# AIM-SE/AC-TSR

Hardware: NVIDIA B200
Metric: AC-SASRec train seq/s (higher is better)
Workload: dtype f32

## Files before the change

### ac-tsr_b200/csrc/attn_bwd.cu

```cuda
#include "attn_bwd_rows.cuh"

namespace acsr {

template <int DH, int G, int MAXNJ, int NS>
__device__ __forceinline__ void bwd_body(const AttnParams& p, const AttnSmem& sm, const BwdSmem<NS>& bs, const RowConst& kc,
                                         const BwdFlags& f, const float* dpen, int b, int h, int nkey, int rstride, BwdAcc& acc) {
  constexpr int dhp = DH + 4;
  constexpr int RPW = 32 / G;
  using CM = CMap<DH, G>;
  const int L = p.L, LP = (L + 3) & ~3;
  const int lane = threadIdx.x & 31, warp = threadIdx.x >> 5;
  const int grp = lane / G, sub = lane % G;
  const int c0 = CM::c0(sub);
  float* wbuf = bs.rowbuf + warp * rowbuf_floats_per_warp(LP, 2 * NS);
  const int rt = p.ctx_rows ? (int)p.ctx_rows[b] - 1 : -1;
  float accOq[CM::CPL], accDq[CM::CPL];
#pragma unroll
  for (int k = 0; k < CM::CPL; ++k) accOq[k] = accDq[k] = 0.f;
  for (int t0 = next_task(sm.misc + 2, RPW); t0 < L; t0 = next_task(sm.misc + 2, RPW)) {
    const int iw = L - 1 - t0;
    const int iraw = iw - grp;
    const bool rowok = iraw >= 0;
    const int i = rowok ? iraw : 0;
    const int bound = p.full ? nkey : min(i + 1, nkey);
    const int nj = ((p.full ? nkey : min(iw + 1, nkey)) + G - 1) / G;
    if (rt >= 0 && (rt > iw || rt <= iw - RPW)) {
#define ACSR_BWD_ROW_M(NJV) bwd_row_iter_m<DH, G, NJV, NS>(p, sm, bs, kc, dpen, b, h, i, rowok, bound, grp, sub, rstride, wbuf)
      if (MAXNJ == 1 || nj == 1) ACSR_BWD_ROW_M(1);
      else if (nj == 2) ACSR_BWD_ROW_M((MAXNJ >= 2 ? 2 : 1));
      else ACSR_BWD_ROW_M((MAXNJ >= 4 ? 4 : 1));
#undef ACSR_BWD_ROW_M
      continue;
    }
#define ACSR_BWD_ROW(NJV) \
  bwd_row_iter<DH, G, NJV, NS>(p, sm, bs, kc, f, dpen, b, h, i, rowok, bound, grp, sub, rstride, wbuf, acc, accOq, accDq)
    if (MAXNJ == 1 || nj == 1) ACSR_BWD_ROW(1);
    else if (nj == 2) ACSR_BWD_ROW((MAXNJ >= 2 ? 2 : 1));
    else ACSR_BWD_ROW((MAXNJ >= 4 ? 4 : 1));
#undef ACSR_BWD_ROW
  }
  if ((p.d_ow || p.d_dw) && CM::split(sub) == 0) {
#pragma unroll
    for (int k = 0; k < CM::CPL; ++k) {
      const int c = c0 + k;
      if (accOq[k] != 0.f) atomicAdd(bs.pacc + c, accOq[k]);
      if (accDq[k] != 0.f) atomicAdd(bs.pacc + 2 * DH + c, accDq[k]);
    }
  }
}

template <int DH, int CG, int NS>
__device__ __forceinline__ void bwd_cols(const AttnParams& p, const AttnSmem& sm, const BwdSmem<NS>& bs, const BwdFlags& f, int b, int h,
                                         int nkey) {
  constexpr int dhp = DH + 4;
  constexpr int RPW = 32 / CG;
  using CM = CMap<DH, CG>;
  const int L = p.L, LP = (L + 3) & ~3;
  const int lane = threadIdx.x & 31;
  const int grp = lane / CG, sub = lane % CG;
  const int c0 = CM::c0(sub);
  float accOk[CM::CPL], accDk[CM::CPL];
#pragma unroll
  for (int k = 0; k < CM::CPL; ++k) accOk[k] = accDk[k] = 0.f;
  for (int t0 = next_task(sm.misc + 3, RPW); t0 < nkey; t0 = next_task(sm.misc + 3, RPW)) {
    const int jraw = t0 + grp;
    const bool colok = jraw < nkey;
    const int j = colok ? jraw : 0;
    float ak_[NS][CM::CPL], ak2_[NS][CM::CPL], av_[NS][CM::CPL];
#pragma unroll
    for (int s = 0; s < NS; ++s)
#pragma unroll
      for (int k = 0; k < CM::CPL; ++k) ak_[s][k] = ak2_[s][k] = av_[s][k] = 0.f;
    int lo, hi;
    CM::slice(sub, p.full ? 0 : (j & ~3), LP, lo, hi);
    const int off = mat_row(p, j, LP);
    for (int i = lo; i < hi; i += 4) {
      float s1v[NS][4], s2v[NS][4];
#pragma unroll
      for (int s = 0; s < NS; ++s) {
        const float4 s1 = *reinterpret_cast<const float4*>(bs.matST[s] + off + i);
        const float4 s2 = *reinterpret_cast<const float4*>(bs.matS2T[s] + off + i);
        s1v[s][0] = s1.x; s1v[s][1] = s1.y; s1v[s][2] = s1.z; s1v[s][3] = s1.w;
        s2v[s][0] = s2.x; s2v[s][1] = s2.y; s2v[s][2] = s2.z; s2v[s][3] = s2.w;
      }
      const float4 pr = *reinterpret_cast<const float4*>(bs.matRT + off + i);
      const float4 pa = *reinterpret_cast<const float4*>(bs.matAT + off + i);
      const float prv[4] = {pr.x, pr.y, pr.z, pr.w}, pav[4] = {pa.x, pa.y, pa.z, pa.w};
#pragma unroll
      for (int u = 0; u < 4; ++u) {
        float qv[CM::CPL], q2v[CM::CPL], t0v[CM::CPL], t1v[CM::CPL];
        VecLd<CM::CPL>::ld(sm.Q + (i + u) * dhp + c0, qv);
        VecLd<CM::CPL>::ld(sm.Q2 + (i + u) * dhp + c0, q2v);
        VecLd<CM::CPL>::ld(bs.sT0 + (i + u) * dhp + c0, t0v);
        VecLd<CM::CPL>::ld(bs.sT1 + (i + u) * dhp + c0, t1v);
#pragma unroll
        for (int k = 0; k < CM::CPL; ++k) {
#pragma unroll
          for (int s = 0; s < NS; ++s) {
            ak_[s][k] = fmaf(s1v[s][u], qv[k], ak_[s][k]);
            ak2_[s][k] = fmaf(s2v[s][u], q2v[k], ak2_[s][k]);
          }
          av_[0][k] = fmaf(prv[u], t0v[k], av_[0][k]);
          av_[NS - 1][k] = fmaf(f.t1_att ? pav[u] : prv[u], t1v[k], av_[NS - 1][k]);
        }
      }
    }
    float kv[CM::CPL];
    VecLd<CM::CPL>::ld(sm.K + j * dhp + c0, kv);
#pragma unroll
    for (int s = 0; s < NS; ++s) {
      const float cdu = bs.colDU[s * LP + j], cdt = bs.colDT[s * LP + j];
      float o1[CM::CPL], o2[CM::CPL], o3[CM::CPL];
#pragma unroll
      for (int k = 0; k < CM::CPL; ++k) {
        o1[k] = CM::reduce(ak_[s][k]) + cdu * sm.wo[DH + c0 + k] + cdt * sm.wd[DH + c0 + k];
        o2[k] = CM::reduce(ak2_[s][k]);
        o3[k] = CM::reduce(av_[s][k]);
      }
      if (CM::split(sub) == 0 && colok) {
        const long long o = s * p.s1_td + ((long long)b * L + j) * p.d + h * DH + c0;
        VecLd<CM::CPL>::st(p.d_mk + o, o1);
        VecLd<CM::CPL>::st(p.d_ak + o, o2);
        VecLd<CM::CPL>::st(p.d_mv + o, o3);
        if (s == 0) {
#pragma unroll
          for (int k = 0; k < CM::CPL; ++k) { accOk[k] = fmaf(cdu, kv[k], accOk[k]); accDk[k] = fmaf(cdt, kv[k], accDk[k]); }
        }
      }
    }
  }
  if ((p.d_ow || p.d_dw) && CM::split(sub) == 0) {
#pragma unroll
    for (int k = 0; k < CM::CPL; ++k) {
      const int c = c0 + k;
      if (accOk[k] != 0.f) atomicAdd(bs.pacc + DH + c, accOk[k]);
      if (accDk[k] != 0.f) atomicAdd(bs.pacc + 3 * DH + c, accDk[k]);
    }
  }
}

template <int DH, int NS>
__global__ void __launch_bounds__(kAttnThreads, 2) attn_bwd_kernel(const AttnParams p) {
  pdl_launch_dependents();
  pdl_wait();
  extern __shared__ __align__(16) float smem_f[];
  constexpr int dhp = DH + 4;
  const int L = p.L, LP = (L + 3) & ~3;
  const int TRI = mat_floats(p.full, L, LP);
  const int b = p.order ? p.order[blockIdx.x / p.H] : (int)(blockIdx.x / p.H), h = blockIdx.x % p.H;
  const int lane = threadIdx.x & 31, warp = threadIdx.x >> 5;
  float* ptr = smem_f;
  AttnSmem sm = carve_common(ptr, LP, DH);
  BwdSmem<NS> bs;
  bs.sT0 = ptr; ptr += LP * dhp;
  bs.sT1 = ptr; ptr += LP * dhp;
#pragma unroll
  for (int s = 0; s < NS; ++s) { bs.matST[s] = ptr; ptr += TRI; bs.matS2T[s] = ptr; ptr += TRI; }
  bs.matRT = ptr; ptr += TRI;
  bs.matAT = ptr; ptr += TRI;
  bs.rowbuf = ptr; ptr += kAttnWarps * rowbuf_floats_per_warp(LP, 2 * NS);
  bs.colDU = ptr; ptr += NS * LP;
  bs.colDT = ptr; ptr += NS * LP;
  bs.pacc = ptr; ptr += 4 * DH;
  bs.red = ptr; ptr += kAttnWarps * 4;
  BwdFlags f;
  f.has_t0 = p.t0 != nullptr || p.dprob_cal != nullptr; f.has_t1 = p.t1 != nullptr || p.dprob_att != nullptr;
  f.t1_att = NS == 1 ? true : (p.t1_is_att != 0);
  f.has_att = f.has_t1 && f.t1_att;
  f.gate = p.combine == ACSR_ATTN_COMBINE_GATE;

  stage_tile<DH>(bs.sT0, p.t0, b, h, L, p.d, L, LP);
  stage_tile<DH>(bs.sT1, p.t1, b, h, L, p.d, L, LP);
  {
    const int ntri = (2 * NS + 2) * TRI;
    float4* z4 = reinterpret_cast<float4*>(bs.matST[0]);
    for (int e = threadIdx.x; e < ntri / 4; e += blockDim.x) z4[e] = make_float4(0.f, 0.f, 0.f, 0.f);
  }
  for (int j = threadIdx.x; j < NS * LP; j += blockDim.x) { bs.colDU[j] = 0.f; bs.colDT[j] = 0.f; }
  for (int j = threadIdx.x; j < 4 * DH; j += blockDim.x) bs.pacc[j] = 0.f;
  const int nkey = stage_common<DH>(p, sm, b, h, LP);

  const RowConst kc = make_consts<DH>(p, f.has_att);
  f.sc2 = kc.sc * kc.sc;
  float dpen[NS];
  dpen[0] = p.d_pen0 ? p.d_pen0[0] : 0.f;
  if (NS == 2) dpen[NS - 1] = p.d_pen1 ? p.d_pen1[0] : 0.f;
  BwdAcc acc;
  acc.s_ob = acc.s_db = acc.s_scalar = acc.s_ratio = 0.f;

  if (nkey <= 8) bwd_body<DH, 8, 1, NS>(p, sm, bs, kc, f, dpen, b, h, nkey, 8, acc);
  else bwd_body<DH, 16, 4, NS>(p, sm, bs, kc, f, dpen, b, h, nkey, LP, acc);
  __syncthreads();
  if (nkey <= 8) bwd_cols<DH, 32, NS>(p, sm, bs, f, b, h, nkey);
  else bwd_cols<DH, 16, NS>(p, sm, bs, f, b, h, nkey);

  for (int e = threadIdx.x; e < (L - nkey) * (DH / 4); e += blockDim.x) {
    const int j = nkey + e / (DH / 4), c4 = e % (DH / 4);
    const float4 z = make_float4(0.f, 0.f, 0.f, 0.f);
#pragma unroll
    for (int s = 0; s < NS; ++s) {
      const long long o = s * p.s1_td + ((long long)b * L + j) * p.d + h * DH + c4 * 4;
      *reinterpret_cast<float4*>(p.d_mk + o) = z;
      *reinterpret_cast<float4*>(p.d_ak + o) = z;
      *reinterpret_cast<float4*>(p.d_mv + o) = z;
    }
  }
  const float s_ob = warp_sum(acc.s_ob), s_db = warp_sum(acc.s_db);
  const float s_scalar = warp_sum(acc.s_scalar), s_ratio = warp_sum(acc.s_ratio);
  if (lane == 0) {
    bs.red[warp * 4 + 0] = s_ob; bs.red[warp * 4 + 1] = s_db; bs.red[warp * 4 + 2] = s_scalar; bs.red[warp * 4 + 3] = s_ratio;
  }
  __syncthreads();
  if (threadIdx.x < 4) {
    float s = 0.f;
    for (int w = 0; w < kAttnWarps; ++w) s += bs.red[w * 4 + threadIdx.x];
    float* dst = threadIdx.x == 0 ? p.d_ob : threadIdx.x == 1 ? p.d_db : threadIdx.x == 2 ? p.d_scalar : p.d_ratio;
    if (dst != nullptr && s != 0.f) atomicAdd(dst, s);
  }
  for (int c = threadIdx.x; c < 4 * DH; c += blockDim.x) {
    const float v = bs.pacc[c];
    float* dst = c < 2 * DH ? p.d_ow : p.d_dw;
    if (dst != nullptr && v != 0.f) atomicAdd(dst + (c < 2 * DH ? c : c - 2 * DH), v);
  }
}

static size_t bwd_smem_bytes(int L, int dh, int ns, int bidir) {
  const int LP = (L + 3) & ~3;
  size_t f = common_floats(LP, dh) + (size_t)2 * LP * (dh + 4) + (size_t)(2 * ns + 2) * mat_floats(bidir, L, LP) +
             (size_t)kAttnWarps * rowbuf_floats_per_warp(LP, 2 * ns) + 2 * ns * LP + 4 * dh + kAttnWarps * 4;
  return f * sizeof(float);
}

template <int DH, int NS>
static int launch_bwd(const AttnParams& p, cudaStream_t st) {
  size_t smem = bwd_smem_bytes(p.L, DH, NS, p.full);
  int rc = prep_kernel(attn_bwd_kernel<DH, NS>, smem, "attn_calib_bwd");
  if (rc) return rc;
  launch_pdl(attn_bwd_kernel<DH, NS>, dim3(p.B * p.H), dim3(kAttnThreads), smem, st, p);
  return check_launch("attn_calib_bwd");
}

template <int NS>
static int dispatch_bwd(const AttnParams& p, cudaStream_t st) {
  switch (p.dh) {
    case 8: return launch_bwd<8, NS>(p, st);
    case 16: return launch_bwd<16, NS>(p, st);
    case 32: return launch_bwd<32, NS>(p, st);
    case 64: return launch_bwd<64, NS>(p, st);
  }
  return ACSR_ERR_UNSUPPORTED;
}

}

using namespace acsr;

extern "C" {

int acsr_attn_calib_bwd(const float* d_ctx_att, const float* d_ctx_cal, const float* d_pen_sq, const float* mq, const float* mk,
                        const float* mv, const float* aq, const float* ak, const float* gate_logit, const int64_t* item_seq,
                        const float* order_w, const float* order_b, const float* dist_w, const float* dist_b, const float* scalar,
                        int B, int L, int H, int dh, int two_level, int combine_option, float comb_scalar, int rich_mode,
                        const float* rich_ratio, float p_attn, const float* D1, const float* D2, const float* D3,
                        const float* noise, const void* rng, uint32_t rng_stream, float* d_mq, float* d_mk, float* d_mv,
                        float* d_aq, float* d_ak, float* d_gate_logit, float* d_order_w, float* d_order_b, float* d_dist_w,
                        float* d_dist_b, float* d_scalar, float* d_rich_ratio, const int32_t* order, const int64_t* ctx_rows,
                        void* stream) {
  AttnParams p = {};
  attn_fill_common(p, mq, mk, mv, aq, ak, gate_logit, item_seq, order_w, order_b, dist_w, dist_b, scalar, B, L, H, dh, two_level,
                   combine_option, comb_scalar, rich_mode, rich_ratio, p_attn, D1, D2, D3, noise, rng, rng_stream, order, ctx_rows);
  p.t0 = d_ctx_cal; p.t1 = d_ctx_att; p.t1_is_att = 1; p.d_pen0 = d_pen_sq;
  p.d_mq = d_mq; p.d_mk = d_mk; p.d_mv = d_mv; p.d_aq = d_aq; p.d_ak = d_ak; p.d_gate = d_gate_logit;
  p.d_ow = d_order_w; p.d_ob = d_order_b; p.d_dw = d_dist_w; p.d_db = d_dist_b; p.d_scalar = d_scalar; p.d_ratio = d_rich_ratio;
  plain_range(p, d_ctx_att != nullptr);
  int rc = attn_validate(p, "attn_calib_bwd");
  if (rc) return rc;
  ACSR_REQUIRE(d_mq && d_mk && d_mv && d_aq && d_ak, "attn_calib_bwd: NULL output");
  ACSR_REQUIRE(combine_option != ACSR_ATTN_COMBINE_GATE || d_gate_logit != nullptr, "attn_calib_bwd: d_gate_logit is NULL");
  if (L > 64) return attn_long_bwd(p, 1, (cudaStream_t)stream);
  return dispatch_bwd<1>(p, (cudaStream_t)stream);
}

int acsr_attn_calib_ti_bwd(const float* d_ctx_att, const float* d_ctx_cal, const float* d_pen_sq, const float* d_prob_att,
                           const float* d_prob_cal, const float* s_bias, const float* mq, const float* mk,
                           const float* mv, const float* aq, const float* ak, const float* gate_logit, const int64_t* item_seq,
                           const float* order_w, const float* order_b, const float* dist_w, const float* dist_b, const float* scalar,
                           int B, int L, int H, int dh, int two_level, int combine_option, float comb_scalar, int rich_mode,
                           const float* rich_ratio, float p_attn, const float* D1, const float* D2, const float* D3,
                           const float* noise, const void* rng, uint32_t rng_stream, float* d_mq, float* d_mk, float* d_mv,
                           float* d_aq, float* d_ak, float* d_gate_logit, float* d_order_w, float* d_order_b, float* d_dist_w,
                           float* d_dist_b, float* d_scalar, float* d_rich_ratio, float* d_s_bias, void* stream) {
  AttnParams p = {};
  attn_fill_common(p, mq, mk, mv, aq, ak, gate_logit, item_seq, order_w, order_b, dist_w, dist_b, scalar, B, L, H, dh, two_level,
                   combine_option, comb_scalar, rich_mode, rich_ratio, p_attn, D1, D2, D3, noise, rng, rng_stream, nullptr, nullptr);
  p.t0 = d_ctx_cal; p.t1 = d_ctx_att; p.t1_is_att = 1; p.d_pen0 = d_pen_sq;
  p.s_bias = s_bias; p.dprob_att = d_prob_att; p.dprob_cal = d_prob_cal; p.d_s_bias = d_s_bias;
  p.d_mq = d_mq; p.d_mk = d_mk; p.d_mv = d_mv; p.d_aq = d_aq; p.d_ak = d_ak; p.d_gate = d_gate_logit;
  p.d_ow = d_order_w; p.d_ob = d_order_b; p.d_dw = d_dist_w; p.d_db = d_dist_b; p.d_scalar = d_scalar; p.d_ratio = d_rich_ratio;
  plain_range(p, d_ctx_att != nullptr || d_prob_att != nullptr);
  int rc = attn_validate(p, "attn_calib_ti_bwd");
  if (rc) return rc;
  ACSR_REQUIRE(d_mq && d_mk && d_mv && d_aq && d_ak, "attn_calib_ti_bwd: NULL output");
  ACSR_REQUIRE(combine_option != ACSR_ATTN_COMBINE_GATE || d_gate_logit != nullptr, "attn_calib_ti_bwd: d_gate_logit is NULL");
  ACSR_REQUIRE(p.plain && L <= 64, "attn_calib_ti_bwd: the time-aware terms need ACSR_ATTN_PLAIN and L <= 64");
  return dispatch_bwd<1>(p, (cudaStream_t)stream);
}

int acsr_attn_calib_bwd2(const float* d_ctx_cal0, const float* d_pen_sq0, const float* d_ctx_att1, const float* d_ctx_cal1,
                         const float* d_pen_sq1, const float* mq, const float* mk, const float* mv, const float* aq,
                         const float* ak, const float* gate_logit, const int64_t* item_seq, const float* order_w,
                         const float* order_b, const float* dist_w, const float* dist_b, const float* scalar, int B, int L, int H,
                         int dh, int two_level, int combine_option, float comb_scalar, int rich_mode, const float* rich_ratio,
                         float p_attn, const float* D1, const float* D2, const float* D3, const float* noise, const void* rng,
                         uint32_t rng_stream, float* d_mq, float* d_mk, float* d_mv, float* d_aq, float* d_ak,
                         float* d_gate_logit, float* d_order_w, float* d_order_b, float* d_dist_w, float* d_dist_b,
                         float* d_scalar, float* d_rich_ratio, const int32_t* order, const int64_t* ctx_rows, void* stream) {
  AttnParams p = {};
  attn_fill_common(p, mq, mk, mv, aq, ak, gate_logit, item_seq, order_w, order_b, dist_w, dist_b, scalar, B, L, H, dh, two_level,
                   combine_option, comb_scalar, rich_mode, rich_ratio, p_attn, D1, D2, D3, noise, rng, rng_stream, order, ctx_rows);
  ACSR_REQUIRE(!(d_ctx_att1 && d_ctx_cal1), "attn_calib_bwd2: stream 1 takes d_ctx_att or d_ctx_cal, not both");
  p.t0 = d_ctx_cal0; p.t1 = d_ctx_att1 ? d_ctx_att1 : d_ctx_cal1; p.t1_is_att = d_ctx_att1 != nullptr;
  p.d_pen0 = d_pen_sq0; p.d_pen1 = d_pen_sq1;
  p.s1_td = (long long)B * L * H * dh; p.s1_ll = (long long)B * L * L;
  p.d_mq = d_mq; p.d_mk = d_mk; p.d_mv = d_mv; p.d_aq = d_aq; p.d_ak = d_ak; p.d_gate = d_gate_logit;
  p.d_ow = d_order_w; p.d_ob = d_order_b; p.d_dw = d_dist_w; p.d_db = d_dist_b; p.d_scalar = d_scalar; p.d_ratio = d_rich_ratio;
  plain_range(p, d_ctx_att1 != nullptr);
  int rc = attn_validate(p, "attn_calib_bwd2");
  if (rc) return rc;
  ACSR_REQUIRE(d_mq && d_mk && d_mv && d_aq && d_ak, "attn_calib_bwd2: NULL output");
  ACSR_REQUIRE(combine_option != ACSR_ATTN_COMBINE_GATE || d_gate_logit != nullptr, "attn_calib_bwd2: d_gate_logit is NULL");
  if (L > 64) return attn_long_bwd(p, 2, (cudaStream_t)stream);
  return dispatch_bwd<2>(p, (cudaStream_t)stream);
}

}
```

### ac-tsr_b200/csrc/attn_bwd_rows.cuh

```cuda
#pragma once
#include "attn_common.cuh"

namespace acsr {

template <int NS>
struct BwdSmem {
  float *sT0, *sT1;
  float *matST[NS], *matS2T[NS];
  float *matRT, *matAT;
  float *rowbuf;
  float *colDU, *colDT;
  float *pacc;
  float *red;
  float *gS[NS], *gS2[NS], *gR, *gA;
};

struct BwdAcc {
  float s_ob, s_db, s_scalar, s_ratio;
};

struct BwdFlags {
  bool has_t0, has_t1, t1_att, has_att, gate;
  float sc2;
};

template <int DH, int G, int NJ, int NS, bool LONG = false>
__device__ __forceinline__ void bwd_row_iter(const AttnParams& p, const AttnSmem& sm, const BwdSmem<NS>& bs, const RowConst& kc,
                                             const BwdFlags& f, const float* dpen, int b, int h, int i, bool rowok, int bound,
                                             int grp, int sub, int rstride, float* wbuf, BwdAcc& acc, float* accOq,
                                             float* accDq) {
  constexpr int dhp = DH + 4;
  using CM = CMap<DH, G>;
  const int L = p.L, LP = (L + 3) & ~3;
  RowF<NJ> r;
  row_forward<DH, G, NJ>(p, sm, kc, b, h, i, bound, sub, f.has_att, r);
  const unsigned act = r.act;
  float d0[NJ], d1[NJ];
#pragma unroll
  for (int jj = 0; jj < NJ; ++jj) d0[jj] = d1[jj] = 0.f;
  if (f.has_t0 || f.has_t1) {
    const float4* a0 = reinterpret_cast<const float4*>(bs.sT0 + i * dhp);
    const float4* a1 = reinterpret_cast<const float4*>(bs.sT1 + i * dhp);
#pragma unroll
    for (int jj = 0; jj < NJ; ++jj) {
      const int jcl = ((act >> jj) & 1u) ? sub + G * jj : 0;
      const float4* vj = reinterpret_cast<const float4*>(sm.V + jcl * dhp);
      float x0 = 0.f, x1 = 0.f;
#pragma unroll
      for (int c4 = 0; c4 < DH / 4; ++c4) {
        const float4 v = vj[c4];
        if (f.has_t0) x0 = dot4(a0[c4], v, x0);
        if (f.has_t1) x1 = dot4(a1[c4], v, x1);
      }
      if ((act >> jj) & 1u) { d0[jj] = x0; d1[jj] = x1; }
    }
  }
  if (p.dprob_cal != nullptr || p.dprob_att != nullptr) {
    const long long ebase = (((long long)b * p.H + h) * L + i) * L;
#pragma unroll
    for (int jj = 0; jj < NJ; ++jj)
      if ((act >> jj) & 1u) {
        const int j = sub + G * jj;
        if (p.dprob_cal != nullptr) d0[jj] += __ldg(p.dprob_cal + ebase + j);
        if (p.dprob_att != nullptr) d1[jj] += __ldg(p.dprob_att + ebase + j);
      }
  }
  float Pj[NJ], Mj[NJ], Oj[NJ], expm[NJ];
#pragma unroll
  for (int jj = 0; jj < NJ; ++jj) {
    const bool a = (act >> jj) & 1u;
    Pj[jj] = r.Psoft[jj] * r.D1[jj];
    Mj[jj] = r.Msoft[jj] * r.D3[jj];
    Oj[jj] = p.two_level ? Pj[jj] : r.P0soft[jj] * r.D2[jj];
    expm[jj] = a ? fexp(1.0f - Mj[jj]) : 0.f;
    if (a && rowok) {
      const int j = sub + G * jj;
      const float rfin = p.two_level ? r.R[jj] : (kc.rr * r.R[jj] + (1.0f - kc.rr) * Pj[jj]);
      if (LONG) {
        bs.gR[(long long)i * L + j] = rfin;
        bs.gA[(long long)i * L + j] = r.A[jj];
      } else {
        const int t = mat_row(p, j, LP) + i;
        bs.matRT[t] = rfin;
        bs.matAT[t] = r.A[jj];
      }
    }
  }
  float* gbuf = wbuf + grp * 2 * NS * rstride;
  bool live[NS];
  float row_du[NS], row_dt[NS];
#pragma unroll
  for (int s = 0; s < NS; ++s) {
    float* bufS = gbuf + (2 * s + 0) * rstride;
    float* bufS2 = gbuf + (2 * s + 1) * rstride;
    row_du[s] = row_dt[s] = 0.f;
    const float* dRf = (NS == 1 || s == 0) ? d0 : d1;
    const float* dA = d1;
    bool useR = (NS == 1 || s == 0) ? f.has_t0 : (f.has_t1 && !f.t1_att);
    bool useA = (NS == 1) ? f.has_t1 : (s == 1 && f.has_t1 && f.t1_att);
    bool nzR = false, nzA = false;
#pragma unroll
    for (int jj = 0; jj < NJ; ++jj) { nzR |= dRf[jj] != 0.f; nzA |= dA[jj] != 0.f; }
    useR = useR && __any_sync(kFull, nzR && rowok);
    useA = useA && __any_sync(kFull, nzA && rowok);
    const float dp = dpen[s];
    live[s] = useR || useA || dp != 0.f;
    if (!live[s]) {
      if (LONG && rowok) {
#pragma unroll
        for (int jj = 0; jj < NJ; ++jj)
          if ((act >> jj) & 1u) {
            const long long e = (long long)i * L + sub + G * jj;
            bs.gS[s][e] = 0.f;
            bs.gS2[s][e] = 0.f;
          }
      }
      continue;
    }
    const bool owner = s == 0;
    float dO[NJ], dP[NJ], dM[NJ], tmp[NJ];
#pragma unroll
    for (int jj = 0; jj < NJ; ++jj) { dO[jj] = 0.f; dP[jj] = 0.f; dM[jj] = 0.f; }
    if (useR) {
      float dR[NJ], dcm[NJ], dC[NJ];
#pragma unroll
      for (int jj = 0; jj < NJ; ++jj) {
        if (p.two_level) dR[jj] = dRf[jj];
        else {
          dR[jj] = dRf[jj] * kc.rr;
          dP[jj] = dRf[jj] * (1.0f - kc.rr);
          if (owner && rowok) acc.s_ratio += dRf[jj] * (r.R[jj] - Pj[jj]);
        }
      }
      if (p.plain) {
#pragma unroll
        for (int jj = 0; jj < NJ; ++jj) dcm[jj] = dR[jj];
      } else softmax_bwd_row<G, NJ>(r.R, dR, dcm);
      if (p.combine == ACSR_ATTN_COMBINE_FIXED) {
        softmax_bwd_row<G, NJ>(r.F, dcm, tmp);
#pragma unroll
        for (int jj = 0; jj < NJ; ++jj) { dO[jj] += tmp[jj]; dC[jj] = 0.5f * tmp[jj]; }
      } else {
#pragma unroll
        for (int jj = 0; jj < NJ; ++jj) {
          const float g = r.g[jj];
          dO[jj] += dcm[jj] * g;
          dC[jj] = dcm[jj] * (1.0f - g);
          if (f.gate && ((act >> jj) & 1u) && rowok) {
            const float dgl = dcm[jj] * (Oj[jj] - r.C[jj]) * g * (1.0f - g);
            if (dgl != 0.f) atomicAdd(p.d_gate + s * p.s1_ll + ((long long)b * L + i) * L + sub + G * jj, dgl);
          }
        }
      }
      if (p.plain) {
#pragma unroll
        for (int jj = 0; jj < NJ; ++jj) tmp[jj] = dC[jj];
      } else softmax_bwd_row<G, NJ>(r.C, dC, tmp);
#pragma unroll
      for (int jj = 0; jj < NJ; ++jj) {
        dO[jj] += tmp[jj] * expm[jj];
        dM[jj] -= tmp[jj] * Oj[jj] * expm[jj];
      }
    }
    if (useA) {
      if (p.plain) {
#pragma unroll
        for (int jj = 0; jj < NJ; ++jj) tmp[jj] = dA[jj];
      } else softmax_bwd_row<G, NJ>(r.A, dA, tmp);
#pragma unroll
      for (int jj = 0; jj < NJ; ++jj) {
        dO[jj] += tmp[jj] * Mj[jj];
        dM[jj] += tmp[jj] * (Oj[jj] - r.nz[jj]);
      }
    }
    float dS2[NJ], dS[NJ], dz[NJ];
#pragma unroll
    for (int jj = 0; jj < NJ; ++jj) {
      if ((act >> jj) & 1u) dM[jj] += dp * (-2.0f) * (1.0f - Mj[jj]);
      dM[jj] *= r.D3[jj];
    }
    softmax_bwd_row<G, NJ>(r.Msoft, dM, dS2);
#pragma unroll
    for (int jj = 0; jj < NJ; ++jj) { dS2[jj] *= kc.inv_sq; dz[jj] = 0.f; dS[jj] = 0.f; }
    if (useR || useA) {
      float dP0[NJ];
#pragma unroll
      for (int jj = 0; jj < NJ; ++jj) {
        if (p.two_level) { dP[jj] += dO[jj]; dP0[jj] = 0.f; }
        else dP0[jj] = dO[jj] * r.D2[jj];
        dP[jj] *= r.D1[jj];
      }
      softmax_bwd_row<G, NJ>(r.Psoft, dP, dz);
#pragma unroll
      for (int jj = 0; jj < NJ; ++jj) { dz[jj] *= kc.inv_sq; dS[jj] = dz[jj]; }
      if (!p.two_level) {
        softmax_bwd_row<G, NJ>(r.P0soft, dP0, tmp);
#pragma unroll
        for (int jj = 0; jj < NJ; ++jj) dS[jj] += tmp[jj] * kc.inv_sq;
      }
    }
    float rdu = 0.f, rdt = 0.f;
#pragma unroll
    for (int jj = 0; jj < NJ; ++jj) {
      const int j = sub + G * jj;
      const bool a = ((act >> jj) & 1u) && rowok;
      if (j < rstride) { bufS[j] = a ? dS[jj] : 0.f; bufS2[j] = a ? dS2[jj] : 0.f; }
      if (!a) continue;
      if (p.ow) {
        const float sg = r.sig[jj];
        const float de = (j > i) ? sg * (1.0f - sg) * frcp(sg + kOrderEps) : -sg * (1.0f - sg) * frcp((1.0f - sg) + kOrderEps);
        const float du = dz[jj] * de;
        rdu += du;
        if (du != 0.f) atomicAdd(bs.colDU + s * LP + j, du);
      }
      if (p.dw) {
        const float dl = r.delta[jj];
        const float dt = dz[jj] * dl * f.sc2;
        rdt += dt;
        if (dt != 0.f) atomicAdd(bs.colDT + s * LP + j, dt);
        if (owner) acc.s_scalar += dz[jj] * (-(dl * dl) * kc.sc);
      }
      if (LONG) {
        bs.gS[s][(long long)i * L + j] = dS[jj];
        bs.gS2[s][(long long)i * L + j] = dS2[jj];
      } else {
        const int t = mat_row(p, j, LP) + i;
        bs.matST[s][t] = dS[jj];
        bs.matS2T[s][t] = dS2[jj];
        if (NS == 1 && p.d_s_bias != nullptr) p.d_s_bias[(((long long)b * p.H + h) * L + i) * L + j] = dS[jj];
      }
    }
    row_du[s] = grp_sum<G>(rdu);
    row_dt[s] = grp_sum<G>(rdt);
  }
  if (sub == 0) { acc.s_ob += row_du[0]; acc.s_db += row_dt[0]; }
  __syncwarp();
  float aq_[NS][CM::CPL], aq2_[NS][CM::CPL];
#pragma unroll
  for (int s = 0; s < NS; ++s)
#pragma unroll
    for (int k = 0; k < CM::CPL; ++k) aq_[s][k] = aq2_[s][k] = 0.f;
  int lo, hi;
  CM::slice(sub, 0, (bound + 3) & ~3, lo, hi);
  const int c0 = CM::c0(sub);
  bool any_live = false;
#pragma unroll
  for (int s = 0; s < NS; ++s) any_live |= live[s];
  if (any_live) {
    for (int j = lo; j < hi; j += 4) {
      float s1v[NS][4], s2v[NS][4];
#pragma unroll
      for (int s = 0; s < NS; ++s) {
        const float4 s1 = *reinterpret_cast<const float4*>(gbuf + (2 * s + 0) * rstride + j);
        const float4 s2 = *reinterpret_cast<const float4*>(gbuf + (2 * s + 1) * rstride + j);
        s1v[s][0] = s1.x; s1v[s][1] = s1.y; s1v[s][2] = s1.z; s1v[s][3] = s1.w;
        s2v[s][0] = s2.x; s2v[s][1] = s2.y; s2v[s][2] = s2.z; s2v[s][3] = s2.w;
      }
#pragma unroll
      for (int u = 0; u < 4; ++u) {
        float kv[CM::CPL], k2v[CM::CPL];
        VecLd<CM::CPL>::ld(sm.K + (j + u) * dhp + c0, kv);
        VecLd<CM::CPL>::ld(sm.K2 + (j + u) * dhp + c0, k2v);
#pragma unroll
        for (int s = 0; s < NS; ++s) {
          if (!live[s]) continue;
#pragma unroll
          for (int k = 0; k < CM::CPL; ++k) {
            aq_[s][k] = fmaf(s1v[s][u], kv[k], aq_[s][k]);
            aq2_[s][k] = fmaf(s2v[s][u], k2v[k], aq2_[s][k]);
          }
        }
      }
    }
  }
  {
    float qv[CM::CPL];
    VecLd<CM::CPL>::ld(sm.Q + i * dhp + c0, qv);
#pragma unroll
    for (int s = 0; s < NS; ++s) {
      float o1[CM::CPL], o2[CM::CPL];
#pragma unroll
      for (int k = 0; k < CM::CPL; ++k) {
        o1[k] = CM::reduce(aq_[s][k]) + row_du[s] * sm.wo[c0 + k] + row_dt[s] * sm.wd[c0 + k];
        o2[k] = CM::reduce(aq2_[s][k]);
      }
      if (CM::split(sub) == 0 && rowok) {
        const long long o = s * p.s1_td + ((long long)b * L + i) * p.d + h * DH + c0;
        VecLd<CM::CPL>::st(p.d_mq + o, o1);
        VecLd<CM::CPL>::st(p.d_aq + o, o2);
      }
    }
    if (CM::split(sub) == 0 && rowok) {
#pragma unroll
      for (int k = 0; k < CM::CPL; ++k) { accOq[k] = fmaf(row_du[0], qv[k], accOq[k]); accDq[k] = fmaf(row_dt[0], qv[k], accDq[k]); }
    }
  }
  __syncwarp();
}

template <int DH, int G, int NJ, int NS, bool LONG = false>
__device__ __forceinline__ void bwd_row_iter_m(const AttnParams& p, const AttnSmem& sm, const BwdSmem<NS>& bs, const RowConst& kc,
                                               const float* dpen, int b, int h, int i, bool rowok, int bound, int grp, int sub,
                                               int rstride, float* wbuf) {
  constexpr int dhp = DH + 4;
  using CM = CMap<DH, G>;
  const int L = p.L, LP = (L + 3) & ~3;
  float Msoft[NJ], D3[NJ];
  unsigned act;
  row_forward_m<DH, G, NJ>(p, sm, kc, b, h, i, bound, sub, Msoft, D3, act);
  float* gbuf = wbuf + grp * 2 * NS * rstride;
  const int c0 = CM::c0(sub);
  if (LONG && rowok) {
#pragma unroll
    for (int jj = 0; jj < NJ; ++jj)
      if ((act >> jj) & 1u) {
        const long long e = (long long)i * L + sub + G * jj;
        bs.gR[e] = 0.f;
        bs.gA[e] = 0.f;
#pragma unroll
        for (int s = 0; s < NS; ++s) {
          bs.gS[s][e] = 0.f;
          if (dpen[s] == 0.f) bs.gS2[s][e] = 0.f;
        }
      }
  }
#pragma unroll
  for (int s = 0; s < NS; ++s) {
    const float dp = dpen[s];
    float o2[CM::CPL];
#pragma unroll
    for (int k = 0; k < CM::CPL; ++k) o2[k] = 0.f;
    if (dp != 0.f) {
      float dM[NJ], dS2[NJ];
#pragma unroll
      for (int jj = 0; jj < NJ; ++jj) dM[jj] = ((act >> jj) & 1u) ? dp * (-2.0f) * (1.0f - Msoft[jj] * D3[jj]) * D3[jj] : 0.f;
      softmax_bwd_row<G, NJ>(Msoft, dM, dS2);
      float* bufS2 = gbuf + (2 * s + 1) * rstride;
#pragma unroll
// ... 39 lines not shown
```

### ac-tsr_b200/csrc/attn_common.cuh

```cuda
#pragma once
#include "acsr_common.cuh"
#include "../../include/acsr.h"

namespace acsr {

constexpr int kAttnWarps = 8;
constexpr int kAttnThreads = kAttnWarps * 32;
constexpr unsigned kFull = 0xffffffffu;

struct AttnParams {
  const float *mq, *mk, *mv, *aq, *ak, *gate;
  const int64_t* item_seq;
  const int32_t* order;
  const int64_t* ctx_rows;
  const float *ow, *ob, *dw, *db, *scalar;
  int B, L, H, dh, d;
  int two_level, combine, rich;
  int bidir;
  int plain;
  int full;
  float comb_scalar;
  const float* rich_ratio;
  float p;
  const float *D1, *D2, *D3, *noise;
  const RngState* rng;
  uint32_t stream;
  float *ctx_att, *ctx_cal;
  double* pen_sq;
  float* probs;
  const float* s_bias;
  float *prob_att_out, *prob_cal_out;
  const float *dprob_att, *dprob_cal;
  float* d_s_bias;
  const float *t0, *t1;
  int t1_is_att;
  const float *d_pen0, *d_pen1;
  long long s1_td, s1_ll;
  float *d_mq, *d_mk, *d_mv, *d_aq, *d_ak, *d_gate, *d_ow, *d_ob, *d_dw, *d_db, *d_scalar, *d_ratio;
};

template <int G>
__device__ __forceinline__ float grp_sum(float v) {
#pragma unroll
  for (int o = G / 2; o > 0; o >>= 1) v += __shfl_xor_sync(kFull, v, o);
  return v;
}
template <int G>
__device__ __forceinline__ float grp_max(float v) {
#pragma unroll
  for (int o = G / 2; o > 0; o >>= 1) v = fmaxf(v, __shfl_xor_sync(kFull, v, o));
  return v;
}

template <int DH, int G>
struct CMap {
  static constexpr int CPL = DH >= G ? DH / G : 1;
  static constexpr int SPL = DH >= G ? 1 : G / DH;
  __device__ static __forceinline__ int c0(int sub) { return DH >= G ? sub * CPL : sub % DH; }
  __device__ static __forceinline__ int split(int sub) { return DH >= G ? 0 : sub / DH; }
  __device__ static __forceinline__ float reduce(float v) {
#pragma unroll
    for (int o = DH; o < G; o <<= 1) v += __shfl_xor_sync(kFull, v, o);
    return v;
  }
  __device__ static __forceinline__ void slice(int sub, int begin, int end, int& lo, int& hi) {
    if (SPL == 1) { lo = begin; hi = end; return; }
    const int chunk = (((end - begin + SPL - 1) / SPL) + 3) & ~3;
    lo = begin + split(sub) * chunk;
    hi = min(end, lo + chunk);
  }
};

template <int N> struct VecLd;
template <> struct VecLd<1> {
  __device__ static __forceinline__ void ld(const float* p, float* v) { v[0] = p[0]; }
  __device__ static __forceinline__ void st(float* p, const float* v) { p[0] = v[0]; }
};
template <> struct VecLd<2> {
  __device__ static __forceinline__ void ld(const float* p, float* v) { const float2 t = *reinterpret_cast<const float2*>(p); v[0] = t.x; v[1] = t.y; }
  __device__ static __forceinline__ void st(float* p, const float* v) { *reinterpret_cast<float2*>(p) = make_float2(v[0], v[1]); }
};
template <> struct VecLd<4> {
  __device__ static __forceinline__ void ld(const float* p, float* v) { const float4 t = *reinterpret_cast<const float4*>(p); v[0] = t.x; v[1] = t.y; v[2] = t.z; v[3] = t.w; }
  __device__ static __forceinline__ void st(float* p, const float* v) { *reinterpret_cast<float4*>(p) = make_float4(v[0], v[1], v[2], v[3]); }
};
template <> struct VecLd<8> {
  __device__ static __forceinline__ void ld(const float* p, float* v) { VecLd<4>::ld(p, v); VecLd<4>::ld(p + 4, v + 4); }
  __device__ static __forceinline__ void st(float* p, const float* v) { VecLd<4>::st(p, v); VecLd<4>::st(p + 4, v + 4); }
};

template <int NJ>
struct RowF {
  float Psoft[NJ], Msoft[NJ], P0soft[NJ];
  float D1[NJ], D2[NJ], D3[NJ], nz[NJ];
  float A[NJ], C[NJ], g[NJ], F[NJ], R[NJ];
  float sig[NJ], delta[NJ];
  unsigned act;
  unsigned valid;
};

struct AttnSmem {
  float *Q, *K, *V, *Q2, *K2;
  float *rowO, *rowD, *colO, *colD, *logd, *keyok;
  float *wo, *wd;
  const float* G;
  int* misc;
};

struct RowConst {
  float ob, db, sc, sc2h, rr, inv_sq, inv_keep;
  unsigned thr16;
  unsigned long long seed, step;
  bool philox_drop, philox_noise, need_p0;
  bool bounded;
};

__device__ __forceinline__ float fex2(float x) { float y; asm("ex2.approx.ftz.f32 %0, %1;" : "=f"(y) : "f"(x)); return y; }
__device__ __forceinline__ float flg2(float x) { float y; asm("lg2.approx.ftz.f32 %0, %1;" : "=f"(y) : "f"(x)); return y; }
__device__ __forceinline__ float frcp(float x) { float y; asm("rcp.approx.ftz.f32 %0, %1;" : "=f"(y) : "f"(x)); return y; }
__device__ __forceinline__ float fexp(float x) { return fex2(x * 1.4426950408889634f); }
__device__ __forceinline__ float flog(float x) { return flg2(x) * 0.6931471805599453f; }
__device__ __forceinline__ float fsigmoid(float x) { return frcp(1.0f + fex2(x * -1.4426950408889634f)); }

__device__ __forceinline__ void cp_async16(void* smem, const void* gmem) {
  asm volatile("cp.async.cg.shared.global [%0], [%1], 16;" ::"r"(smem_u32(smem)), "l"(gmem) : "memory");
}
__device__ __forceinline__ void cp_async4(void* smem, const void* gmem) {
  asm volatile("cp.async.ca.shared.global [%0], [%1], 4;" ::"r"(smem_u32(smem)), "l"(gmem) : "memory");
}
__device__ __forceinline__ void cp_async_wait_all() {
  asm volatile("cp.async.commit_group;\n\tcp.async.wait_group 0;" ::: "memory");
}

__device__ __forceinline__ float dot4(const float4 a, const float4 b, float acc) {
  acc = fmaf(a.x, b.x, acc); acc = fmaf(a.y, b.y, acc); acc = fmaf(a.z, b.z, acc); acc = fmaf(a.w, b.w, acc);
  return acc;
}

template <int G, int NJ>
__device__ __forceinline__ void softmax_row(const float* z, unsigned act, float* y) {
  float m = -INFINITY;
#pragma unroll
  for (int jj = 0; jj < NJ; ++jj) if ((act >> jj) & 1u) m = fmaxf(m, z[jj]);
  m = grp_max<G>(m) * 1.4426950408889634f;
  float s = 0.f;
#pragma unroll
  for (int jj = 0; jj < NJ; ++jj) { y[jj] = ((act >> jj) & 1u) ? fex2(fmaf(z[jj], 1.4426950408889634f, -m)) : 0.f; s += y[jj]; }
  s = grp_sum<G>(s);
  const float inv = frcp(s);
#pragma unroll
  for (int jj = 0; jj < NJ; ++jj) y[jj] *= inv;
}

template <int G, int NJ>
__device__ __forceinline__ void softmax_row_bounded(const float* z, unsigned act, float* y) {
  float s = 0.f;
#pragma unroll
  for (int jj = 0; jj < NJ; ++jj) { y[jj] = ((act >> jj) & 1u) ? fex2(z[jj] * 1.4426950408889634f) : 0.f; s += y[jj]; }
  s = grp_sum<G>(s);
  const float inv = s > 0.f ? frcp(s) : 0.f;
#pragma unroll
  for (int jj = 0; jj < NJ; ++jj) y[jj] *= inv;
}

template <int G, int NJ>
__device__ __forceinline__ void softmax_bwd_row(const float* y, const float* dy, float* dz) {
  float s = 0.f;
#pragma unroll
  for (int jj = 0; jj < NJ; ++jj) s = fmaf(y[jj], dy[jj], s);
  s = grp_sum<G>(s);
#pragma unroll
  for (int jj = 0; jj < NJ; ++jj) dz[jj] = y[jj] * (dy[jj] - s);
}

__device__ __forceinline__ int next_task(int* counter, int step) {
  int t = 0;
  if ((threadIdx.x & 31) == 0) t = atomicAdd(counter, step);
  return __shfl_sync(kFull, t, 0);
}

__host__ __device__ __forceinline__ int tri_off(int j, int LP) {
  const int a = j >> 2, b = j & 3;
  return j * LP - 8 * a * (a - 1) - 4 * a * b;
}

__device__ __forceinline__ int mat_row(const AttnParams& p, int j, int LP) { return p.full ? j * LP : tri_off(j, LP) - (j & ~3); }
__host__ __device__ __forceinline__ int mat_floats(int bidir, int L, int LP) { return bidir ? L * LP : tri_off(L, LP); }

template <int DH>
__device__ __forceinline__ void stage_tile(float* dst, const float* __restrict__ src, int b, int h, int L, int d, int rows,
                                           int rows_pad) {
  constexpr int dhp = DH + 4;
  if (src == nullptr) rows = 0;
  const float* base = src + (long long)b * L * d + h * DH;
  for (int e = threadIdx.x; e < rows_pad * (DH / 4); e += blockDim.x) {
    const int r = e / (DH / 4), c4 = e % (DH / 4);
    if (r < rows) cp_async16(dst + r * dhp + c4 * 4, base + (long long)r * d + c4 * 4);
    else *reinterpret_cast<float4*>(dst + r * dhp + c4 * 4) = make_float4(0.f, 0.f, 0.f, 0.f);
  }
}

template <int DH>
__device__ __forceinline__ int stage_common(const AttnParams& p, const AttnSmem& sm, int b, int h, int LP) {
  constexpr int dhp = DH + 4;
  const int L = p.L;
  if (threadIdx.x < 64) {
    const int j = threadIdx.x;
    const bool ok = j < L && p.item_seq[(long long)b * L + j] != 0;
    const unsigned m = __ballot_sync(kFull, ok);
    if ((threadIdx.x & 31) == 0) sm.misc[threadIdx.x >> 5] = (int)m;
    if (threadIdx.x >= 2 && threadIdx.x < 5) sm.misc[threadIdx.x] = 0;
    if (j < LP) { sm.keyok[j] = ok ? 1.0f : 0.0f; sm.logd[j] = logf((float)j + 1.0f); }
  }
  stage_tile<DH>(sm.Q, p.mq, b, h, L, p.d, L, LP);
  stage_tile<DH>(sm.Q2, p.aq, b, h, L, p.d, L, LP);
  for (int c = threadIdx.x; c < 2 * DH; c += blockDim.x) {
    sm.wo[c] = p.ow ? p.ow[c] : 0.f;
    sm.wd[c] = p.dw ? p.dw[c] : 0.f;
  }
  __syncthreads();
  const unsigned m0 = (unsigned)sm.misc[0], m1 = (unsigned)sm.misc[1];
  int nkey = m1 ? 64 - __clz(m1) : (m0 ? 32 - __clz(m0) : 0);
  nkey = max(nkey, 1);
  if (p.plain && p.full) nkey = L;
  const int nkp = (nkey + 3) & ~3;
  stage_tile<DH>(sm.K, p.mk, b, h, L, p.d, nkey, nkp);
  stage_tile<DH>(sm.V, p.mv, b, h, L, p.d, nkey, nkp);
  stage_tile<DH>(sm.K2, p.ak, b, h, L, p.d, nkey, nkp);
  cp_async_wait_all();
  __syncthreads();
  if (p.ow || p.dw) {
    const int j = threadIdx.x >> 2, part = threadIdx.x & 3;
    float ro = 0.f, rd = 0.f, co = 0.f, cd = 0.f;
    if (j < L) {
#pragma unroll
      for (int cc = 0; cc < DH / 4; ++cc) {
        const int c = part * (DH / 4) + cc;
        const float q = sm.Q[j * dhp + c];
        ro = fmaf(q, sm.wo[c], ro); rd = fmaf(q, sm.wd[c], rd);
        if (j < nkey) {
          const float k = sm.K[j * dhp + c];
          co = fmaf(k, sm.wo[DH + c], co); cd = fmaf(k, sm.wd[DH + c], cd);
        }
      }
    }
    ro += __shfl_xor_sync(kFull, ro, 1); ro += __shfl_xor_sync(kFull, ro, 2);
    rd += __shfl_xor_sync(kFull, rd, 1); rd += __shfl_xor_sync(kFull, rd, 2);
    co += __shfl_xor_sync(kFull, co, 1); co += __shfl_xor_sync(kFull, co, 2);
    cd += __shfl_xor_sync(kFull, cd, 1); cd += __shfl_xor_sync(kFull, cd, 2);
    if (part == 0 && j < LP) { sm.rowO[j] = ro; sm.rowD[j] = rd; sm.colO[j] = co; sm.colD[j] = cd; }
    __syncthreads();
  }
  return nkey;
}

template <int DH>
__device__ __forceinline__ RowConst make_consts(const AttnParams& p, bool need_att) {
  RowConst k;
  k.ob = p.ob ? p.ob[0] : 0.f;
  k.db = p.db ? p.db[0] : 0.f;
  k.sc = p.scalar ? p.scalar[0] : 0.f;
  k.sc2h = k.sc * k.sc * 0.5f;
  k.rr = 1.0f;
  if (!p.two_level) k.rr = (p.rich == ACSR_ATTN_RICH_TRAINABLE) ? p.rich_ratio[0] : 0.5f;
  k.inv_sq = 1.0f / sqrtf((float)DH);
  k.inv_keep = p.p > 0.f ? 1.0f / (1.0f - p.p) : 1.0f;
  k.thr16 = (unsigned)(p.p * 65536.0f + 0.5f);
  k.bounded = k.inv_keep <= 16.0f;
  k.philox_drop = p.p > 0.f && p.D1 == nullptr;
  k.philox_noise = need_att && p.noise == nullptr && p.rng != nullptr;
  k.need_p0 = !p.two_level || p.probs != nullptr;
  k.seed = 0; k.step = 0;
  if (p.rng != nullptr) { k.seed = p.rng->seed; k.step = p.rng->step; }
  return k;
}

template <int DH, int G, int NJ>
__device__ __forceinline__ void row_forward(const AttnParams& p, const AttnSmem& sm, const RowConst& kc, int b, int h, int i,
                                            int bound, int sub, bool need_att, RowF<NJ>& r) {
  constexpr int dhp = DH + 4;
  const int L = p.L;
  int jc[NJ];
  float S[NJ], S2[NJ], gl[NJ];
  unsigned act = 0;
#pragma unroll
  for (int jj = 0; jj < NJ; ++jj) {
    const int j = sub + G * jj;
    const bool a = j < bound;
    act |= (a ? 1u : 0u) << jj;
    jc[jj] = a ? j : 0;
    gl[jj] = 0.f;
  }
  r.act = act;
  const long long ebase = (((long long)b * p.H + h) * L + i) * L;
  if (p.combine == ACSR_ATTN_COMBINE_GATE) {
    if (sm.G != nullptr) {
      const float* gp = sm.G + i * L;
#pragma unroll
      for (int jj = 0; jj < NJ; ++jj) if ((act >> jj) & 1u) gl[jj] = gp[jc[jj]];
    } else {
      const float* gp = p.gate + ((long long)b * L + i) * L;
#pragma unroll
      for (int jj = 0; jj < NJ; ++jj) if ((act >> jj) & 1u) gl[jj] = __ldg(gp + jc[jj]);
    }
  }
  {
    const float4* qi = reinterpret_cast<const float4*>(sm.Q + i * dhp);
    const float4* q2i = reinterpret_cast<const float4*>(sm.Q2 + i * dhp);
    if (NJ == 1) {
      const float4* kj = reinterpret_cast<const float4*>(sm.K + jc[0] * dhp);
      const float4* k2j = reinterpret_cast<const float4*>(sm.K2 + jc[0] * dhp);
      float s = 0.f, s2 = 0.f;
#pragma unroll
      for (int c4 = 0; c4 < DH / 4; ++c4) { s = dot4(qi[c4], kj[c4], s); s2 = dot4(q2i[c4], k2j[c4], s2); }
      S[0] = s; S2[0] = s2;
    } else {
      {
        float4 q[DH / 4];
#pragma unroll
        for (int c4 = 0; c4 < DH / 4; ++c4) q[c4] = qi[c4];
#pragma unroll
        for (int jj = 0; jj < NJ; ++jj) {
          const float4* kj = reinterpret_cast<const float4*>(sm.K + jc[jj] * dhp);
          float s = 0.f;
#pragma unroll
          for (int c4 = 0; c4 < DH / 4; ++c4) s = dot4(q[c4], kj[c4], s);
          S[jj] = s;
        }
      }
      {
        float4 q[DH / 4];
#pragma unroll
        for (int c4 = 0; c4 < DH / 4; ++c4) q[c4] = q2i[c4];
#pragma unroll
        for (int jj = 0; jj < NJ; ++jj) {
          const float4* kj = reinterpret_cast<const float4*>(sm.K2 + jc[jj] * dhp);
          float s = 0.f;
#pragma unroll
          for (int c4 = 0; c4 < DH / 4; ++c4) s = dot4(q[c4], kj[c4], s);
          S2[jj] = s;
        }
      }
    }
  }
  if (p.s_bias != nullptr) {
#pragma unroll
    for (int jj = 0; jj < NJ; ++jj) if ((act >> jj) & 1u) S[jj] += __ldg(p.s_bias + ebase + jc[jj]);
  }
  const float rowO = sm.rowO[i], rowD = sm.rowD[i];
  float zP[NJ], z0[NJ], zM[NJ];
  unsigned valid = 0;
#pragma unroll
  for (int jj = 0; jj < NJ; ++jj) {
    const int j = jc[jj];
    const bool a = (act >> jj) & 1u;
    const bool v = a && (p.bidir || j <= i) && (sm.keyok[j] != 0.f);
    valid |= (v ? 1u : 0u) << jj;
    const float msk = v ? 0.f : kMaskNeg;
    r.sig[jj] = 0.f; r.delta[jj] = 0.f;
    float eo = 0.f, ed = 0.f;
    if (p.ow) {
      const float sg = fsigmoid(rowO + sm.colO[j] + kc.ob);
      r.sig[jj] = sg;
      eo = (j > i) ? flog(sg + kOrderEps) : flog((1.0f - sg) + kOrderEps);
    }
    if (p.dw) {
      const int dist = i > j ? i - j : j - i;
      const float dl = sm.logd[dist] - (rowD + sm.colD[j] + kc.db);
      r.delta[jj] = dl;
      ed = -(dl * dl) * kc.sc2h;
    }
    zP[jj] = (S[jj] + eo + ed) * kc.inv_sq + msk;
    z0[jj] = S[jj] * kc.inv_sq + msk;
    zM[jj] = S2[jj] * kc.inv_sq + msk;
  }
  r.valid = valid;
  softmax_row<G, NJ>(zP, act, r.Psoft);
  softmax_row<G, NJ>(zM, act, r.Msoft);
  if (kc.need_p0) softmax_row<G, NJ>(z0, act, r.P0soft);
  else {
#pragma unroll
    for (int jj = 0; jj < NJ; ++jj) r.P0soft[jj] = 0.f;
  }
#pragma unroll
  for (int jj = 0; jj < NJ; ++jj) { r.D1[jj] = r.D2[jj] = r.D3[jj] = 1.0f; r.nz[jj] = 0.f; }
  if (kc.philox_drop || kc.philox_noise) {
#pragma unroll
    for (int jj = 0; jj < NJ; jj += 2) {
      const uint4 w = philox4x32(kc.seed, kc.step, p.stream, (unsigned long long)(ebase + jc[jj]));
      if (kc.philox_drop) {
        r.D1[jj] = ((w.x & 0xffffu) >= kc.thr16) ? kc.inv_keep : 0.f;
        r.D3[jj] = ((w.x >> 16) >= kc.thr16) ? kc.inv_keep : 0.f;
        if (jj + 1 < NJ) {
          r.D1[jj + 1] = ((w.y & 0xffffu) >= kc.thr16) ? kc.inv_keep : 0.f;
          r.D3[jj + 1] = ((w.y >> 16) >= kc.thr16) ? kc.inv_keep : 0.f;
        }
      }
      if (kc.philox_noise) {
        const float rad = sqrtf(-2.0f * flog(u32_to_unit(w.z)));
        float sn, cs;
        __sincosf(6.283185307179586f * u32_to_unit(w.w), &sn, &cs);
        r.nz[jj] = rad * cs;
        if (jj + 1 < NJ) r.nz[jj + 1] = rad * sn;
      }
      if (kc.philox_drop && kc.need_p0) {
        const uint4 w2 = philox4x32(kc.seed, kc.step, p.stream + 1u, (unsigned long long)(ebase + jc[jj]));
        r.D2[jj] = ((w2.x & 0xffffu) >= kc.thr16) ? kc.inv_keep : 0.f;
        if (jj + 1 < NJ) r.D2[jj + 1] = ((w2.x >> 16) >= kc.thr16) ? kc.inv_keep : 0.f;
      }
    }
  }
  if (p.D1 || p.noise) {
#pragma unroll
    for (int jj = 0; jj < NJ; ++jj) {
      if (!((act >> jj) & 1u)) continue;
      const long long e = ebase + jc[jj];
      if (p.D1) r.D1[jj] = p.D1[e];
      if (p.D2) r.D2[jj] = p.D2[e];
      if (p.D3) r.D3[jj] = p.D3[e];
      if (p.noise) r.nz[jj] = p.noise[e];
    }
  }
  float O[NJ], M[NJ], expm[NJ], z[NJ];
#pragma unroll
  for (int jj = 0; jj < NJ; ++jj) {
    const bool a = (act >> jj) & 1u;
    M[jj] = r.Msoft[jj] * r.D3[jj];
    O[jj] = p.two_level ? r.Psoft[jj] * r.D1[jj] : r.P0soft[jj] * r.D2[jj];
    expm[jj] = a ? fexp(1.0f - M[jj]) : 0.f;
  }
  if (need_att) {
#pragma unroll
    for (int jj = 0; jj < NJ; ++jj)
      z[jj] = O[jj] * M[jj] + r.nz[jj] * (1.0f - M[jj]) + ((p.plain || ((valid >> jj) & 1u)) ? 0.f : kMaskNeg);
    if (p.plain) {
#pragma unroll
      for (int jj = 0; jj < NJ; ++jj) r.A[jj] = ((act >> jj) & 1u) ? z[jj] : 0.f;
    } else softmax_row<G, NJ>(z, act, r.A);
  } else {
#pragma unroll
    for (int jj = 0; jj < NJ; ++jj) r.A[jj] = 0.f;
  }
#pragma unroll
  for (int jj = 0; jj < NJ; ++jj) z[jj] = O[jj] * expm[jj] + ((p.plain || ((valid >> jj) & 1u)) ? 0.f : kMaskNeg);
  if (p.plain) {
#pragma unroll
    for (int jj = 0; jj < NJ; ++jj) r.C[jj] = z[jj];
  } else if (kc.bounded) softmax_row_bounded<G, NJ>(z, act, r.C);
  else softmax_row<G, NJ>(z, act, r.C);
  if (p.combine == ACSR_ATTN_COMBINE_FIXED) {
    const float ninact = (float)(L - bound);
    float m = -INFINITY;
#pragma unroll
    for (int jj = 0; jj < NJ; ++jj) { z[jj] = O[jj] + 0.5f * r.C[jj]; r.g[jj] = 0.f; if ((act >> jj) & 1u) m = fmaxf(m, z[jj]); }
    m = grp_max<G>(m);
    if (ninact > 0.f) m = fmaxf(m, 0.f);
    float s = 0.f;
#pragma unroll
    for (int jj = 0; jj < NJ; ++jj) { r.F[jj] = ((act >> jj) & 1u) ? fexp(z[jj] - m) : 0.f; s += r.F[jj]; }
    s = grp_sum<G>(s) + ninact * fexp(-m);
    const float inv = frcp(s);
#pragma unroll
    for (int jj = 0; jj < NJ; ++jj) { r.F[jj] *= inv; z[jj] = r.F[jj] + (((valid >> jj) & 1u) ? 0.f : kMaskNeg); }
  } else {
#pragma unroll
    for (int jj = 0; jj < NJ; ++jj) {
      float g = p.comb_scalar;
      if (p.combine == ACSR_ATTN_COMBINE_GATE) g = fsigmoid(gl[jj]);
      r.g[jj] = g; r.F[jj] = 0.f;
      z[jj] = g * O[jj] + (1.0f - g) * r.C[jj] + ((p.plain || ((valid >> jj) & 1u)) ? 0.f : kMaskNeg);
    }
  }
  if (p.plain) {
    const bool fixed = p.combine == ACSR_ATTN_COMBINE_FIXED;
#pragma unroll
    for (int jj = 0; jj < NJ; ++jj) r.R[jj] = fixed ? r.F[jj] : (((act >> jj) & 1u) ? z[jj] : 0.f);
    return;
  }
  if (kc.bounded) softmax_row_bounded<G, NJ>(z, act, r.R);
  else softmax_row<G, NJ>(z, act, r.R);
}

template <int DH, int G, int NJ>
__device__ __forceinline__ void row_forward_m(const AttnParams& p, const AttnSmem& sm, const RowConst& kc, int b, int h, int i,
                                              int bound, int sub, float* Msoft, float* D3, unsigned& act_out) {
  constexpr int dhp = DH + 4;
  const int L = p.L;
  int jc[NJ];
  float zM[NJ];
  unsigned act = 0;
#pragma unroll
  for (int jj = 0; jj < NJ; ++jj) {
    const int j = sub + G * jj;
    const bool a = j < bound;
    act |= (a ? 1u : 0u) << jj;
    jc[jj] = a ? j : 0;
  }
  act_out = act;
  const long long ebase = (((long long)b * p.H + h) * L + i) * L;
  const float4* q2i = reinterpret_cast<const float4*>(sm.Q2 + i * dhp);
#pragma unroll
  for (int jj = 0; jj < NJ; ++jj) {
    const float4* kj = reinterpret_cast<const float4*>(sm.K2 + jc[jj] * dhp);
    float s0 = 0.f, s1 = 0.f;
#pragma unroll
    for (int c4 = 0; c4 < DH / 4; c4 += 2) { s0 = dot4(q2i[c4], kj[c4], s0); s1 = dot4(q2i[c4 + 1], kj[c4 + 1], s1); }
    const bool v = ((act >> jj) & 1u) && (p.bidir || jc[jj] <= i) && (sm.keyok[jc[jj]] != 0.f);
    zM[jj] = (s0 + s1) * kc.inv_sq + (v ? 0.f : kMaskNeg);
  }
  softmax_row<G, NJ>(zM, act, Msoft);
#pragma unroll
  for (int jj = 0; jj < NJ; ++jj) D3[jj] = 1.0f;
  if (kc.philox_drop) {
#pragma unroll
    for (int jj = 0; jj < NJ; jj += 2) {
      const uint4 w = philox4x32(kc.seed, kc.step, p.stream, (unsigned long long)(ebase + jc[jj]));
      D3[jj] = ((w.x >> 16) >= kc.thr16) ? kc.inv_keep : 0.f;
      if (jj + 1 < NJ) D3[jj + 1] = ((w.y >> 16) >= kc.thr16) ? kc.inv_keep : 0.f;
    }
  }
  if (p.D3) {
#pragma unroll
    for (int jj = 0; jj < NJ; ++jj) if ((act >> jj) & 1u) D3[jj] = p.D3[ebase + jc[jj]];
  }
}

__device__ __forceinline__ AttnSmem carve_common(float*& ptr, int LP, int dh) {
  AttnSmem sm;
  const int tile = LP * (dh + 4);
  sm.Q = ptr; ptr += tile;
  sm.K = ptr; ptr += tile;
  sm.V = ptr; ptr += tile;
  sm.Q2 = ptr; ptr += tile;
  sm.K2 = ptr; ptr += tile;
  sm.rowO = ptr; ptr += LP;
  sm.rowD = ptr; ptr += LP;
  sm.colO = ptr; ptr += LP;
  sm.colD = ptr; ptr += LP;
  sm.logd = ptr; ptr += LP;
  sm.keyok = ptr; ptr += LP;
  sm.wo = ptr; ptr += 2 * dh;
  sm.wd = ptr; ptr += 2 * dh;
  sm.misc = reinterpret_cast<int*>(ptr); ptr += 8;
  sm.G = nullptr;
  return sm;
}
static inline size_t common_floats(int LP, int dh) { return (size_t)5 * LP * (dh + 4) + 6 * LP + 4 * dh + 8; }

__host__ __device__ __forceinline__ int rowbuf_floats_per_warp(int LP, int bufs_per_row) {
  const int a = 2 * bufs_per_row * LP, b = 4 * bufs_per_row * 8;
  return a > b ? a : b;
}

template <typename K>
static int prep_kernel(K kernel, size_t smem, const char* who) {
  if (smem > 227 * 1024) { set_error("%s: needs %zu bytes of shared memory (> 227 KB)", who, smem); return ACSR_ERR_UNSUPPORTED; }
  cudaError_t e = cudaFuncSetAttribute(kernel, cudaFuncAttributeMaxDynamicSharedMemorySize, (int)smem);
  if (e == cudaSuccess) e = cudaFuncSetAttribute(kernel, cudaFuncAttributePreferredSharedMemoryCarveout, 100);
  if (e != cudaSuccess) { set_error("%s: smem %zu: %s", who, smem, cudaGetErrorString(e)); return ACSR_ERR_CUDA; }
  return ACSR_OK;
}

static inline int attn_validate(const AttnParams& p, const char* who) {
  ACSR_REQUIRE(p.mq && p.mk && p.mv && p.aq && p.ak && p.item_seq, "%s: NULL input", who);
  ACSR_REQUIRE(p.B > 0 && p.H > 0, "%s: bad B/H", who);
  if (p.L < 1 || p.L > 256) { set_error("%s: L=%d unsupported (1..256)", who, p.L); return ACSR_ERR_UNSUPPORTED; }
  if ((p.full || p.plain) && p.L > 64) { set_error("%s: the bidirectional mask / the transformer_layers variant are implemented for L <= 64 (L=%d)", who, p.L); return ACSR_ERR_UNSUPPORTED; }
  if (!(p.dh == 8 || p.dh == 16 || p.dh == 32 || p.dh == 64)) {
    set_error("%s: head size %d unsupported (8/16/32/64)", who, p.dh);
    return ACSR_ERR_UNSUPPORTED;
  }
  ACSR_REQUIRE((p.ow == nullptr) == (p.ob == nullptr), "%s: order_w/order_b mismatch", who);
  ACSR_REQUIRE((p.dw == nullptr) == (p.db == nullptr) && (p.dw == nullptr) == (p.scalar == nullptr), "%s: distance params mismatch", who);
  ACSR_REQUIRE(p.combine >= 0 && p.combine <= 2, "%s: unknown combine_option %d", who, p.combine);
  ACSR_REQUIRE(p.combine != ACSR_ATTN_COMBINE_GATE || p.gate != nullptr, "%s: combine_option gate needs gate_logit", who);
  ACSR_REQUIRE(p.two_level || p.rich == ACSR_ATTN_RICH_FIXED || (p.rich == ACSR_ATTN_RICH_TRAINABLE && p.rich_ratio),
               "%s: two_level=False needs rich_calibrated_combine fixed/trainable", who);
  ACSR_REQUIRE(p.p >= 0.f && p.p < 1.f, "%s: dropout p=%f", who, p.p);
  ACSR_REQUIRE(!(p.p > 0.f && p.D1 == nullptr && p.rng == nullptr), "%s: p>0 needs explicit masks or rng", who);
  ACSR_REQUIRE((p.D1 == nullptr) == (p.D3 == nullptr), "%s: D1/D3 must be given together", who);
  return ACSR_OK;
}

static inline void plain_range(AttnParams& p, bool attacked_stream) {
  if (p.plain && !p.bidir && !attacked_stream && p.combine != ACSR_ATTN_COMBINE_FIXED) p.full = 0;
}

int attn_long_fwd(const AttnParams& p, cudaStream_t st);
int attn_long_bwd(const AttnParams& p, int ns, cudaStream_t st);
int seq_order_long(const int64_t* item_seq, int B, int L, int32_t* order, cudaStream_t st);

static inline void attn_fill_common(AttnParams& p, const float* mq, const float* mk, const float* mv, const float* aq,
                                    const float* ak, const float* gate_logit, const int64_t* item_seq, const float* order_w,
                                    const float* order_b, const float* dist_w, const float* dist_b, const float* scalar, int B,
                                    int L, int H, int dh, int two_level, int combine_option, float comb_scalar, int rich_mode,
                                    const float* rich_ratio, float p_attn, const float* D1, const float* D2, const float* D3,
                                    const float* noise, const void* rng, uint32_t rng_stream, const int32_t* order, const int64_t* ctx_rows) {
  p.order = order; p.ctx_rows = ctx_rows;
  p.mq = mq; p.mk = mk; p.mv = mv; p.aq = aq; p.ak = ak; p.gate = combine_option == ACSR_ATTN_COMBINE_GATE ? gate_logit : nullptr;
  p.item_seq = item_seq;
  p.ow = order_w; p.ob = order_b; p.dw = dist_w; p.db = dist_b; p.scalar = scalar;
  p.B = B; p.L = L; p.H = H; p.dh = dh; p.d = H * dh;
  p.two_level = two_level & 1; p.bidir = (two_level >> 1) & 1; p.plain = (two_level >> 2) & 1; p.full = p.bidir | p.plain; p.combine = combine_option; p.rich = rich_mode; p.comb_scalar = comb_scalar; p.rich_ratio = rich_ratio;
  p.p = p_attn; p.D1 = D1; p.D2 = D2; p.D3 = D3; p.noise = noise; p.rng = (const RngState*)rng; p.stream = rng_stream;
}

}
```

### ac-tsr_b200/csrc/attn_fwd.cu

```cuda
#include "attn_fwd_rows.cuh"

namespace acsr {

template <int DH, int G, int MAXNJ>
__device__ __forceinline__ void fwd_rows(const AttnParams& p, const AttnSmem& sm, const RowConst& kc, int b, int h, int nkey,
                                         bool need_att, int rstride, FwdCtx& cx) {
  constexpr int RPW = 32 / G;
  const int L = p.L;
  const int lane = threadIdx.x & 31;
  const int grp = lane / G, sub = lane % G;
  const int rt = p.ctx_rows ? (int)p.ctx_rows[b] - 1 : -1;
  for (int t0 = next_task(sm.misc + 2, RPW); t0 < L; t0 = next_task(sm.misc + 2, RPW)) {
    const int iw = L - 1 - t0;
    const int iraw = iw - grp;
    const bool rowok = iraw >= 0;
    const int i = rowok ? iraw : 0;
    const int bound = p.full ? nkey : min(i + 1, nkey);
    const int nj = ((p.full ? nkey : min(iw + 1, nkey)) + G - 1) / G;
    if (rt >= 0 && (rt > iw || rt <= iw - RPW)) {
      if (p.pen_sq == nullptr) continue;
      if (MAXNJ == 1 || nj == 1) fwd_row_iter_m<DH, G, 1>(p, sm, kc, b, h, i, rowok, bound, sub, cx);
      else if (nj == 2) fwd_row_iter_m<DH, G, (MAXNJ >= 2 ? 2 : 1)>(p, sm, kc, b, h, i, rowok, bound, sub, cx);
      else if (nj == 3) fwd_row_iter_m<DH, G, (MAXNJ >= 3 ? 3 : 1)>(p, sm, kc, b, h, i, rowok, bound, sub, cx);
      else fwd_row_iter_m<DH, G, (MAXNJ >= 4 ? 4 : 1)>(p, sm, kc, b, h, i, rowok, bound, sub, cx);
      continue;
    }
    if (MAXNJ == 1 || nj == 1) fwd_row_iter<DH, G, 1>(p, sm, kc, b, h, i, rowok, bound, grp, sub, need_att, rstride, cx);
    else if (nj == 2) fwd_row_iter<DH, G, (MAXNJ >= 2 ? 2 : 1)>(p, sm, kc, b, h, i, rowok, bound, grp, sub, need_att, rstride, cx);
    else if (nj == 3) fwd_row_iter<DH, G, (MAXNJ >= 3 ? 3 : 1)>(p, sm, kc, b, h, i, rowok, bound, grp, sub, need_att, rstride, cx);
    else fwd_row_iter<DH, G, (MAXNJ >= 4 ? 4 : 1)>(p, sm, kc, b, h, i, rowok, bound, grp, sub, need_att, rstride, cx);
  }
}

template <int DH>
__global__ void __launch_bounds__(kAttnThreads, 4) attn_fwd_kernel(const AttnParams p) {
  pdl_launch_dependents();
  pdl_wait();
  extern __shared__ __align__(16) float smem_f[];
  const int L = p.L, LP = (L + 3) & ~3;
  const int b = p.order ? p.order[blockIdx.x / p.H] : (int)(blockIdx.x / p.H), h = blockIdx.x % p.H;
  const int lane = threadIdx.x & 31, warp = threadIdx.x >> 5;
  float* ptr = smem_f;
  AttnSmem sm = carve_common(ptr, LP, DH);
  const int rbw = rowbuf_floats_per_warp(LP, 2);
  FwdCtx cx;
  cx.rowbuf = ptr + warp * rbw;
  cx.pen = 0.f;
  ptr += kAttnWarps * rbw;
  double* pen_red = reinterpret_cast<double*>(ptr);
  if (threadIdx.x == 0) *pen_red = 0.0;
  const int nkey = stage_common<DH>(p, sm, b, h, LP);
  const bool need_att = p.ctx_att != nullptr;
  const RowConst kc = make_consts<DH>(p, need_att);
  if (p.probs) {
    const long long plane = (long long)p.B * p.H * L * L;
    float* base = p.probs + ((long long)b * p.H + h) * L * L;
    for (int e = threadIdx.x; e < L * L; e += blockDim.x)
#pragma unroll
      for (int k = 0; k < 6; ++k) base[k * plane + e] = 0.f;
    __syncthreads();
  }
  if (nkey <= 8) fwd_rows<DH, 8, 1>(p, sm, kc, b, h, nkey, need_att, 8, cx);
  else fwd_rows<DH, 16, 4>(p, sm, kc, b, h, nkey, need_att, LP, cx);
  const double pd = warp_sum_d((double)cx.pen);
  if (lane == 0 && p.pen_sq != nullptr) {
    atomicAdd(pen_red, pd);
    __threadfence_block();
    if (atomicAdd(sm.misc + 4, 1) == kAttnWarps - 1) atomicAdd(p.pen_sq, *reinterpret_cast<volatile double*>(pen_red));
  }
}

static size_t fwd_smem_bytes(int L, int dh) {
  const int LP = (L + 3) & ~3;
  size_t f = common_floats(LP, dh) + (size_t)kAttnWarps * rowbuf_floats_per_warp(LP, 2);
  return f * sizeof(float) + kAttnWarps * sizeof(double);
}

template <int DH>
static int launch_fwd(const AttnParams& p, cudaStream_t st) {
  size_t smem = fwd_smem_bytes(p.L, DH);
  int rc = prep_kernel(attn_fwd_kernel<DH>, smem, "attn_calib_fwd");
  if (rc) return rc;
  launch_pdl(attn_fwd_kernel<DH>, dim3(p.B * p.H), dim3(kAttnThreads), smem, st, p);
  return check_launch("attn_calib_fwd");
}

__global__ void __launch_bounds__(256) seq_order_kernel(const int64_t* __restrict__ item_seq, int B, int L, int32_t* __restrict__ order) {
  pdl_launch_dependents();
  pdl_wait();
  __shared__ int cnt[66], off[66];
  __shared__ unsigned char key[2048];
  for (int i = threadIdx.x; i < 66; i += blockDim.x) cnt[i] = 0;
  __syncthreads();
  for (int b = threadIdx.x; b < B; b += blockDim.x) {
    const long long* row = reinterpret_cast<const long long*>(item_seq) + (long long)b * L;
    unsigned long long m = 0ull;
#pragma unroll 16
    for (int j = 0; j < L; ++j) m |= (unsigned long long)(__ldg(row + j) != 0) << j;
    const int nkey = m ? 64 - __clzll((long long)m) : 0;
    key[b] = (unsigned char)nkey;
    atomicAdd(cnt + nkey, 1);
  }
  __syncthreads();
  if (threadIdx.x == 0) {
    int run = 0;
    for (int k = 65; k >= 0; --k) { off[k] = run; run += cnt[k]; }
  }
  __syncthreads();
  for (int b = threadIdx.x; b < B; b += blockDim.x) order[atomicAdd(off + key[b], 1)] = b;
}

}

using namespace acsr;

extern "C" int acsr_seq_order(const int64_t* item_seq, int B, int L, int32_t* order, void* stream) {
  ACSR_REQUIRE(item_seq && order && B > 0 && B <= 2048 && L > 0 && L <= 1024, "seq_order: bad arguments (B <= 2048, L <= 1024)");
  if (L > 64) return seq_order_long(item_seq, B, L, order, (cudaStream_t)stream);
  launch_pdl(seq_order_kernel, dim3(1), dim3(256), 0, (cudaStream_t)stream, item_seq, B, L, order);
  return check_launch("seq_order");
}


extern "C" int acsr_attn_calib_fwd(const float* mq, const float* mk, const float* mv, const float* aq, const float* ak,
                                   const float* gate_logit, const int64_t* item_seq, const float* order_w, const float* order_b,
                                   const float* dist_w, const float* dist_b, const float* scalar, int B, int L, int H, int dh,
                                   int two_level, int combine_option, float comb_scalar, int rich_mode, const float* rich_ratio,
                                   float p_attn, const float* D1, const float* D2, const float* D3, const float* noise,
                                   const void* rng, uint32_t rng_stream, float* ctx_att, float* ctx_cal, double* pen_sq,
                                   float* probs_out, const int32_t* order, const int64_t* ctx_rows, void* stream) {
  AttnParams p = {};
  attn_fill_common(p, mq, mk, mv, aq, ak, gate_logit, item_seq, order_w, order_b, dist_w, dist_b, scalar, B, L, H, dh, two_level,
                   combine_option, comb_scalar, rich_mode, rich_ratio, p_attn, D1, D2, D3, noise, rng, rng_stream, order, ctx_rows);
  p.ctx_att = ctx_att; p.ctx_cal = ctx_cal; p.pen_sq = pen_sq; p.probs = probs_out;
  plain_range(p, ctx_att != nullptr || probs_out != nullptr);
  int rc = attn_validate(p, "attn_calib_fwd");
  if (rc) return rc;
  ACSR_REQUIRE(ctx_cal != nullptr, "attn_calib_fwd: ctx_cal is NULL");
  if (L > 64) return attn_long_fwd(p, (cudaStream_t)stream);
  switch (dh) {
    case 8: return launch_fwd<8>(p, (cudaStream_t)stream);
    case 16: return launch_fwd<16>(p, (cudaStream_t)stream);
    case 32: return launch_fwd<32>(p, (cudaStream_t)stream);
    case 64: return launch_fwd<64>(p, (cudaStream_t)stream);
  }
  return ACSR_ERR_UNSUPPORTED;
}

extern "C" int acsr_attn_calib_ti_fwd(const float* s_bias, const float* mq, const float* mk, const float* mv, const float* aq,
                                      const float* ak, const float* gate_logit, const int64_t* item_seq, const float* order_w,
                                      const float* order_b, const float* dist_w, const float* dist_b, const float* scalar, int B,
                                      int L, int H, int dh, int two_level, int combine_option, float comb_scalar, int rich_mode,
                                      const float* rich_ratio, float p_attn, const float* D1, const float* D2, const float* D3,
                                      const float* noise, const void* rng, uint32_t rng_stream, float* ctx_att, float* ctx_cal,
                                      double* pen_sq, float* prob_att, float* prob_cal, void* stream) {
  AttnParams p = {};
  attn_fill_common(p, mq, mk, mv, aq, ak, gate_logit, item_seq, order_w, order_b, dist_w, dist_b, scalar, B, L, H, dh, two_level,
                   combine_option, comb_scalar, rich_mode, rich_ratio, p_attn, D1, D2, D3, noise, rng, rng_stream, nullptr, nullptr);
  p.ctx_att = ctx_att; p.ctx_cal = ctx_cal; p.pen_sq = pen_sq; p.probs = nullptr;
  p.s_bias = s_bias; p.prob_att_out = prob_att; p.prob_cal_out = prob_cal;
  plain_range(p, ctx_att != nullptr);
  int rc = attn_validate(p, "attn_calib_ti_fwd");
  if (rc) return rc;
  ACSR_REQUIRE(ctx_cal != nullptr && prob_cal != nullptr, "attn_calib_ti_fwd: ctx_cal / prob_cal is NULL");
  ACSR_REQUIRE(p.plain && L <= 64, "attn_calib_ti_fwd: the time-aware terms need ACSR_ATTN_PLAIN and L <= 64");
  switch (dh) {
    case 8: return launch_fwd<8>(p, (cudaStream_t)stream);
    case 16: return launch_fwd<16>(p, (cudaStream_t)stream);
    case 32: return launch_fwd<32>(p, (cudaStream_t)stream);
    case 64: return launch_fwd<64>(p, (cudaStream_t)stream);
  }
  return ACSR_ERR_UNSUPPORTED;
}
```

### ac-tsr_b200/csrc/attn_fwd_rows.cuh

```cuda
#pragma once
#include "attn_common.cuh"

namespace acsr {

struct FwdCtx {
  float* rowbuf;
  float pen;
};

template <int DH, int G, int NJ>
__device__ __forceinline__ void fwd_row_iter(const AttnParams& p, const AttnSmem& sm, const RowConst& kc, int b, int h, int i,
                                             bool rowok, int bound, int grp, int sub, bool need_att, int rstride, FwdCtx& cx) {
  constexpr int dhp = DH + 4;
  using CM = CMap<DH, G>;
  const int L = p.L;
  RowF<NJ> r;
  row_forward<DH, G, NJ>(p, sm, kc, b, h, i, bound, sub, need_att, r);
  float* bufR = cx.rowbuf + (grp * 2 + 0) * rstride;
  float* bufA = cx.rowbuf + (grp * 2 + 1) * rstride;
#pragma unroll
  for (int jj = 0; jj < NJ; ++jj) {
    const int j = sub + G * jj;
    const bool a = (r.act >> jj) & 1u;
    const float Pj = r.Psoft[jj] * r.D1[jj];
    const float Rf = p.two_level ? r.R[jj] : (kc.rr * r.R[jj] + (1.0f - kc.rr) * Pj);
    const float Mj = r.Msoft[jj] * r.D3[jj];
    if (j < rstride) {
      bufR[j] = a ? Rf : 0.f;
      bufA[j] = a ? r.A[jj] : 0.f;
    }
    if (a && rowok) { const float om = 1.0f - Mj; cx.pen = fmaf(om, om, cx.pen); }
    if (p.prob_cal_out != nullptr && a && rowok) {
      const long long e = (((long long)b * p.H + h) * L + i) * L + j;
      p.prob_cal_out[e] = Rf;
      if (p.prob_att_out != nullptr && need_att) p.prob_att_out[e] = r.A[jj];
    }
    if (p.probs && a && rowok) {
      const long long e = (((long long)b * p.H + h) * L + i) * L + j;
      const long long plane = (long long)p.B * p.H * L * L;
      p.probs[0 * plane + e] = r.P0soft[jj] * r.D2[jj]; p.probs[1 * plane + e] = Pj;
      p.probs[2 * plane + e] = Mj; p.probs[3 * plane + e] = r.A[jj];
      p.probs[4 * plane + e] = r.C[jj]; p.probs[5 * plane + e] = Rf;
    }
  }
  if (rowok && sub == 0) cx.pen += (float)(L - bound);
  __syncwarp();
  float accR[CM::CPL], accA[CM::CPL];
#pragma unroll
  for (int k = 0; k < CM::CPL; ++k) accR[k] = accA[k] = 0.f;
  int lo, hi;
  CM::slice(sub, 0, (bound + 3) & ~3, lo, hi);
  const int c0 = CM::c0(sub);
  for (int j = lo; j < hi; j += 4) {
    const float4 pr = *reinterpret_cast<const float4*>(bufR + j);
    const float4 pa = *reinterpret_cast<const float4*>(bufA + j);
    const float prv[4] = {pr.x, pr.y, pr.z, pr.w}, pav[4] = {pa.x, pa.y, pa.z, pa.w};
#pragma unroll
    for (int u = 0; u < 4; ++u) {
      float v[CM::CPL];
      VecLd<CM::CPL>::ld(sm.V + (j + u) * dhp + c0, v);
#pragma unroll
      for (int k = 0; k < CM::CPL; ++k) {
        accR[k] = fmaf(prv[u], v[k], accR[k]);
        if (need_att) accA[k] = fmaf(pav[u], v[k], accA[k]);
      }
    }
  }
#pragma unroll
  for (int k = 0; k < CM::CPL; ++k) { accR[k] = CM::reduce(accR[k]); accA[k] = CM::reduce(accA[k]); }
  if (CM::split(sub) == 0 && rowok) {
    const long long o = ((long long)b * L + i) * p.d + h * DH + c0;
    VecLd<CM::CPL>::st(p.ctx_cal + o, accR);
    if (need_att) VecLd<CM::CPL>::st(p.ctx_att + o, accA);
  }
  __syncwarp();
}

template <int DH, int G, int NJ>
__device__ __forceinline__ void fwd_row_iter_m(const AttnParams& p, const AttnSmem& sm, const RowConst& kc, int b, int h, int i,
                                               bool rowok, int bound, int sub, FwdCtx& cx) {
  float Msoft[NJ], D3[NJ];
  unsigned act;
  row_forward_m<DH, G, NJ>(p, sm, kc, b, h, i, bound, sub, Msoft, D3, act);
  if (!rowok) return;
#pragma unroll
  for (int jj = 0; jj < NJ; ++jj)
    if ((act >> jj) & 1u) { const float om = 1.0f - Msoft[jj] * D3[jj]; cx.pen = fmaf(om, om, cx.pen); }
  if (sub == 0) cx.pen += (float)(p.L - bound);
}

}
```

### ac-tsr_b200/fused_step.py

```python
import math

import torch

from . import ops
from ._lib import LIB
from .ops import _p, _stream


class _RandSlice(object):

    def __init__(self, rand, sl):
        self.rand, self.sl = rand, sl

    def get(self, key):
        t = self.rand.get(key)
        return None if t is None else t[self.sl].contiguous()


class FusedTrainStep(object):
    def __init__(self, model, optimizer):
        if model.loss_type not in ('CE', 'BPR'):
            raise NotImplementedError("Make sure 'loss_type' in ['BPR', 'CE']!")
        self.m, self.opt = model, optimizer
        self.buf = {}
        self.vp = None
        self.tc = model.hidden_size == 64 and model.inner_size <= 256 and model.inner_size % 4 == 0
        self.passes = 3
        self.overlap_wgrad = True
        self.n_branches = int(getattr(model, 'step_branches', 1))
        self._streams = {}
        self.pdl = True
        self.tail_fused = self.tc and model.inner_size % 16 == 0
        self.dense_bwd = self.tc and model.inner_size % 64 == 0
        self.ce_fused_bwd = model.hidden_size == 64

    def _stream_for(self, dev, key):
        if key not in self._streams:
            self._streams[key] = torch.cuda.Stream(device=dev)
        return self._streams[key]

    def _branch_buffers(self, Bs, L, dev, idx, grads=True):
        key = ('branch', Bs, L, idx)
        if key in self.buf:
            return self.buf[key]
        m = self.m
        d, I, N = m.hidden_size, m.inner_size, m.n_layers
        T = Bs * L

        def f(*s):
            return torch.empty(s, dtype=torch.float32, device=dev)
        b = dict(T=T, x0=f(T, d), st_e=f(T, 2), layers=[], order=torch.empty(Bs, dtype=torch.int32, device=dev))
        for l in range(N):
            last = l == N - 1
            qkv5 = f(5, T, d)
            qkv, aqk = qkv5[:3], qkv5[3:]
            lb = dict(qkv5=qkv5, qkv=qkv, aqk=aqk, mq=qkv[0], mk=qkv[1], mv=qkv[2], aq=aqk[0], ak=aqk[1], gl=f(T, L),
                      ctx=f(2 * T if last else T, d))
            if not last:
                lb.update(hz=f(T, d), st_a=f(T, 2), h=f(T, d), z1=f(T, I), a1=f(T, I), z2=f(T, d), st_f=f(T, 2), out=f(T, d))
            if grads:
                lb['d_gl'] = f(2 * T, L)
                if not last:
                    lb['d_z2'], lb['d_z1'], lb['d_hz'] = f(2 * T, d), f(2 * T, I), f(2 * T, d)
                lb['d_qkv'], lb['d_aqk'] = f(3, 2 * T, d), f(2, 2 * T, d)
                lb['d_mq'], lb['d_mk'], lb['d_mv'] = lb['d_qkv'][0], lb['d_qkv'][1], lb['d_qkv'][2]
                lb['d_aq'], lb['d_ak'] = lb['d_aqk'][0], lb['d_aqk'][1]
            b['layers'].append(lb)
        C = 2 * Bs
        b['c'] = dict(ctx=f(C, d), x=f(Bs, d), hz=f(C, d), st_a=f(C, 2), h=f(C, d), z1=f(C, I), a1=f(C, I), z2=f(C, d), st_f=f(C, 2),
                      out=f(C, d), d_out=f(C, d), d_z2=f(C, d), d_h=f(C, d), d_a1=f(C, I), d_z1=f(C, I), d_hz=f(C, d), d_x=f(C, d),
                      d_ctx=f(C, d))
        if grads:
            for n, w in (('d_out', d), ('d_a1', I), ('d_h', d), ('d_x', d), ('d_ctx', d)):
                b[n] = f(2 * T, w)
        self.buf[key] = b
        return b

    def _joint_buffers(self, B, dev):
        key = ('joint', B)
        if key in self.buf:
            return self.buf[key]
        m = self.m
        d, N, V = m.hidden_size, m.n_layers, m.n_items

        def f(*s):
            return torch.empty(s, dtype=torch.float32, device=dev)
        nc = ops.logits_num_chunks(2 * B, V, d)
        loss3 = f(3)
        j = dict(pen=torch.zeros(N, dtype=torch.float64, device=dev), out2=f(2 * B, d), partial=f(2 * B, nc, 2), lse=f(2 * B),
                 tgt=f(2 * B), row_loss=f(2 * B), loss3=loss3, loss=loss3[:2], loss_att=loss3[2:], dpen=f(N), Gt=None,
                 d_out2=f(2 * B, d),
                 target2=torch.empty(2 * B, dtype=torch.int64, device=dev), ce_cnt=torch.zeros(1, dtype=torch.int32, device=dev),
                 neg2=torch.empty(2 * B, dtype=torch.int64, device=dev), row_x=f(2 * B),
                 row_scale=torch.cat((torch.full((B,), 1.0 / B), torch.full((B,), -1.0 / B))).to(dev))
        self.buf[key] = j
        return j

    @torch.no_grad()
    def __call__(self, interaction):
        was = LIB.query('acsr_set_pdl', 1 if self.pdl else 0)
        try:
            return self._step(interaction)
        finally:
            LIB.query('acsr_set_pdl', was)

    def _step(self, interaction):
        m, opt = self.m, self.opt
        seq = interaction[m.ITEM_SEQ].contiguous()
        ln = interaction[m.ITEM_SEQ_LEN].contiguous()
        pos_items = interaction[m.POS_ITEM_ID]
        B, L = seq.shape
        dev = seq.device
        d, N, V = m.hidden_size, m.n_layers, m.n_items
        rt = m._runtime(dev)
        rng, rand = rt.rng, rt.rand
        training = m.training
        E = m.item_embedding.weight
        main = torch.cuda.current_stream()
        nb = self.n_branches if (self.n_branches > 1 and B % self.n_branches == 0 and L <= 64 and self.vp is None) else 1
        Bs = B // nb
        jb = self._joint_buffers(B, dev)
        branches = []
        for s in range(nb):
            sl = slice(s * Bs, (s + 1) * Bs)
            branches.append(dict(idx=s, sl=sl, seq=seq[sl], ln=ln[sl], buf=self._branch_buffers(Bs, L, dev, s),
                                 rand=rand if (rand is None or nb == 1) else _RandSlice(rand, sl),
                                 stream=main if s == 0 else self._stream_for(dev, ('branch', s)),
                                 side=self._stream_for(dev, ('side', s)) if self.overlap_wgrad else None))
        rng.advance()
        jb['pen'].zero_()
        torch.cat((pos_items, pos_items), out=jb['target2'])
        zero_done = None
        if training:
            zs = self._stream_for(dev, ('zero',))
            zs.wait_stream(main)
            with torch.cuda.stream(zs):
                opt.zero_grad()
                jb['d_out2'].zero_()
                for br in branches:
                    bb = br['buf']
                    if self._sharded():
                        self._shard_buffers(bb, dev)['d_xrows'].zero_()
                    bb['d_ctx'].zero_()
                    bb['d_x'].zero_()
                    for l, layer in enumerate(m.trm_encoder.layer):
                        if layer.combine_option == 'gate':
                            bb['layers'][l]['d_gl'].zero_()
            zero_done = torch.cuda.Event()
            zero_done.record(zs)
        for br in branches:
            if br['stream'] is not main:
                br['stream'].wait_stream(main)
            with torch.cuda.stream(br['stream']):
                self._forward_branch(br, jb, B, L, rt, training)
        for br in branches:
            if br['stream'] is not main:
                main.wait_stream(br['stream'])
        if getattr(self, '_stop_after', None) == 'fwd':
            if zero_done is not None:
                main.wait_event(zero_done)
            return jb['loss'][0], jb['loss'][0]
        st = _stream()
        passes = m.logits_passes
        vst = None
        if self.vp is not None:
            loss2, vst = self.vp.ce_forward(jb['out2'], E, jb['target2'], 2)
            jb['loss'].copy_(loss2)
        wp = m.mask_loss_weight.detach() if m.trainable_mask_loss_weight else None
        wv = 0.0 if wp is not None else float(m.mask_loss_weight)
        bpr = m.loss_type == 'BPR'
        if bpr:
            if self.vp is not None:
                raise NotImplementedError('vocab-parallel logits are a CE construct; loss_type BPR touches two table rows per sequence')
            neg_items = interaction[m.NEG_ITEM_ID]
            torch.cat((neg_items, neg_items), out=jb['neg2'])
            LIB.call('acsr_bpr_loss_fwd', _p(jb['out2']), _p(E), _p(jb['target2'], torch.int64), _p(jb['neg2'], torch.int64), 2 * B, d, 2,
                     float(m.loss_fct.gamma), _p(jb['row_x']), _p(jb['row_loss']), _p(jb['loss']), st)
            LIB.call('acsr_loss_combine', jb['pen'].data_ptr(), N, _p(jb['loss'][1:]), _p(wp), wv, _p(jb['loss_att']), _p(jb['dpen']), st)
        elif self.vp is None:
            LIB.call('acsr_logits_ce_partial', _p(jb['out2']), _p(E), 2 * B, V, d, passes, _p(jb['partial']), st)
            LIB.call('acsr_ce_finalize_losses', _p(jb['partial']), jb['partial'].shape[1], _p(jb['out2']), _p(E),
                     _p(jb['target2'], torch.int64), 2 * B, d, V, 0, 2, _p(jb['lse']), _p(jb['tgt']), _p(jb['row_loss']),
                     _p(jb['loss']), jb['pen'].data_ptr(), N, _p(wp), wv, _p(jb['loss_att']), _p(jb['dpen']),
                     jb['ce_cnt'].data_ptr(), st)
        else:
            LIB.call('acsr_loss_combine', jb['pen'].data_ptr(), N, _p(jb['loss'][1:]), _p(wp), wv, _p(jb['loss_att']), _p(jb['dpen']), st)
        loss_cal = jb['loss'][0]
        loss_att = jb['loss_att'][0]
        self.last_losses = jb['loss3']
        if not training or getattr(self, '_stop_after', None) == 'ce':
            if zero_done is not None:
                main.wait_event(zero_done)
            return loss_att, loss_cal
        dpen = jb['dpen']
        main.wait_event(zero_done)
        if bpr:
            LIB.call('acsr_bpr_loss_bwd', _p(jb['out2']), _p(E), _p(jb['target2'], torch.int64), _p(jb['neg2'], torch.int64),
                     _p(jb['row_x']), _p(jb['row_scale']), 2 * B, d, float(m.loss_fct.gamma), 0, B, _p(jb['d_out2']), _p(E.grad), st)
        elif self.vp is not None:
            jb['d_out2'].copy_(self.vp.ce_backward(vst, E, jb['row_scale'], E.grad, table_half=0, n_groups=2))
        elif self.ce_fused_bwd:
            ops.ce_bwd_dout(jb['out2'], E, jb['lse'], jb['target2'], jb['row_scale'], jb['d_out2'], passes)
        else:
            if jb['Gt'] is None:
                jb['Gt'] = torch.empty((V, 2 * B), dtype=torch.float32, device=dev)
            LIB.call('acsr_logits_ce_grad', _p(jb['out2']), _p(E), _p(jb['lse']), _p(jb['target2'], torch.int64),
                     _p(jb['row_scale']), 2 * B, V, d, passes, _p(jb['Gt']), 2 * B, st)
            ops.gemm_batch([ops.wgrad_problem(jb['Gt'], E, V, 2 * B, d, jb['d_out2'])])
        for br in branches:
            if br['stream'] is not main:
                br['stream'].wait_stream(main)
        if self.vp is None and not bpr:
            dE_stream = branches[0]['side'] if (nb == 1 and branches[0]['side'] is not None) else main
            if dE_stream is not main:
                dE_stream.wait_stream(main)
            with torch.cuda.stream(dE_stream):
                if self.ce_fused_bwd:
                    ops.ce_bwd_dtable(jb['out2'][:B], E, jb['lse'][:B], jb['target2'][:B], jb['row_scale'][:B], E.grad, passes)
                else:
                    ops.gemm_batch([ops.gemm_problem(jb['Gt'], jb['out2'], E.grad, V, d, B, a_strides=(2 * B, 1, 0, B),
                                                     b_strides=(1, d, 0, B), accumulate=True)])
        else:
            dE_stream = main
        dE_done = torch.cuda.Event()
        dE_done.record(dE_stream)
        for br in branches:
            with torch.cuda.stream(br['stream']):
                self._backward_branch(br, jb, B, L, rt, dpen, dE_done)
        for br in branches:
            if br['stream'] is not main:
                main.wait_stream(br['stream'])
        return loss_att, loss_cal

    def _forward_branch(self, br, jb, B, L, rt, training, need_att=True):
        m = self.m
        b, seq, ln, s = br['buf'], br['seq'], br['ln'], br['idx']
        Bs = seq.shape[0]
        T, d, I, N, V, H = b['T'], m.hidden_size, m.inner_size, m.n_layers, m.n_items, m.n_heads
        dh = d // H
        rng, rand = rt.rng, br['rand']
        rngp = rng.ptr
        st = _stream()
        p_h = m.dropout.p if training else 0.0
        soff = 4096 * s

        def mask(key):
            return None if (rand is None or p_h == 0.0) else rand.get(key)

        def mask2(l, k_cal, k_att, last):
            if rand is None or p_h == 0.0:
                return None
            a = rand.get((l, k_cal))
            return torch.cat((a.reshape(T, d), rand.get((l, k_att)).reshape(T, d))) if last else a

        E = m.item_embedding.weight
        posw = m.position_embedding.weight if m.use_position_embedding else None
        b['me'] = mask('emb')
        cur = torch.cuda.current_stream()
        so = self._stream_for(seq.device, ('order', s))
        so.wait_stream(cur)
        folded = {}
        if self.tc:
            for l in range(N):
                st3 = self._stacked(l)
                if st3 is None:
                    continue
                fw = self._folded_buffers(l, seq.device)
                LIB.call('acsr_fold_attack_weights', _p(st3['Wqkv']), _p(st3['bqkv']), _p(st3['Waqk']), _p(st3['baqk']), d,
                         _p(fw['W']), _p(fw['b']), so.cuda_stream)
                fw['done'] = torch.cuda.Event()
                fw['done'].record(so)
                folded[l] = fw
        bwd_ops = {}
        if self.dense_bwd and training:
            for l in range(N - 1):
                lay = m.trm_encoder.layer[l]
                dbuf = self._dense_bwd_ops_buffer(l, s, seq.device)
                LIB.call('acsr_dense_bwd_prep', _p(lay.attack_attention.dense.weight), _p(lay.feed_forward.dense_1.weight),
                         _p(lay.feed_forward.dense_2.weight), d, I, _p(dbuf), so.cuda_stream)
                bwd_ops[l] = dbuf
        b['dense_bwd_ops'] = bwd_ops
        LIB.call('acsr_seq_order', _p(seq, torch.int64), Bs, L, _p(b['order'], torch.int32), so.cuda_stream)
        order_done = torch.cuda.Event()
        order_done.record(so)
        if self._sharded():
            sb = self._shard_buffers(b, seq.device)
            _, b['ids_all'] = self.vp.fetch_rows(seq.reshape(-1), E, out=sb['xrows'][1:])
            LIB.call('acsr_embed_ln_dropout_fwd', _p(sb['iota1'], torch.int64), _p(sb['xrows']), _p(posw), _p(m.LayerNorm.weight),
                     _p(m.LayerNorm.bias), m.LayerNorm.eps, T, L, d, T + 1, p_h, _p(b['me']), rngp, soff + 1, _p(b['x0']), _p(b['st_e']), st)
        else:
            LIB.call('acsr_embed_ln_dropout_fwd', _p(seq, torch.int64), _p(E), _p(posw), _p(m.LayerNorm.weight), _p(m.LayerNorm.bias),
                     m.LayerNorm.eps, T, L, d, V, p_h, _p(b['me']), rngp, soff + 1, _p(b['x0']), _p(b['st_e']), st)
        x = b['x0']
        b['xs'] = []
        act_id = ops.ACT_IDS[m.hidden_act]
        for l, layer in enumerate(m.trm_encoder.layer):
            last = l == N - 1 and need_att
            lb = b['layers'][l]
            aa, ff = layer.attack_attention, layer.feed_forward
            base = soff + 16 * (l + 1)
            b['xs'].append(x)
            fw = folded.get(l)
            if fw is not None:
                cur.wait_event(fw['done'])
                ops.linear_tok(x, T, d, fw['W'], d, lb['qkv5'], d, bias=fw['b'], batch=5, sx=0, sw=d * d, sb=d, sy=T * d)
            else:
                gp = ops.gemm_problem
                ops.gemm_batch([gp(x, lin.weight, lb[k], T, d, d, bias=lin.bias)
                                for lin, k in ((aa.query, 'mq'), (aa.key, 'mk'), (aa.value, 'mv'))], passes=self.passes)
                second = [gp(lb['mq'], aa.attack_query_transform.weight, lb['aq'], T, d, d, bias=aa.attack_query_transform.bias),
                          gp(lb['mk'], aa.attack_key_transform.weight, lb['ak'], T, d, d, bias=aa.attack_key_transform.bias)]
                if layer.combine_option == 'gate' and not self.tc:
                    if layer.gate.out_features != L:
                        raise ValueError('gate width %d != sequence length %d' % (layer.gate.out_features, L))
                    second.append(gp(lb['mq'], layer.gate.weight, lb['gl'], T, L, d, bias=layer.gate.bias))
                ops.gemm_batch(second, passes=self.passes)
            gate = layer.combine_option == 'gate'
            comb_scalar = 0.0
            if gate:
                if layer.gate.out_features != L:
                    raise ValueError('gate width %d != sequence length %d' % (layer.gate.out_features, L))
                if self.tc:
                    ops.linear_tok(lb['mq'], T, d, layer.gate.weight, L, lb['gl'], L, bias=layer.gate.bias)
            elif layer.combine_option == 'annealing':
                comb_scalar = math.exp(-layer.anneal_step / 100000)
                if s == 0:
                    layer.anneal_step += 1
            p_attn = aa.attn_dropout.p if training else 0.0
            lb['attn_args'] = self._attn_args(layer, lb, seq, Bs, L, H, dh, comb_scalar, p_attn, rand, l, rngp, base)
            ctx_cal, ctx_att = lb['ctx'][:T], (lb['ctx'][T:] if last else None)
            if l == 0:
                cur.wait_event(order_done)
            LIB.call('acsr_attn_calib_fwd', *lb['attn_args'], _p(ctx_att), _p(ctx_cal),
                     jb['pen'][l:].data_ptr() if need_att else None, None, _p(b['order'], torch.int32),
                     _p(ln, torch.int64) if l == N - 1 else None, st)
            m_a, m_f = mask2(l, 'D5', 'D4', last), mask2(l, 'D7', 'D6', last)
            if l == N - 1:
                cb = b['c']
                C = 2 * Bs if need_att else Bs
                if m_a is not None or m_f is not None:
                    idx = torch.arange(Bs, device=seq.device) * L + ln - 1
                    rows = torch.cat((idx, T + idx)) if need_att else idx
                    m_a = None if m_a is None else m_a.reshape(-1, d)[rows].contiguous()
                    m_f = None if m_f is None else m_f.reshape(-1, d)[rows].contiguous()
                cb['m_a'], cb['m_f'] = m_a, m_f
                out_buf = jb['out2'] if Bs == B else cb['out']
                if self.tail_fused:
                    LIB.call('acsr_tail_fwd', _p(lb['ctx'][:T]), _p(lb['ctx'][T:]) if need_att else None, _p(x), _p(ln, torch.int64),
                             Bs, L, d, I, act_id, _p(aa.dense.weight), _p(aa.dense.bias), _p(aa.LayerNorm.weight), _p(aa.LayerNorm.bias),
                             aa.LayerNorm.eps, _p(ff.dense_1.weight), _p(ff.dense_1.bias), _p(ff.dense_2.weight), _p(ff.dense_2.bias),
                             _p(ff.LayerNorm.weight), _p(ff.LayerNorm.bias), ff.LayerNorm.eps, p_h, _p(m_a), _p(m_f), rngp, base + 3,
                             base + 5, _p(cb['ctx']), _p(cb['x']), _p(cb['hz']), _p(cb['st_a']), _p(cb['h']), _p(cb['z1']), _p(cb['a1']),
                             _p(cb['z2']), _p(cb['st_f']), _p(out_buf), st)
                else:
                    LIB.call('acsr_gather_last_fwd', _p(lb['ctx'][:T]) if need_att else None, _p(lb['ctx'][T:] if need_att else lb['ctx'][:T]),
                             _p(ln, torch.int64), Bs, L, d, _p(cb['ctx']), st)
                    LIB.call('acsr_gather_last_fwd', None, _p(x), _p(ln, torch.int64), Bs, L, d, _p(cb['x']), st)
                    self._post_attn_fwd(layer, cb, cb['x'], Bs, C, out_buf, p_h, rngp, base, act_id, st)
                if Bs != B:
                    lo = br['sl'].start
                    jb['out2'][lo:lo + Bs].copy_(cb['out'][:Bs])
                    if need_att:
                        jb['out2'][B + lo:B + lo + Bs].copy_(cb['out'][Bs:C])
                return
            lb['m_a'], lb['m_f'] = m_a, m_f
            self._post_attn_fwd(layer, lb, x, T, T, lb['out'], p_h, rngp, base, act_id, st)
            x = lb['out']

    def _post_attn_fwd(self, layer, bf, x_res, res_rows, R, out, p_h, rngp, base, act_id, st):
        m = self.m
        d, I = m.hidden_size, m.inner_size
        aa, ff = layer.attack_attention, layer.feed_forward
        if self.tc:
            ops.linear_tok_bdrl(bf['ctx'], R, d, aa.dense.weight, aa.dense.bias, x_res, res_rows, aa.LayerNorm.weight,
                                aa.LayerNorm.bias, aa.LayerNorm.eps, p_h, bf['m_a'], rngp, base + 3, bf['hz'], bf['h'], bf['st_a'])
            ops.linear_tok(bf['h'], R, d, ff.dense_1.weight, I, bf['z1'], I)
            LIB.call('acsr_bias_act_fwd', _p(bf['z1']), _p(ff.dense_1.bias), R, I, act_id, _p(bf['a1']), st)
            ops.linear_tok_bdrl(bf['a1'], R, I, ff.dense_2.weight, ff.dense_2.bias, bf['h'], R, ff.LayerNorm.weight,
                                ff.LayerNorm.bias, ff.LayerNorm.eps, p_h, bf['m_f'], rngp, base + 5, bf['z2'], out, bf['st_f'])
        else:
            gp, ps = ops.gemm_problem, self.passes
            ops.gemm_batch([gp(bf['ctx'], aa.dense.weight, bf['hz'], R, d, d, bias=aa.dense.bias, epilogue=ops.EPI_BDRL, res=x_res,
                               res_rows=res_rows, ln_w=aa.LayerNorm.weight, ln_b=aa.LayerNorm.bias, eps=aa.LayerNorm.eps, p_drop=p_h,
                               mask=bf['m_a'], rngp=rngp, rng_stream=base + 3, out=bf['h'], stats=bf['st_a'])], passes=ps)
            ops.gemm_batch([gp(bf['h'], ff.dense_1.weight, bf['z1'], R, I, d, bias=ff.dense_1.bias, epilogue=ops.EPI_ACT, act=act_id,
                               C2=bf['a1'])], passes=ps)
            ops.gemm_batch([gp(bf['a1'], ff.dense_2.weight, bf['z2'], R, d, I, bias=ff.dense_2.bias, epilogue=ops.EPI_BDRL, res=bf['h'],
                               res_rows=R, ln_w=ff.LayerNorm.weight, ln_b=ff.LayerNorm.bias, eps=ff.LayerNorm.eps, p_drop=p_h,
                               mask=bf['m_f'], rngp=rngp, rng_stream=base + 5, out=out, stats=bf['st_f'])], passes=ps)

    @torch.no_grad()
    def encode_eval(self, item_seq, item_seq_len):
        m = self.m
        seq, ln = item_seq.contiguous(), item_seq_len.contiguous()
        B, L = seq.shape
        dev = seq.device
        rt = m._runtime(dev)
        jb = self._joint_buffers(B, dev)
        br = dict(idx=0, sl=slice(0, B), seq=seq, ln=ln, buf=self._branch_buffers(B, L, dev, 'eval', grads=False), rand=rt.rand,
                  stream=torch.cuda.current_stream(), side=None)
        jb['pen'].zero_()
        self._forward_branch(br, jb, B, L, rt, False, need_att=False)
        return jb['out2'][:B]

    def _backward_branch(self, br, jb, B, L, rt, dpen, dE_done):
        m = self.m
        b, seq, ln, s = br['buf'], br['seq'], br['ln'], br['idx']
        Bs = seq.shape[0]
        T, d, I, N, V = b['T'], m.hidden_size, m.inner_size, m.n_layers, m.n_items
        rngp = rt.rng.ptr
        st = _stream()
        main = torch.cuda.current_stream()
        side = br['side']
        p_h = m.dropout.p
        soff = 4096 * s
        act_id = ops.ACT_IDS[m.hidden_act]
        E = m.item_embedding.weight
        posw = m.position_embedding.weight if m.use_position_embedding else None

        def fork():
            if side is None:
                return st
            side.wait_stream(main)
            return side.cuda_stream

        d_out, d_x = b['d_out'], b['d_x']
        lo = br['sl'].start
        T2 = 2 * T
        for l in reversed(range(N)):
            last = l == N - 1
            lb = b['layers'][l]
            layer = m.trm_encoder.layer[l]
            aa, ff = layer.attack_attention, layer.feed_forward
            base = soff + 16 * (l + 1)
            x = b['xs'][l]
            gate = layer.combine_option == 'gate'
            wg = []
            if last:
                cb = b['c']
                C = 2 * Bs
                if Bs == B:
                    dc_out = jb['d_out2']
                else:
                    dc_out = cb['d_out']
                    dc_out[:Bs].copy_(jb['d_out2'][lo:lo + Bs])
                    dc_out[Bs:].copy_(jb['d_out2'][B + lo:B + lo + Bs])
                if self.tail_fused:
                    g = lambda t: _p(t.grad)
                    LIB.call('acsr_tail_bwd', _p(dc_out), _p(ln, torch.int64), Bs, L, d, I, act_id, 2, _p(cb['x']), _p(cb['hz']),
                             _p(cb['st_a']), _p(cb['h']), _p(cb['z1']), _p(cb['z2']), _p(cb['st_f']), _p(aa.dense.weight), _p(aa.dense.bias),
                             _p(aa.LayerNorm.weight), _p(ff.dense_1.weight), _p(ff.dense_1.bias), _p(ff.dense_2.weight),
                             _p(ff.dense_2.bias), _p(ff.LayerNorm.weight), p_h, _p(cb['m_a']), _p(cb['m_f']), rngp, base + 3, base + 5,
                             _p(cb['d_z2']), _p(cb['d_z1']), _p(cb['d_hz']), _p(d_x[:T]), _p(d_x[T:]), _p(b['d_ctx'][:T]),
                             _p(b['d_ctx'][T:]), g(aa.dense.bias), g(aa.LayerNorm.weight), g(aa.LayerNorm.bias), g(ff.dense_1.bias),
                             g(ff.dense_2.bias), g(ff.LayerNorm.weight), g(ff.LayerNorm.bias), st)
                    self._wgrad(cb['d_z2'], cb['a1'], Bs, ff.dense_2.weight.grad, None, wg)
                    self._wgrad(cb['d_z1'], cb['h'], Bs, ff.dense_1.weight.grad, None, wg)
                    self._wgrad(cb['d_hz'], cb['ctx'], Bs, aa.dense.weight.grad, None, wg)
                else:
                    self._post_attn_bwd(layer, cb, cb, dc_out, cb['x'], C, C, Bs, Bs, cb['d_x'], cb['d_ctx'], p_h, rngp, base, act_id, st, wg)
                    LIB.call('acsr_gather_last_bwd', _p(cb['d_ctx']), _p(ln, torch.int64), Bs, L, d, _p(b['d_ctx'][:T]), _p(b['d_ctx'][T:]), st)
                    LIB.call('acsr_gather_last_bwd', _p(cb['d_x']), _p(ln, torch.int64), Bs, L, d, _p(d_x[:T]), _p(d_x[T:]), st)
            else:
                self._post_attn_bwd(layer, lb, lb, d_out, x, T2, T, T, T, d_x, b['d_ctx'], p_h, rngp, base, act_id, st, wg, b=b,
                                    dops=b['dense_bwd_ops'].get(l))
            if wg and l == 0:
                ops.gemm_batch(wg, passes=self.passes, stream=fork())
                wg = []
            g = lambda t: None if t is None else t.grad
            ow, ob_ = (aa.order_affine.weight, aa.order_affine.bias) if aa.use_order else (None, None)
            dw, db_, sc = (aa.distance_affine.weight, aa.distance_affine.bias, aa.scalar) if aa.use_distance else (None, None, None)
            rr = getattr(layer, 'rich_calibrated_combine_ratio', None) if not layer.two_level else None
            dc = b['d_ctx']
            d_att1, d_cal1 = (dc[T:], None) if last else (None, dc[T:])
            ops.attn_workspace(Bs, L, m.n_heads, 2, seq.device)
            LIB.call('acsr_attn_calib_bwd2', _p(dc[:T]), None, _p(d_att1), _p(d_cal1), _p(dpen[l:l + 1]), *lb['attn_args'],
                     _p(lb['d_mq']), _p(lb['d_mk']), _p(lb['d_mv']), _p(lb['d_aq']), _p(lb['d_ak']),
                     _p(lb['d_gl']) if gate else None, _p(g(ow)), _p(g(ob_)), _p(g(dw)), _p(g(db_)), _p(g(sc)), _p(g(rr)),
                     _p(b['order'], torch.int32), _p(ln, torch.int64) if last else None, st)
            aqt, akt = aa.attack_query_transform, aa.attack_key_transform
            self._wgrad(lb['d_aq'][T:], lb['mq'], T, aqt.weight.grad, aqt.bias.grad, wg)
            self._wgrad(lb['d_ak'][T:], lb['mk'], T, akt.weight.grad, akt.bias.grad, wg)
            if gate:
                self._wgrad(lb['d_gl'], lb['mq'], T, layer.gate.weight.grad, layer.gate.bias.grad, wg)

            st3 = self._stacked(l)
            gp = ops.gemm_problem
            rows_x = T2 if l > 0 else T
            if self.tc and st3 is not None and (not gate or L <= d):
                LIB.call('acsr_proj_input_grad', _p(lb['d_qkv']), _p(lb['d_aqk']), T2, _p(lb['d_gl']) if gate else None, L,
                         _p(st3['Wqkv']), _p(st3['Waqk']), _p(layer.gate.weight) if gate else None, d, rows_x, T, _p(d_x),
                         self.passes, st)
            else:
                ops.gemm_batch([gp(lb['d_aq'], aqt.weight, lb['d_mq'], T2, d, d, b_strides=(1, d, 0, d), accumulate=True),
                                gp(lb['d_ak'], akt.weight, lb['d_mk'], T2, d, d, b_strides=(1, d, 0, d), accumulate=True)],
                               passes=self.passes)
                if gate:
                    ops.gemm_batch([gp(lb['d_gl'], layer.gate.weight, lb['d_mq'], T2, d, L, b_strides=(1, d, 0, L), accumulate=True)],
                                   passes=self.passes)
                if st3 is not None:
                    ops.gemm_batch([gp(lb['d_qkv'], st3['Wqkv'], d_x, rows_x, d, 3 * d, a_strides=(d, 1, T2 * d, d),
                                       b_strides=(1, d, d * d, d), accumulate=True)], passes=self.passes)
                else:
                    for lin, dk in ((aa.query, 'd_mq'), (aa.key, 'd_mk'), (aa.value, 'd_mv')):
                        ops.gemm_batch([gp(lb[dk], lin.weight, d_x, rows_x, d, d, b_strides=(1, d, 0, d), accumulate=True)],
                                       passes=self.passes)
            for lin, dk in ((aa.query, 'd_mq'), (aa.key, 'd_mk'), (aa.value, 'd_mv')):
                self._wgrad(lb[dk], x, T, lin.weight.grad, lin.bias.grad, wg)
            if wg:
                ops.gemm_batch(wg, passes=self.passes, stream=fork())
            if l > 0:
                d_out, d_x = d_x, d_out
        main.wait_event(dE_done)
        if self._sharded():
            sb = self._shard_buffers(b, seq.device)
            LIB.call('acsr_embed_ln_dropout_bwd', _p(d_x[:T]), _p(sb['iota1'], torch.int64), _p(sb['xrows']), _p(posw), _p(m.LayerNorm.weight),
                     _p(b['st_e']), T, L, d, T + 1, p_h, _p(b['me']), rngp, soff + 1, _p(sb['d_xrows']),
                     _p(posw.grad if posw is not None else None), _p(m.LayerNorm.weight.grad), _p(m.LayerNorm.bias.grad), st)
            self.vp.scatter_grad_rows(b['ids_all'], sb['d_xrows'][1:], E.grad)
        else:
            LIB.call('acsr_embed_ln_dropout_bwd', _p(d_x[:T]), _p(seq, torch.int64), _p(E), _p(posw), _p(m.LayerNorm.weight),
                     _p(b['st_e']), T, L, d, V, p_h, _p(b['me']), rngp, soff + 1, _p(E.grad), _p(posw.grad if posw is not None else None),
                     _p(m.LayerNorm.weight.grad), _p(m.LayerNorm.bias.grad), st)
        if side is not None:
            main.wait_stream(side)

    def _post_attn_bwd(self, layer, bf, gb, d_out, x_res, R2, P, res_rows, w_rows, d_xres, d_ctx, p_h, rngp, base, act_id, st, wg, b=None,
                       dops=None):
        m = self.m
        d, I = m.hidden_size, m.inner_size
        aa, ff = layer.attack_attention, layer.feed_forward
        if dops is not None:
            LIB.call('acsr_dense_bwd', _p(d_out), R2, P, res_rows, w_rows, d, I, act_id, _p(dops), _p(bf['z2']), _p(ff.dense_2.bias),
                     _p(bf['h']), _p(ff.LayerNorm.weight), _p(bf['st_f']), _p(bf['z1']), _p(ff.dense_1.bias), _p(bf['hz']),
                     _p(aa.dense.bias), _p(x_res), _p(aa.LayerNorm.weight), _p(bf['st_a']), p_h, _p(bf['m_a']), _p(bf['m_f']), rngp,
                     base + 3, base + 5, _p(gb['d_z2']), _p(gb['d_z1']), _p(gb['d_hz']), _p(d_xres), _p(d_ctx),
                     _p(ff.LayerNorm.weight.grad), _p(ff.LayerNorm.bias.grad), _p(aa.LayerNorm.weight.grad),
                     _p(aa.LayerNorm.bias.grad), self.passes, st)
            self._wgrad(gb['d_z2'], bf['a1'], w_rows, ff.dense_2.weight.grad, ff.dense_2.bias.grad, wg)
            self._wgrad(gb['d_z1'], bf['h'], w_rows, ff.dense_1.weight.grad, ff.dense_1.bias.grad, wg)
            self._wgrad(gb['d_hz'], bf['ctx'], w_rows, aa.dense.weight.grad, aa.dense.bias.grad, wg)
            return
        d_h = gb['d_h'] if b is None else b['d_h']
        d_a1 = gb['d_a1'] if b is None else b['d_a1']
        gp, ps = ops.gemm_problem, self.passes
        LIB.call('acsr_bias_dropout_res_ln_bwd', _p(d_out), _p(bf['z2']), _p(ff.dense_2.bias), _p(bf['h']),
                 _p(ff.LayerNorm.weight), _p(bf['st_f']), R2, d, P, P, w_rows, p_h, _p(bf['m_f']), rngp, base + 5,
                 _p(gb['d_z2']), _p(d_h), _p(ff.dense_2.bias.grad), _p(ff.LayerNorm.weight.grad),
                 _p(ff.LayerNorm.bias.grad), st)
        self._wgrad(gb['d_z2'], bf['a1'], w_rows, ff.dense_2.weight.grad, None, wg)
        if self.tc:
            ops.linear_tok(gb['d_z2'], R2, d, ff.dense_2.weight, I, d_a1, I, w_sn=1, w_sk=I, wkb=64 * I)
        else:
            ops.gemm_batch([gp(gb['d_z2'], ff.dense_2.weight, d_a1, R2, I, d, b_strides=(1, I, 0, d))], passes=ps)
        LIB.call('acsr_bias_act_bwd', _p(d_a1), _p(bf['z1']), _p(ff.dense_1.bias), R2, I, act_id, P, w_rows, _p(gb['d_z1']),
                 _p(ff.dense_1.bias.grad), st)
        self._wgrad(gb['d_z1'], bf['h'], w_rows, ff.dense_1.weight.grad, None, wg)
        if self.tc:
            ops.linear_tok(gb['d_z1'], R2, I, ff.dense_1.weight, d, d_h, d, w_sn=1, w_sk=d, wkb=64 * d, accumulate=True)
        else:
            ops.gemm_batch([gp(gb['d_z1'], ff.dense_1.weight, d_h, R2, d, I, b_strides=(1, d, 0, I), accumulate=True)], passes=ps)
        LIB.call('acsr_bias_dropout_res_ln_bwd', _p(d_h), _p(bf['hz']), _p(aa.dense.bias), _p(x_res),
                 _p(aa.LayerNorm.weight), _p(bf['st_a']), R2, d, P, res_rows, w_rows, p_h, _p(bf['m_a']), rngp, base + 3,
                 _p(gb['d_hz']), _p(d_xres), _p(aa.dense.bias.grad), _p(aa.LayerNorm.weight.grad), _p(aa.LayerNorm.bias.grad), st)
        self._wgrad(gb['d_hz'], bf['ctx'], w_rows, aa.dense.weight.grad, None, wg)
        if self.tc:
            ops.linear_tok(gb['d_hz'], R2, d, aa.dense.weight, d, d_ctx, d, w_sn=1, w_sk=d, wkb=64 * d)
        else:
            ops.gemm_batch([gp(gb['d_hz'], aa.dense.weight, d_ctx, R2, d, d, b_strides=(1, d, 0, d))], passes=ps)

    @staticmethod
    def _wgrad(dY, X, rows, dW, db, wg):
        wg.append(ops.wgrad_problem(dY, X, rows, dY.shape[-1], X.shape[-1], dW, db))

    def _sharded(self):
        return self.vp is not None and self.vp.sharded

    def _shard_buffers(self, b, dev):
        if 'shard' not in b:
            T, d = b['T'], self.m.hidden_size
            b['shard'] = dict(xrows=torch.zeros((T + 1, d), dtype=torch.float32, device=dev),
                              d_xrows=torch.zeros((T + 1, d), dtype=torch.float32, device=dev),
                              iota1=torch.arange(1, T + 1, dtype=torch.int64, device=dev))
        return b['shard']

    def _folded_buffers(self, l, dev):
        key = ('folded', l)
        if key not in self.buf:
            d = self.m.hidden_size
            self.buf[key] = dict(W=torch.zeros((5, d, d), dtype=torch.float32, device=dev), b=torch.zeros((5, 1, d), dtype=torch.float32, device=dev))
            for t in list(self.buf[key].values()):
                LIB.query('acsr_register_static', t.data_ptr(), t.numel() * 4)
        return self.buf[key]

    def _dense_bwd_ops_buffer(self, l, s, dev):
        key = ('dense_bwd_ops', l, s)
        if key not in self.buf:
            t = torch.empty(LIB.query('acsr_dense_bwd_prep_floats', int(self.m.inner_size)), dtype=torch.float32, device=dev)
            LIB.query('acsr_register_static', t.data_ptr(), t.numel() * 4)
            self.buf[key] = t
        return self.buf[key]

    def _stacked(self, l):
        if not hasattr(self, '_st'):
            self._st = {}
        if l not in self._st:
            aa = self.m.trm_encoder.layer[l].attack_attention
            opt = self.opt
            if not hasattr(opt, 'stacked'):
                self._st[l] = None
            else:
                qkv_w, qkv_b = [aa.query.weight, aa.key.weight, aa.value.weight], [aa.query.bias, aa.key.bias, aa.value.bias]
                aqk_w = [aa.attack_query_transform.weight, aa.attack_key_transform.weight]
                aqk_b = [aa.attack_query_transform.bias, aa.attack_key_transform.bias]
                v = dict(Wqkv=opt.stacked(qkv_w), bqkv=opt.stacked(qkv_b), Waqk=opt.stacked(aqk_w), baqk=opt.stacked(aqk_b),
                         gWqkv=opt.stacked(qkv_w, True), gbqkv=opt.stacked(qkv_b, True), gWaqk=opt.stacked(aqk_w, True),
                         gbaqk=opt.stacked(aqk_b, True))
                if any(t is None for t in v.values()):
                    self._st[l] = None
                else:
                    v['bqkv'] = v['bqkv'].unsqueeze(1)
                    v['baqk'] = v['baqk'].unsqueeze(1)
                    self._st[l] = v
        return self._st[l]

    @staticmethod
    def _attn_args(layer, lb, seq, B, L, H, dh, comb_scalar, p_attn, rand, l, rngp, base):
        aa = layer.attack_attention
        r = (lambda k: None) if (rand is None) else (lambda k: rand.get((l, k)))
        drop = p_attn > 0.0
        D1, D2, D3 = (r('D1'), r('D2'), r('D3')) if drop else (None, None, None)
        lb['_keep'] = (D1, D2, D3, r('noise'))
        two_level = int(bool(layer.two_level))
        rich = ops.RICH_IDS.get(layer.rich_calibrated_combine, 0) if not layer.two_level else 0
        rr = getattr(layer, 'rich_calibrated_combine_ratio', None) if not layer.two_level else None
        return (_p(lb['mq']), _p(lb['mk']), _p(lb['mv']), _p(lb['aq']), _p(lb['ak']),
                _p(lb['gl']) if layer.combine_option == 'gate' else None, _p(seq, torch.int64),
                _p(aa.order_affine.weight) if aa.use_order else None, _p(aa.order_affine.bias) if aa.use_order else None,
                _p(aa.distance_affine.weight) if aa.use_distance else None, _p(aa.distance_affine.bias) if aa.use_distance else None,
                _p(aa.scalar) if aa.use_distance else None,
                B, L, H, dh, two_level, ops.COMBINE_IDS[layer.combine_option], float(comb_scalar), rich, _p(rr),
                float(p_attn), _p(D1), _p(D2), _p(D3), _p(lb['_keep'][3]), rngp, base)
```

### ac-tsr_b200/ops.py

```python
import numpy as np
import torch

from ._lib import LIB, AcsrError

ACT_IDS = {'gelu': 0, 'relu': 1, 'swish': 2, 'tanh': 3, 'sigmoid': 4}
COMBINE_IDS = {'gate': 0, 'fixed': 1, 'annealing': 2}
RICH_IDS = {'none': 0, 'fixed': 1, 'trainable': 2}


def _p(t, dtype=torch.float32):
    if t is None:
        return None
    if not t.is_cuda:
        raise AcsrError('AC-SASRec hot path needs CUDA tensors (got %s); there is no CPU fallback' % t.device)
    if t.dtype != dtype:
        raise AcsrError('expected dtype %s, got %s' % (dtype, t.dtype))
    if not t.is_contiguous():
        raise AcsrError('tensor must be contiguous')
    return t.data_ptr()


def _stream():
    return torch.cuda.current_stream().cuda_stream


def _c(t):
    return None if t is None else t.contiguous()


def _wants_grad(t):
    return t is not None and (t.requires_grad or not t.is_leaf)


_DIRECT_GRAD = [False]


class direct_param_grads:

    def __enter__(self):
        self.prev = _DIRECT_GRAD[0]
        _DIRECT_GRAD[0] = True

    def __exit__(self, *a):
        _DIRECT_GRAD[0] = self.prev


def _grad_sink(t):
    if _DIRECT_GRAD[0] and t is not None and t.is_leaf and t.requires_grad and t.grad is not None and t.grad.is_contiguous():
        return t.grad
    return None


def _param_grad_buffers(params):
    bufs, rets, need = [None] * len(params), [None] * len(params), []
    for i, t in enumerate(params):
        if t is None or not _wants_grad(t):
            continue
        sink = _grad_sink(t)
        if sink is not None:
            bufs[i] = sink
        else:
            need.append(i)
    if need:
        sizes = [(params[i].numel() + 3) // 4 * 4 for i in need]
        block = torch.zeros(sum(sizes), dtype=torch.float32, device=params[need[0]].device)
        off = 0
        for i, n in zip(need, sizes):
            bufs[i] = rets[i] = block[off:off + params[i].numel()].view(params[i].shape)
            off += n
    return bufs, rets


class DeviceRng:

    def __init__(self, seed, device):
        self.state = torch.tensor([int(seed) & 0x7fffffffffffffff, 0], dtype=torch.int64, device=device)

    @property
    def ptr(self):
        return self.state.data_ptr()

    def advance(self):
        LIB.call('acsr_rng_advance', self.ptr, _stream())


class EmbedLnDropoutFn(torch.autograd.Function):
    @staticmethod
    def forward(ctx, item_seq, table, pos_emb, ln_w, ln_b, eps, p, mask, rng, rng_stream):
        B, L = item_seq.shape
        V, d = table.shape
        item_seq = item_seq.contiguous()
        out = torch.empty((B, L, d), dtype=torch.float32, device=table.device)
        stats = torch.empty((B * L, 2), dtype=torch.float32, device=table.device)
        mask = _c(mask)
        LIB.call('acsr_embed_ln_dropout_fwd', _p(item_seq, torch.int64), _p(table), _p(pos_emb), _p(ln_w), _p(ln_b),
                 eps, B * L, L, d, V, p, _p(mask), rng.ptr if rng is not None else None, rng_stream,
                 _p(out), _p(stats), _stream())
        ctx.save_for_backward(item_seq, table, pos_emb, ln_w, stats, mask)
        ctx.meta = (B, L, d, V, p, rng, rng_stream)
        return out

    @staticmethod
    def backward(ctx, d_out):
        item_seq, table, pos_emb, ln_w, stats, mask = ctx.saved_tensors
        B, L, d, V, p, rng, rng_stream = ctx.meta
        if not (_wants_grad(table) or _wants_grad(pos_emb) or _wants_grad(ln_w)):
            return None, None, None, None, None, None, None, None, None, None
        d_out = d_out.contiguous()
        d_table = torch.zeros_like(table)
        d_pos = torch.zeros_like(pos_emb) if pos_emb is not None else None
        d_w = torch.zeros_like(ln_w)
        d_b = torch.zeros_like(ln_w)
        LIB.call('acsr_embed_ln_dropout_bwd', _p(d_out), _p(item_seq, torch.int64), _p(table), _p(pos_emb), _p(ln_w),
                 _p(stats), B * L, L, d, V, p, _p(mask), rng.ptr if rng is not None else None, rng_stream,
                 _p(d_table), _p(d_pos), _p(d_w), _p(d_b), _stream())
        return None, d_table, d_pos, d_w, d_b, None, None, None, None, None


class BiasDropoutResLnFn(torch.autograd.Function):

    @staticmethod
    def forward(ctx, h, bias, res, ln_w, ln_b, eps, p, mask, rng, rng_stream):
        h, res, mask = h.contiguous(), res.contiguous(), _c(mask)
        d = h.shape[-1]
        T = h.numel() // d
        out = torch.empty_like(h)
        stats = torch.empty((T, 2), dtype=torch.float32, device=h.device)
        LIB.call('acsr_bias_dropout_res_ln_fwd', _p(h), _p(bias), _p(res), _p(ln_w), _p(ln_b), eps, T, d, T, p, _p(mask),
                 rng.ptr if rng is not None else None, rng_stream, _p(out), _p(stats), _stream())
        ctx.save_for_backward(h, bias, res, ln_w, stats, mask)
        ctx.meta = (T, d, p, rng, rng_stream)
        ctx.ln_b_ref = ln_b
        return out

    @staticmethod
    def backward(ctx, d_out):
        h, bias, res, ln_w, stats, mask = ctx.saved_tensors
        T, d, p, rng, rng_stream = ctx.meta
        d_out = d_out.contiguous()
        d_h = torch.empty_like(h)
        d_res = torch.empty_like(h)
        (b_bias, b_w, b_b), (d_bias, d_w, d_b) = _param_grad_buffers([bias, ln_w, ctx.ln_b_ref])
        LIB.call('acsr_bias_dropout_res_ln_bwd', _p(d_out), _p(h), _p(bias), _p(res), _p(ln_w), _p(stats), T, d, T, T, T, p,
                 _p(mask), rng.ptr if rng is not None else None, rng_stream, _p(d_h), _p(d_res), _p(b_bias), _p(b_w),
                 _p(b_b), _stream())
        return d_h, d_bias, d_res, d_w, d_b, None, None, None, None, None


class BiasActFn(torch.autograd.Function):

    @staticmethod
    def forward(ctx, h, bias, act):
        h = h.contiguous()
        n = h.shape[-1]
        T = h.numel() // n
        out = torch.empty_like(h)
        LIB.call('acsr_bias_act_fwd', _p(h), _p(bias), T, n, act, _p(out), _stream())
        ctx.save_for_backward(h, bias)
        ctx.meta = (T, n, act)
        return out

    @staticmethod
    def backward(ctx, d_out):
        h, bias = ctx.saved_tensors
        T, n, act = ctx.meta
        d_out = d_out.contiguous()
        d_h = torch.empty_like(h)
        (b_bias,), (d_bias,) = _param_grad_buffers([bias])
        LIB.call('acsr_bias_act_bwd', _p(d_out), _p(h), _p(bias), T, n, act, T, T, _p(d_h), _p(b_bias), _stream())
        return d_h, d_bias, None


class GatherLastFn(torch.autograd.Function):

    @staticmethod
    def forward(ctx, x_att, x_cal, item_len):
        B, L, d = x_cal.shape
        x_cal = x_cal.contiguous()
        x_att = _c(x_att)
        item_len = item_len.contiguous()
        rows = 2 * B if x_att is not None else B
        out = torch.empty((rows, d), dtype=torch.float32, device=x_cal.device)
        LIB.call('acsr_gather_last_fwd', _p(x_att), _p(x_cal), _p(item_len, torch.int64), B, L, d, _p(out), _stream())
        ctx.save_for_backward(item_len)
        ctx.meta = (B, L, d, x_att is not None)
        return out

    @staticmethod
    def backward(ctx, d_out):
        (item_len,) = ctx.saved_tensors
        B, L, d, has_att = ctx.meta
        d_out = d_out.contiguous()
        d_cal = torch.zeros((B, L, d), dtype=torch.float32, device=d_out.device)
        d_att = torch.zeros_like(d_cal) if has_att else None
        LIB.call('acsr_gather_last_bwd', _p(d_out), _p(item_len, torch.int64), B, L, d, _p(d_att), _p(d_cal), _stream())
        return d_att, d_cal, None


def attn_workspace(B, L, H, n_streams, device):
    if L <= 64:
        return
    import os
    per_seq = LIB.query('acsr_attn_workspace_bytes', int(L), int(H), int(n_streams))
    cap = int(os.environ.get('ACSR_WORKSPACE_MB', 4096)) << 20
    LIB.ensure_workspace(max(per_seq, min(B * per_seq, cap)), device)


class AttnOpts:

    def __init__(self, n_heads, two_level, combine_option, rich_mode, p_attn, bidirectional=False, plain=False):
        self.n_heads = n_heads
        self.two_level = int(bool(two_level)) | (2 if bidirectional else 0) | (4 if plain else 0)
        self.combine = COMBINE_IDS[combine_option]
        self.rich = RICH_IDS.get(rich_mode, 0)
        self.p_attn = float(p_attn)


class AttnCalibFn(torch.autograd.Function):

    @staticmethod
    def forward(ctx, mq, mk, mv, aq, ak, gate_logit, key_ids, order_w, order_b, dist_w, dist_b, scalar, rich_ratio,
                opts, comb_scalar, p_attn, rand, rng, rng_stream, need_att, want_probs):
        B, L, d = mq.shape
        H = opts.n_heads
        dh = d // H
        ctx.set_materialize_grads(False)
        mq, mk, mv, aq, ak = (t.contiguous() for t in (mq, mk, mv, aq, ak))
        gate_logit = _c(gate_logit)
        key_ids = key_ids.contiguous()
        D1, D2, D3, noise = (_c(rand.get(k)) if rand else None for k in ('D1', 'D2', 'D3', 'noise'))
        dev = mq.device
        ctx_cal = torch.empty((B, L, d), dtype=torch.float32, device=dev)
        ctx_att = torch.empty_like(ctx_cal) if need_att else None
        pen = torch.zeros(1, dtype=torch.float64, device=dev)
        probs = torch.empty((6, B, H, L, L), dtype=torch.float32, device=dev) if want_probs else None
        rngp = rng.ptr if rng is not None else None
        LIB.call('acsr_attn_calib_fwd', _p(mq), _p(mk), _p(mv), _p(aq), _p(ak), _p(gate_logit), _p(key_ids, torch.int64),
                 _p(order_w), _p(order_b), _p(dist_w), _p(dist_b), _p(scalar), B, L, H, dh,
                 opts.two_level, opts.combine, float(comb_scalar), opts.rich, _p(rich_ratio),
                 p_attn, _p(D1), _p(D2), _p(D3), _p(noise), rngp, rng_stream,
                 _p(ctx_att), _p(ctx_cal), pen.data_ptr(), _p(probs), None, None, _stream())
        ctx.save_for_backward(mq, mk, mv, aq, ak, gate_logit, key_ids, order_w, order_b, dist_w, dist_b, scalar, rich_ratio,
                              D1, D2, D3, noise)
        ctx.meta = (B, L, H, dh, opts, float(comb_scalar), p_attn, rng, rng_stream, need_att)
        pen32 = pen.to(torch.float32)
        ctx.mark_non_differentiable(*([probs] if probs is not None else []))
        return ctx_att, ctx_cal, pen32, probs

    @staticmethod
    def backward(ctx, d_att, d_cal, d_pen, _d_probs):
        (mq, mk, mv, aq, ak, gate_logit, key_ids, order_w, order_b, dist_w, dist_b, scalar, rich_ratio,
         D1, D2, D3, noise) = ctx.saved_tensors
        B, L, H, dh, opts, comb_scalar, p_attn, rng, rng_stream, need_att = ctx.meta
        d_att = _c(d_att) if need_att else None
        d_cal = _c(d_cal)
        d_pen = _c(d_pen)
        z = torch.zeros_like
        d_mq, d_mk, d_mv, d_aq, d_ak = (torch.empty_like(mq) for _ in range(5))
        d_gate = z(gate_logit) if gate_logit is not None else None
        (b_ow, b_ob, b_dw, b_db, b_sc, b_rr), (d_ow, d_ob, d_dw, d_db, d_sc, d_rr) = _param_grad_buffers(
            [order_w, order_b, dist_w, dist_b, scalar, rich_ratio])
        attn_workspace(B, L, H, 1, mq.device)
        LIB.call('acsr_attn_calib_bwd', _p(d_att), _p(d_cal), _p(d_pen), _p(mq), _p(mk), _p(mv), _p(aq), _p(ak),
                 _p(gate_logit), _p(key_ids, torch.int64), _p(order_w), _p(order_b), _p(dist_w), _p(dist_b), _p(scalar),
                 B, L, H, dh, opts.two_level, opts.combine, comb_scalar, opts.rich, _p(rich_ratio),
                 p_attn, _p(D1), _p(D2), _p(D3), _p(noise), rng.ptr if rng is not None else None, rng_stream,
                 _p(d_mq), _p(d_mk), _p(d_mv), _p(d_aq), _p(d_ak), _p(d_gate), _p(b_ow), _p(b_ob), _p(b_dw), _p(b_db),
                 _p(b_sc), _p(b_rr), None, None, _stream())
        return (d_mq, d_mk, d_mv, d_aq, d_ak, d_gate, None, d_ow, d_ob, d_dw, d_db, d_sc, d_rr,
                None, None, None, None, None, None, None, None)


def time_matrix(time_seq, time_span):
    ts = time_seq.to(torch.float32).contiguous()
    B, L = ts.shape
    out = torch.empty((B, L, L), dtype=torch.int32, device=ts.device)
    LIB.call('acsr_time_matrix', _p(ts), B, L, int(time_span), _p(out, torch.int32), _stream())
    return out


class PairSpec:

    def __init__(self, tmat, n_heads, p, Dp=None, Dt=None, rng=None, stream_p=0, stream_t=0):
        self.tmat, self.H, self.p = tmat.contiguous(), int(n_heads), float(p)
        self.Dp, self.Dt = _c(Dp), _c(Dt)
        self.rng, self.stream_p, self.stream_t = rng, int(stream_p), int(stream_t)

    def args(self, B, L, d, span1):
        return (_p(self.tmat, torch.int32), B, L, self.H, d // self.H, span1, self.p, _p(self.Dp), _p(self.Dt),
                self.rng.ptr if (self.rng is not None and self.p > 0) else None, self.stream_p, self.stream_t)


def _pair_score(x, P, T, spec, causal):
    B, L, d = x.shape
    out = torch.empty((B, spec.H, L, L), dtype=torch.float32, device=x.device)
    a = spec.args(B, L, d, T.shape[0])
    LIB.call('acsr_pair_score', _p(x), _p(P), _p(T), *a, int(causal), _p(out), _stream())
    return out


def _pair_context(prob, P, T, spec, d):
    B, H, L, _ = prob.shape
    y = torch.empty((B, L, d), dtype=torch.float32, device=prob.device)
    a = spec.args(B, L, d, T.shape[0])
    LIB.call('acsr_pair_context', _p(prob), _p(P), _p(T), *a, 0, _p(y), _stream())
    return y


def _pair_wgrad(a_mat, v, P, T, spec):
    B, L, d = v.shape
    dP, dT = torch.zeros_like(P), torch.zeros_like(T)
    a = spec.args(B, L, d, T.shape[0])
    LIB.call('acsr_pair_wgrad', _p(a_mat), _p(v), a[0], *a[1:], _p(dP), _p(dT), _stream())
    return dP, dT


class PairScoreFn(torch.autograd.Function):

    @staticmethod
    def forward(ctx, x, P, T, spec, causal):
        x, P, T = x.contiguous(), P.contiguous(), T.contiguous()
        ctx.save_for_backward(x, P, T)
        ctx.spec, ctx.causal = spec, bool(causal)
        return _pair_score(x, P, T, spec, causal)

    @staticmethod
    def backward(ctx, ds):
        x, P, T = ctx.saved_tensors
        ds = (torch.tril(ds) if ctx.causal else ds).contiguous()
        dx = _pair_context(ds, P, T, ctx.spec, x.shape[-1]) if ctx.needs_input_grad[0] else None
        dP = dT = None
        if (ctx.needs_input_grad[1] and _wants_grad(P)) or (ctx.needs_input_grad[2] and _wants_grad(T)):
            dP, dT = _pair_wgrad(ds, x, P, T, ctx.spec)
        return dx, dP, dT, None, None


class PairContextFn(torch.autograd.Function):

    @staticmethod
    def forward(ctx, prob, P, T, spec):
        prob, P, T = prob.contiguous(), P.contiguous(), T.contiguous()
        ctx.save_for_backward(prob, P, T)
        ctx.spec = spec
        return _pair_context(prob, P, T, spec, P.shape[1])

    @staticmethod
    def backward(ctx, dy):
        prob, P, T = ctx.saved_tensors
        dy = dy.contiguous()
        dprob = _pair_score(dy, P, T, ctx.spec, 0) if ctx.needs_input_grad[0] else None
        dP = dT = None
        if (ctx.needs_input_grad[1] and _wants_grad(P)) or (ctx.needs_input_grad[2] and _wants_grad(T)):
            dP, dT = _pair_wgrad(prob, dy, P, T, ctx.spec)
        return dprob, dP, dT, None


class AttnCalibTiFn(torch.autograd.Function):

    @staticmethod
    def forward(ctx, s_bias, mq, mk, mv, aq, ak, gate_logit, key_ids, order_w, order_b, dist_w, dist_b, scalar, rich_ratio,
                opts, comb_scalar, p_attn, rand, rng, rng_stream, need_att):
        B, L, d = mq.shape
        H = opts.n_heads
        dh = d // H
        ctx.set_materialize_grads(False)
        s_bias, mq, mk, mv, aq, ak = (t.contiguous() for t in (s_bias, mq, mk, mv, aq, ak))
        gate_logit = _c(gate_logit)
        key_ids = key_ids.contiguous()
        D1, D2, D3, noise = (_c(rand.get(k)) if rand else None for k in ('D1', 'D2', 'D3', 'noise'))
        dev = mq.device
        ctx_cal = torch.empty((B, L, d), dtype=torch.float32, device=dev)
        ctx_att = torch.empty_like(ctx_cal) if need_att else None
        prob_cal = (torch.empty if need_att else torch.zeros)((B, H, L, L), dtype=torch.float32, device=dev)
        prob_att = torch.empty_like(prob_cal) if need_att else None
        pen = torch.zeros(1, dtype=torch.float64, device=dev)
        LIB.call('acsr_attn_calib_ti_fwd', _p(s_bias), _p(mq), _p(mk), _p(mv), _p(aq), _p(ak), _p(gate_logit),
                 _p(key_ids, torch.int64), _p(order_w), _p(order_b), _p(dist_w), _p(dist_b), _p(scalar), B, L, H, dh,
                 opts.two_level, opts.combine, float(comb_scalar), opts.rich, _p(rich_ratio),
                 p_attn, _p(D1), _p(D2), _p(D3), _p(noise), rng.ptr if rng is not None else None, rng_stream,
                 _p(ctx_att), _p(ctx_cal), pen.data_ptr(), _p(prob_att), _p(prob_cal), _stream())
        ctx.save_for_backward(s_bias, mq, mk, mv, aq, ak, gate_logit, key_ids, order_w, order_b, dist_w, dist_b, scalar,
                              rich_ratio, D1, D2, D3, noise)
        ctx.meta = (B, L, H, dh, opts, float(comb_scalar), p_attn, rng, rng_stream, need_att)
        return ctx_att, ctx_cal, pen.to(torch.float32), prob_att, prob_cal

    @staticmethod
    def backward(ctx, d_att, d_cal, d_pen, d_pa, d_pc):
        (s_bias, mq, mk, mv, aq, ak, gate_logit, key_ids, order_w, order_b, dist_w, dist_b, scalar, rich_ratio,
         D1, D2, D3, noise) = ctx.saved_tensors
        B, L, H, dh, opts, comb_scalar, p_attn, rng, rng_stream, need_att = ctx.meta
        d_att = _c(d_att) if need_att else None
        d_pa = _c(d_pa) if need_att else None
        d_cal, d_pen, d_pc = _c(d_cal), _c(d_pen), _c(d_pc)
        z = torch.zeros_like
        d_mq, d_mk, d_mv, d_aq, d_ak = (torch.empty_like(mq) for _ in range(5))
        d_gate = z(gate_logit) if gate_logit is not None else None
        (b_ow, b_ob, b_dw, b_db, b_sc, b_rr), (d_ow, d_ob, d_dw, d_db, d_sc, d_rr) = _param_grad_buffers(
            [order_w, order_b, dist_w, dist_b, scalar, rich_ratio])
        d_sb = z(s_bias)
        LIB.call('acsr_attn_calib_ti_bwd', _p(d_att), _p(d_cal), _p(d_pen), _p(d_pa), _p(d_pc), _p(s_bias), _p(mq), _p(mk),
                 _p(mv), _p(aq), _p(ak), _p(gate_logit), _p(key_ids, torch.int64), _p(order_w), _p(order_b), _p(dist_w),
                 _p(dist_b), _p(scalar), B, L, H, dh, opts.two_level, opts.combine, comb_scalar, opts.rich, _p(rich_ratio),
                 p_attn, _p(D1), _p(D2), _p(D3), _p(noise), rng.ptr if rng is not None else None, rng_stream,
                 _p(d_mq), _p(d_mk), _p(d_mv), _p(d_aq), _p(d_ak), _p(d_gate), _p(b_ow), _p(b_ob), _p(b_dw), _p(b_db),
                 _p(b_sc), _p(b_rr), _p(d_sb), _stream())
        return (d_sb, d_mq, d_mk, d_mv, d_aq, d_ak, d_gate, None, d_ow, d_ob, d_dw, d_db, d_sc, d_rr,
                None, None, None, None, None, None, None)


def logits_num_chunks(M, V, d=64):
    return LIB.query('acsr_logits_num_chunks_d', int(M), int(V), int(d))


def ce_partial(out, table, passes=3):
    M, d = out.shape
    V = table.shape[0]
    part = torch.empty((M, logits_num_chunks(M, V, d), 2), dtype=torch.float32, device=out.device)
    LIB.call('acsr_logits_ce_partial', _p(out), _p(table), M, V, d, passes, _p(part), _stream())
    return part


def ce_finalize(partial, out, table, target, n_groups, idx_offset=0):
    M, d = out.shape
    dev = out.device
    lse = torch.empty(M, dtype=torch.float32, device=dev)
    tgt = torch.empty_like(lse)
    row_loss = torch.empty_like(lse)
    loss = torch.empty(n_groups, dtype=torch.float32, device=dev)
    LIB.call('acsr_ce_finalize', _p(partial), partial.shape[1], _p(out), _p(table), _p(target, torch.int64), M, d,
             table.shape[0], idx_offset, n_groups, _p(lse), _p(tgt), _p(row_loss), _p(loss), _stream())
    return lse, tgt, row_loss, loss


def ce_grad_matrix_t(out, table, lse, target, row_scale, passes=3):
    M, d = out.shape
    V = table.shape[0]
    Gt = torch.empty((V, M), dtype=torch.float32, device=out.device)
    LIB.call('acsr_logits_ce_grad', _p(out), _p(table), _p(lse), _p(target, torch.int64), _p(row_scale), M, V, d, passes,
             _p(Gt), M, _stream())
    return Gt


def ce_bwd_dout(out, table, lse, target, row_scale, d_out, passes=3):
    M, d = out.shape
    LIB.call('acsr_ce_bwd_dout', _p(out), _p(table), _p(lse), _p(target, torch.int64), _p(row_scale), M, table.shape[0], d, passes,
             _p(d_out), _stream())
    return d_out


def ce_bwd_dtable(out, table, lse, target, row_scale, d_table, passes=3, stream=None):
    M, d = out.shape
    LIB.call('acsr_ce_bwd_dtable', _p(out), _p(table), _p(lse), _p(target, torch.int64), _p(row_scale), M, table.shape[0], d, passes,
             _p(d_table), _stream() if stream is None else stream)
    return d_table


def linear_wgrad(dY, X, dW=None, db=None, want_bias=True):
    N, K = dY.shape[-1], X.shape[-1]
    dY2, X2 = dY.reshape(-1, N), X.reshape(-1, K)
    if not dY2.is_contiguous():
        dY2 = dY2.contiguous()
    if not X2.is_contiguous():
        X2 = X2.contiguous()
    if dW is None:
        dW = torch.zeros((N, K), dtype=torch.float32, device=dY.device)
    if db is None and want_bias:
        db = torch.zeros(N, dtype=torch.float32, device=dY.device)
    LIB.call('acsr_linear_wgrad', _p(dY2), _p(X2), dY2.shape[0], N, K, _p(dW), _p(db), _stream())
    return dW, db


def linear_tc(X, rows, W, N, w_sn, w_sk, bias, Y, ldy, accumulate=False, batch=1, sx=0, sw=0, sb=0, sy=0, passes=3):
    LIB.call('acsr_linear_tc', _p(X), int(rows), 64, _p(W), int(N), int(w_sn), int(w_sk), _p(bias), int(bool(accumulate)),
             _p(Y), int(ldy), int(batch), int(sx), int(sw), int(sb), int(sy), passes, _stream())


def linear_tok(X, rows, K, W, N, Y, ldy, ldx=None, xkb=64, w_sn=None, w_sk=1, wkb=64, bias=None, accumulate=False,
               batch=1, sx=0, sw=0, sb=0, sy=0, passes=3):
    LIB.call('acsr_linear_tok', _p(X), int(K if ldx is None else ldx), int(xkb), int(rows), int(K), _p(W),
             int(K if w_sn is None else w_sn), int(w_sk), int(wkb), int(N), _p(bias), int(bool(accumulate)), _p(Y), int(ldy),
             int(batch), int(sx), int(sw), int(sb), int(sy), passes, _stream())


def linear_tok_bdrl(X, rows, K, W, bias, res, res_rows, ln_w, ln_b, eps, p, mask, rngp, rng_stream, HZ, out, stats, passes=3):
    LIB.call('acsr_linear_tok_bdrl', _p(X), int(K), int(rows), int(K), _p(W), _p(bias), _p(res), int(res_rows), _p(ln_w), _p(ln_b),
             float(eps), float(p), _p(mask), rngp, int(rng_stream), _p(HZ), _p(out), _p(stats), passes, _stream())


def _linear_grad_buffers(weight, bias):
    sw, sb = _grad_sink(weight), (_grad_sink(bias) if bias is not None else None)
    if sw is not None and (bias is None or sb is not None):
        return (sw, sb), (None, None)
    dW = torch.zeros(weight.shape, dtype=torch.float32, device=weight.device)
    db = torch.zeros(bias.shape, dtype=torch.float32, device=weight.device) if bias is not None else None
    return (dW, db), (dW, db)


class LinearFn(torch.autograd.Function):

    @staticmethod
    def forward(ctx, x, weight, bias):
        ctx.save_for_backward(x, weight)
        ctx.has_bias = bias is not None
        ctx.bias_ref = bias
        N, K = weight.shape
        x2 = x.reshape(-1, K)
        if not x2.is_contiguous():
            x2 = x2.contiguous()
        w = weight if weight.is_contiguous() else weight.contiguous()
        y = torch.empty((x2.shape[0], N), dtype=torch.float32, device=x.device)
        gemm_batch([gemm_problem(x2, w, y, x2.shape[0], N, K, bias=bias)])
        return y.view(*x.shape[:-1], N)

    @staticmethod
    def backward(ctx, dy):
        x, weight = ctx.saved_tensors
        N, K = weight.shape
        dy2 = dy.reshape(-1, N)
        if not dy2.is_contiguous():
            dy2 = dy2.contiguous()
        rows = dy2.shape[0]
        dx = dW = db = None
        if ctx.needs_input_grad[0]:
            w = weight if weight.is_contiguous() else weight.contiguous()
            dx = torch.empty((rows, K), dtype=torch.float32, device=dy.device)
            gemm_batch([gemm_problem(dy2, w, dx, rows, K, N, b_strides=(1, K, 0, N))])
            dx = dx.view_as(x)
        if (ctx.needs_input_grad[1] and _wants_grad(weight)) or (ctx.has_bias and ctx.needs_input_grad[2] and _wants_grad(ctx.bias_ref)):
            x2 = x.reshape(-1, K)
            if not x2.is_contiguous():
                x2 = x2.contiguous()
            (bW, bb), (dW, db) = _linear_grad_buffers(weight, ctx.bias_ref)
            gemm_batch([wgrad_problem(dy2, x2, rows, N, K, bW, bb)])
        return dx, dW, db


def linear(x, weight, bias=None):
    return LinearFn.apply(x, weight, bias)


class MultiLinearFn(torch.autograd.Function):

    @staticmethod
    def forward(ctx, n, *args):
# ... 470 lines not shown
```

### include/acsr.h

```cpp
#ifndef ACSR_H_
#define ACSR_H_
#include <stdint.h>

#ifdef __cplusplus
extern "C" {
#endif

#define ACSR_ABI_VERSION 1
#define ACSR_OK 0
#define ACSR_ERR_ARG (-1)
#define ACSR_ERR_UNSUPPORTED (-2)
#define ACSR_ERR_CUDA (-3)

int acsr_version(void);
const char* acsr_last_error(void);
int acsr_num_sms(void);
int acsr_set_pdl(int on);

int acsr_register_static(const void* ptr, int64_t bytes);

int acsr_set_workspace(void* ptr, int64_t bytes);
int64_t acsr_attn_workspace_bytes(int L, int H, int n_streams);

int acsr_rng_advance(void* rng, void* stream);

int acsr_embed_ln_dropout_fwd(const int64_t* item_seq, const float* table, const float* pos_emb,
                              const float* ln_w, const float* ln_b, float eps,
                              int T, int L, int d, int64_t V,
                              float p, const float* mask, const void* rng, uint32_t rng_stream,
                              float* out, float* stats, void* stream);
int acsr_embed_ln_dropout_bwd(const float* d_out, const int64_t* item_seq, const float* table, const float* pos_emb,
                              const float* ln_w, const float* stats,
                              int T, int L, int d, int64_t V,
                              float p, const float* mask, const void* rng, uint32_t rng_stream,
                              float* d_table, float* d_pos, float* d_ln_w, float* d_ln_b, void* stream);

int acsr_seq_order(const int64_t* item_seq, int B, int L, int32_t* order, void* stream);
#define ACSR_ATTN_TWO_LEVEL 1
#define ACSR_ATTN_BIDIRECTIONAL 2
#define ACSR_ATTN_PLAIN 4
#define ACSR_ATTN_COMBINE_GATE 0
#define ACSR_ATTN_COMBINE_FIXED 1
#define ACSR_ATTN_COMBINE_ANNEAL 2
#define ACSR_ATTN_RICH_NONE 0
#define ACSR_ATTN_RICH_FIXED 1
#define ACSR_ATTN_RICH_TRAINABLE 2
int acsr_attn_calib_fwd(const float* mq, const float* mk, const float* mv, const float* aq, const float* ak,
                        const float* gate_logit, const int64_t* item_seq,
                        const float* order_w, const float* order_b,
                        const float* dist_w, const float* dist_b, const float* scalar,
                        int B, int L, int H, int dh,
                        int two_level, int combine_option, float comb_scalar, int rich_mode, const float* rich_ratio,
                        float p_attn, const float* D1, const float* D2, const float* D3, const float* noise,
                        const void* rng, uint32_t rng_stream,
                        float* ctx_att, float* ctx_cal, double* pen_sq, float* probs_out,
                        const int32_t* order, const int64_t* ctx_rows, void* stream);
int acsr_attn_calib_bwd(const float* d_ctx_att, const float* d_ctx_cal, const float* d_pen_sq,
                        const float* mq, const float* mk, const float* mv, const float* aq, const float* ak,
                        const float* gate_logit, const int64_t* item_seq,
                        const float* order_w, const float* order_b,
                        const float* dist_w, const float* dist_b, const float* scalar,
                        int B, int L, int H, int dh,
                        int two_level, int combine_option, float comb_scalar, int rich_mode, const float* rich_ratio,
                        float p_attn, const float* D1, const float* D2, const float* D3, const float* noise,
                        const void* rng, uint32_t rng_stream,
                        float* d_mq, float* d_mk, float* d_mv, float* d_aq, float* d_ak,
                        float* d_gate_logit, float* d_order_w, float* d_order_b,
                        float* d_dist_w, float* d_dist_b, float* d_scalar, float* d_rich_ratio,
                        const int32_t* order, const int64_t* ctx_rows, void* stream);
int acsr_attn_calib_bwd2(const float* d_ctx_cal0, const float* d_pen_sq0,
                         const float* d_ctx_att1, const float* d_ctx_cal1, const float* d_pen_sq1,
                         const float* mq, const float* mk, const float* mv, const float* aq, const float* ak,
                         const float* gate_logit, const int64_t* item_seq,
                         const float* order_w, const float* order_b,
                         const float* dist_w, const float* dist_b, const float* scalar,
                         int B, int L, int H, int dh,
                         int two_level, int combine_option, float comb_scalar, int rich_mode, const float* rich_ratio,
                         float p_attn, const float* D1, const float* D2, const float* D3, const float* noise,
                         const void* rng, uint32_t rng_stream,
                         float* d_mq, float* d_mk, float* d_mv, float* d_aq, float* d_ak,
                         float* d_gate_logit, float* d_order_w, float* d_order_b,
                         float* d_dist_w, float* d_dist_b, float* d_scalar, float* d_rich_ratio,
                        const int32_t* order, const int64_t* ctx_rows, void* stream);

int acsr_bias_dropout_res_ln_fwd(const float* h, const float* bias, const float* res,
                                 const float* ln_w, const float* ln_b, float eps, int T, int d, int res_rows,
                                 float p, const float* mask, const void* rng, uint32_t rng_stream,
                                 float* out, float* stats, void* stream);
int acsr_bias_dropout_res_ln_bwd(const float* d_out, const float* h, const float* bias, const float* res,
                                 const float* ln_w, const float* stats, int T, int d,
                                 int act_rows, int res_rows, int param_rows,
                                 float p, const float* mask, const void* rng, uint32_t rng_stream,
                                 float* d_h, float* d_res, float* d_bias, float* d_ln_w, float* d_ln_b, void* stream);

int acsr_bias_act_fwd(const float* h, const float* bias, int T, int n, int act, float* out, void* stream);
int acsr_bias_act_bwd(const float* d_out, const float* h, const float* bias, int T, int n, int act,
                      int act_rows, int param_rows, float* d_h, float* d_bias, void* stream);

int acsr_gather_last_fwd(const float* x_att, const float* x_cal, const int64_t* item_len,
                         int B, int L, int d, float* out, void* stream);
int acsr_gather_last_bwd(const float* d_out, const int64_t* item_len, int B, int L, int d,
                         float* d_x_att, float* d_x_cal, void* stream);

int acsr_logits_num_chunks(int M, int64_t V);
int acsr_logits_num_chunks_d(int M, int64_t V, int d);
int acsr_logits_store(const float* out, const float* table, int M, int64_t V, int d, int passes,
                      float* scores, int64_t ldc, void* stream);
int acsr_logits_ce_partial(const float* out, const float* table, int M, int64_t V, int d, int passes,
                           float* partial, void* stream);
int acsr_ce_finalize(const float* partial, int n_parts, const float* out, const float* table,
                     const int64_t* target, int M, int d, int64_t V, int64_t idx_offset, int n_groups,
                     float* lse, float* tgt_logit, float* row_loss, float* loss, void* stream);
int acsr_loss_combine(const double* pen_sq, int n_layers, const float* ce_attacked, const float* mask_loss_weight,
                      float mask_loss_weight_value, float* loss_attacked, float* d_pen_sq, void* stream);
int acsr_ce_finalize_losses(const float* partial, int n_parts, const float* out, const float* table, const int64_t* target, int M, int d,
                            int64_t V, int64_t idx_offset, int n_groups, float* lse, float* tgt_logit, float* row_loss, float* loss,
                            const double* pen_sq, int n_layers, const float* mask_loss_weight, float mask_loss_weight_value,
                            float* loss_attacked, float* d_pen_sq, uint32_t* counter, void* stream);
int acsr_logits_ce_grad(const float* out, const float* table, const float* lse, const int64_t* target,
                        const float* row_scale, int M, int64_t V, int d, int passes,
                        float* Gt, int64_t ldg, void* stream);
int acsr_ce_bwd_dout(const float* out, const float* table, const float* lse, const int64_t* target, const float* row_scale, int M,
                     int64_t V, int d, int passes, float* d_out, void* stream);
int acsr_ce_bwd_dtable(const float* out, const float* table, const float* lse, const int64_t* target, const float* row_scale, int M,
                       int64_t V, int d, int passes, float* d_table, void* stream);
int acsr_logits_topk_partial(const float* out, const float* table, int M, int64_t V, int d, int passes,
                             int k, int64_t idx_offset, int skip_col0,
                             float* partial_val, int64_t* partial_idx, void* stream);
int acsr_logits_topk_partial_ws(const float* out, const float* table, int M, int64_t V, int d, int passes,
                                int k, int64_t idx_offset, int skip_col0,
                                float* partial_val, int64_t* partial_idx, int32_t* row_bound, void* stream);
int acsr_topk_merge(const float* partial_val, const int64_t* partial_idx, int M, int n_parts, int k,
                    const int64_t* positive, float* topk_val, int64_t* topk_idx, int32_t* rec_topk, void* stream);

int acsr_row_dot(const float* out, const float* table, const int64_t* ids, int M, int d, int64_t V, int64_t idx_offset, float* dot,
                 void* stream);
int acsr_logits_topk_rank_partial(const float* out, const float* table, int M, int64_t V, int d, int passes, int k, int64_t idx_offset,
                                  int skip_col0, const int64_t* positive, const float* pos_score, float* partial_val,
                                  int64_t* partial_idx, int32_t* partial_counts, int32_t* row_bound, void* stream);
int acsr_topk_merge_rank(const float* partial_val, const int64_t* partial_idx, int M, int n_parts, int k,
                         const int64_t* positive, const int32_t* partial_counts, int n_count_parts, float* topk_val,
                         int64_t* topk_idx, int32_t* rec_topk, int32_t* counts, void* stream);

int acsr_topk_select_max_items(void);
int acsr_topk_select(const float* scores, int M, int64_t V, int64_t ld, int k, int skip_col0, int64_t idx_offset,
                     const int64_t* positive, float* topk_val, int64_t* topk_idx, int32_t* rec_topk, void* stream);
int acsr_topk_select_rank(const float* scores, int M, int64_t V, int64_t ld, int k, int skip_col0, int64_t idx_offset,
                          const int64_t* positive, const float* pos_score, float* topk_val, int64_t* topk_idx, int32_t* rec_topk,
                          int32_t* counts, void* stream);

int acsr_fold_attack_weights(const float* Wqkv, const float* bqkv, const float* Waqk, const float* baqk, int d, float* out_W,
                             float* out_b, void* stream);

int acsr_linear_tok(const float* X, int64_t ldx, int64_t x_kblock_stride, int64_t rows, int K,
                    const float* W, int64_t w_stride_n, int64_t w_stride_k, int64_t w_kblock_stride, int N,
                    const float* bias, int accumulate, float* Y, int64_t ldy,
                    int batch, int64_t stride_x, int64_t stride_w, int64_t stride_bias, int64_t stride_y,
                    int passes, void* stream);
int acsr_linear_tok_bdrl(const float* X, int64_t ldx, int64_t rows, int K, const float* W, const float* bias,
                         const float* res, int64_t res_rows, const float* ln_w, const float* ln_b, float eps,
                         float p_drop, const float* mask, const void* rng, uint32_t rng_stream,
                         float* HZ, float* out, float* stats, int passes, void* stream);
int acsr_proj_input_grad(float* d_qkv, const float* d_aqk, int64_t plane_rows, const float* d_gl, int L, const float* Wqkv,
                         const float* Waqk, const float* Wg, int d, int64_t rows, int64_t rows_keep, float* d_x, int passes,
                         void* stream);

int acsr_linear_tc(const float* X, int64_t rows, int K, const float* W, int N, int64_t w_stride_n, int64_t w_stride_k,
                   const float* bias, int accumulate, float* Y, int64_t ldy, int batch, int64_t stride_x, int64_t stride_w,
                   int64_t stride_bias, int64_t stride_y, int passes, void* stream);

int acsr_linear_wgrad(const float* dY, const float* X, int T, int N, int K, float* dW, float* db, void* stream);
int acsr_linear_wgrad_batched(const float* dY, const float* X, int T, int N, int K, float* dW, float* db, int batch,
                              int64_t stride_dy, int64_t stride_x, int64_t stride_dw, int64_t stride_db, void* stream);

#define ACSR_EPI_STORE 0
#define ACSR_EPI_ATOMIC 1
#define ACSR_EPI_ACT 2
#define ACSR_EPI_BDRL 3
#define ACSR_EPI_CE 4
#define ACSR_EPI_CE_GRAD 5
#define ACSR_GEMM_MAX_PROBLEMS 16
typedef struct acsr_gemm_problem {
  const float* A; int64_t a_row_stride; int64_t a_k_stride; int64_t a_kb_stride;
  const float* B; int64_t b_row_stride; int64_t b_k_stride; int64_t b_kb_stride;
  float* C; int64_t ldc;
  int64_t M;
  const float* bias;
  float* colsum;
  float* C2;
  const float* res; int64_t res_rows;
  const float* ln_w; const float* ln_b;
  const float* mask; const void* rng;
  float* out; float* stats;
  int32_t a_kblk; int32_t b_kblk;
  int32_t N; int32_t K;
  int32_t epilogue; int32_t accumulate; int32_t k_splits; int32_t act;
  uint32_t rng_stream; float eps; float p_drop; int32_t reserved;
} acsr_gemm_problem;
int acsr_gemm_batch(const acsr_gemm_problem* problems, int n_problems, int passes, void* stream);
int acsr_gemm_ce_parts(int64_t V);

int acsr_tail_fwd(const float* ctx_first, const float* ctx_second, const float* x, const int64_t* item_len, int B, int L, int d, int I,
                  int act, const float* Wo, const float* bo, const float* lnA_w, const float* lnA_b, float epsA, const float* W1,
                  const float* b1, const float* W2, const float* b2, const float* lnF_w, const float* lnF_b, float epsF, float p_drop,
                  const float* mask_a, const float* mask_f, const void* rng, uint32_t stream_a, uint32_t stream_f, float* c_ctx,
                  float* c_x, float* hz, float* st_a, float* h, float* z1, float* a1, float* z2, float* st_f, float* out, void* stream);
int acsr_tail_bwd(const float* d_out, const int64_t* item_len, int B, int L, int d, int I, int act, int n_groups, const float* c_x,
                  const float* hz, const float* st_a, const float* h, const float* z1, const float* z2, const float* st_f,
                  const float* Wo, const float* bo, const float* lnA_w, const float* W1, const float* b1, const float* W2,
                  const float* b2, const float* lnF_w, float p_drop, const float* mask_a, const float* mask_f, const void* rng,
                  uint32_t stream_a, uint32_t stream_f, float* d_z2, float* d_z1, float* d_hz, float* d_x_first, float* d_x_second,
                  float* d_ctx_first, float* d_ctx_second, float* g_bo, float* g_lnA_w, float* g_lnA_b, float* g_b1, float* g_b2,
                  float* g_lnF_w, float* g_lnF_b, void* stream);

int64_t acsr_dense_bwd_prep_floats(int I);
int acsr_dense_bwd_prep(const float* Wo, const float* W1, const float* W2, int d, int I, float* ops, void* stream);
int acsr_dense_bwd(const float* d_out, int64_t rows, int64_t act_rows, int64_t res_rows, int64_t param_rows, int d, int I, int act,
                   const float* ops, const float* z2, const float* b2, const float* h, const float* lnF_w, const float* st_f,
                   const float* z1, const float* b1, const float* hz, const float* bo, const float* x_res, const float* lnA_w,
                   const float* st_a, float p_drop, const float* mask_a, const float* mask_f, const void* rng, uint32_t stream_a,
                   uint32_t stream_f, float* d_z2, float* d_z1, float* d_hz, float* d_xres, float* d_ctx, float* g_lnF_w,
                   float* g_lnF_b, float* g_lnA_w, float* g_lnA_b, int passes, void* stream);

int acsr_bpr_loss_fwd(const float* out, const float* table, const int64_t* pos_items, const int64_t* neg_items, int M, int d,
                      int n_groups, float gamma, float* row_x, float* row_loss, float* loss, void* stream);
int acsr_bpr_loss_bwd(const float* out, const float* table, const int64_t* pos_items, const int64_t* neg_items, const float* row_x,
                      const float* row_scale, int M, int d, float gamma, int table_row_begin, int table_row_end, float* d_out,
                      float* d_table, void* stream);

int acsr_shard_gather_rows(const int64_t* ids, int64_t n, const float* shard, int64_t row_lo, int64_t row_hi, int d, float* out,
                           void* stream);
int acsr_shard_scatter_add_rows(const int64_t* ids, int64_t n, const float* rows, int64_t row_lo, int64_t row_hi, int d,
                                float* shard_grad, void* stream);

int acsr_batch_gather(const int64_t* seqs, const int64_t* lens, const int64_t* targets, const int64_t* negs, const int64_t* perm,
                      const int64_t* cursor, int64_t n_rows, int B, int L, int64_t* out_packed, void* stream);
int acsr_cursor_advance(int64_t* cursor, void* stream);

int acsr_neg_sample(const int64_t* users, const int64_t* positives, const int64_t* perm, const int64_t* cursor, int64_t n_rows, int M,
                    int N, const int64_t* used_offsets, const int64_t* used_items, int64_t n_users, int64_t n_items,
                    const float* alias_prob, const int64_t* alias_idx, const void* rng, uint32_t rng_stream, int64_t* negs,
                    int64_t ld_negs, void* stream);
int acsr_candidate_rank_max_candidates(void);
int acsr_candidate_rank(const float* out, const float* table, int64_t V, int d, const int64_t* cand, int M, int n_cand, int kmax,
                        int32_t* rec, float* scores, void* stream);
int acsr_candidate_rank_counts(const float* out, const float* table, int64_t V, int d, const int64_t* cand, int M, int n_cand, int kmax,
                               int32_t* rec, float* scores, int32_t* counts, void* stream);

int acsr_adam_step(float* param, const float* grad, float* exp_avg, float* exp_avg_sq, int64_t n,
                   float lr, float beta1, float beta2, float eps, float weight_decay,
                   int64_t* step_count, void* stream);

int acsr_time_matrix(const float* time_seq, int B, int L, int time_span, int32_t* tmat, void* stream);
int acsr_pair_score(const float* x, const float* P, const float* T, const int32_t* tmat, int B, int L, int H, int dh, int span1,
                    float p, const float* Dp, const float* Dt, const void* rng, uint32_t stream_p, uint32_t stream_t, int causal,
                    float* s_out, void* stream);
int acsr_pair_context(const float* prob, const float* P, const float* T, const int32_t* tmat, int B, int L, int H, int dh, int span1,
                      float p, const float* Dp, const float* Dt, const void* rng, uint32_t stream_p, uint32_t stream_t,
                      int accumulate, float* y, void* stream);
int acsr_pair_wgrad(const float* a, const float* v, const int32_t* tmat, int B, int L, int H, int dh, int span1,
                    float p, const float* Dp, const float* Dt, const void* rng, uint32_t stream_p, uint32_t stream_t,
                    float* dP, float* dT, void* stream);
int acsr_attn_calib_ti_fwd(const float* s_bias, const float* mq, const float* mk, const float* mv, const float* aq,
                           const float* ak, const float* gate_logit, const int64_t* item_seq, const float* order_w,
                           const float* order_b, const float* dist_w, const float* dist_b, const float* scalar, int B,
                           int L, int H, int dh, int two_level, int combine_option, float comb_scalar, int rich_mode,
                           const float* rich_ratio, float p_attn, const float* D1, const float* D2, const float* D3,
                           const float* noise, const void* rng, uint32_t rng_stream, float* ctx_att, float* ctx_cal,
                           double* pen_sq, float* prob_att, float* prob_cal, void* stream);
int acsr_attn_calib_ti_bwd(const float* d_ctx_att, const float* d_ctx_cal, const float* d_pen_sq, const float* d_prob_att,
                           const float* d_prob_cal, const float* s_bias, const float* mq, const float* mk,
                           const float* mv, const float* aq, const float* ak, const float* gate_logit, const int64_t* item_seq,
                           const float* order_w, const float* order_b, const float* dist_w, const float* dist_b, const float* scalar,
                           int B, int L, int H, int dh, int two_level, int combine_option, float comb_scalar, int rich_mode,
                           const float* rich_ratio, float p_attn, const float* D1, const float* D2, const float* D3,
                           const float* noise, const void* rng, uint32_t rng_stream, float* d_mq, float* d_mk, float* d_mv,
                           float* d_aq, float* d_ak, float* d_gate_logit, float* d_order_w, float* d_order_b, float* d_dist_w,
                           float* d_dist_b, float* d_scalar, float* d_rich_ratio, float* d_s_bias, void* stream);

#ifdef __cplusplus
}
#endif
#endif
```

Baseline: 410,200.

## Save attention softmax state in forward and reload it in backward

The forward attention kernel now writes per-row probabilities, masks (with the dropout bit packed into the sign), combine weights and noise to a global state buffer during training. The backward kernel gains a SAVED variant that loads these values instead of recomputing the full row forward (QK dot products, softmaxes, logs). This trades recomputation for extra global-memory writes in forward, reads in backward, and a larger workspace. It only applies for L <= 64.

```diff
diff --git a/ac-tsr_b200/csrc/attn_bwd.cu b/ac-tsr_b200/csrc/attn_bwd.cu
--- a/ac-tsr_b200/csrc/attn_bwd.cu
+++ b/ac-tsr_b200/csrc/attn_bwd.cu
@@ -2,7 +2,7 @@
 
 namespace acsr {
 
-template <int DH, int G, int MAXNJ, int NS>
+template <int DH, int G, int MAXNJ, int NS, bool SAVED>
 __device__ __forceinline__ void bwd_body(const AttnParams& p, const AttnSmem& sm, const BwdSmem<NS>& bs, const RowConst& kc,
                                          const BwdFlags& f, const float* dpen, int b, int h, int nkey, int rstride, BwdAcc& acc) {
   constexpr int dhp = DH + 4;
@@ -33,7 +33,7 @@
       continue;
     }
 #define ACSR_BWD_ROW(NJV) \
-  bwd_row_iter<DH, G, NJV, NS>(p, sm, bs, kc, f, dpen, b, h, i, rowok, bound, grp, sub, rstride, wbuf, acc, accOq, accDq)
+  bwd_row_iter<DH, G, NJV, NS, false, SAVED>(p, sm, bs, kc, f, dpen, b, h, i, rowok, bound, grp, sub, rstride, wbuf, acc, accOq, accDq)
     if (MAXNJ == 1 || nj == 1) ACSR_BWD_ROW(1);
     else if (nj == 2) ACSR_BWD_ROW((MAXNJ >= 2 ? 2 : 1));
     else ACSR_BWD_ROW((MAXNJ >= 4 ? 4 : 1));
@@ -139,7 +139,7 @@
   }
 }
 
-template <int DH, int NS>
+template <int DH, int NS, bool SAVED>
 __global__ void __launch_bounds__(kAttnThreads, 2) attn_bwd_kernel(const AttnParams p) {
   pdl_launch_dependents();
   pdl_wait();
@@ -188,8 +188,8 @@
   BwdAcc acc;
   acc.s_ob = acc.s_db = acc.s_scalar = acc.s_ratio = 0.f;
 
-  if (nkey <= 8) bwd_body<DH, 8, 1, NS>(p, sm, bs, kc, f, dpen, b, h, nkey, 8, acc);
-  else bwd_body<DH, 16, 4, NS>(p, sm, bs, kc, f, dpen, b, h, nkey, LP, acc);
+  if (nkey <= 8) bwd_body<DH, 8, 1, NS, SAVED>(p, sm, bs, kc, f, dpen, b, h, nkey, 8, acc);
+  else bwd_body<DH, 16, 4, NS, SAVED>(p, sm, bs, kc, f, dpen, b, h, nkey, LP, acc);
   __syncthreads();
   if (nkey <= 8) bwd_cols<DH, 32, NS>(p, sm, bs, f, b, h, nkey);
   else bwd_cols<DH, 16, NS>(p, sm, bs, f, b, h, nkey);
@@ -231,22 +231,22 @@
   return f * sizeof(float);
 }
 
-template <int DH, int NS>
+template <int DH, int NS, bool SAVED>
 static int launch_bwd(const AttnParams& p, cudaStream_t st) {
   size_t smem = bwd_smem_bytes(p.L, DH, NS, p.full);
-  int rc = prep_kernel(attn_bwd_kernel<DH, NS>, smem, "attn_calib_bwd");
+  int rc = prep_kernel(attn_bwd_kernel<DH, NS, SAVED>, smem, "attn_calib_bwd");
   if (rc) return rc;
-  launch_pdl(attn_bwd_kernel<DH, NS>, dim3(p.B * p.H), dim3(kAttnThreads), smem, st, p);
+  launch_pdl(attn_bwd_kernel<DH, NS, SAVED>, dim3(p.B * p.H), dim3(kAttnThreads), smem, st, p);
   return check_launch("attn_calib_bwd");
 }
 
-template <int NS>
+template <int NS, bool SAVED = false>
 static int dispatch_bwd(const AttnParams& p, cudaStream_t st) {
   switch (p.dh) {
-    case 8: return launch_bwd<8, NS>(p, st);
-    case 16: return launch_bwd<16, NS>(p, st);
-    case 32: return launch_bwd<32, NS>(p, st);
-    case 64: return launch_bwd<64, NS>(p, st);
+    case 8: return launch_bwd<8, NS, SAVED>(p, st);
+    case 16: return launch_bwd<16, NS, SAVED>(p, st);
+    case 32: return launch_bwd<32, NS, SAVED>(p, st);
+    case 64: return launch_bwd<64, NS, SAVED>(p, st);
   }
   return ACSR_ERR_UNSUPPORTED;
 }
@@ -306,15 +306,16 @@
   return dispatch_bwd<1>(p, (cudaStream_t)stream);
 }
 
-int acsr_attn_calib_bwd2(const float* d_ctx_cal0, const float* d_pen_sq0, const float* d_ctx_att1, const float* d_ctx_cal1,
-                         const float* d_pen_sq1, const float* mq, const float* mk, const float* mv, const float* aq,
-                         const float* ak, const float* gate_logit, const int64_t* item_seq, const float* order_w,
-                         const float* order_b, const float* dist_w, const float* dist_b, const float* scalar, int B, int L, int H,
-                         int dh, int two_level, int combine_option, float comb_scalar, int rich_mode, const float* rich_ratio,
-                         float p_attn, const float* D1, const float* D2, const float* D3, const float* noise, const void* rng,
-                         uint32_t rng_stream, float* d_mq, float* d_mk, float* d_mv, float* d_aq, float* d_ak,
-                         float* d_gate_logit, float* d_order_w, float* d_order_b, float* d_dist_w, float* d_dist_b,
-                         float* d_scalar, float* d_rich_ratio, const int32_t* order, const int64_t* ctx_rows, void* stream) {
+int acsr_attn_calib_bwd2_saved(const float* d_ctx_cal0, const float* d_pen_sq0, const float* d_ctx_att1, const float* d_ctx_cal1,
+                               const float* d_pen_sq1, const float* mq, const float* mk, const float* mv, const float* aq,
+                               const float* ak, const float* gate_logit, const int64_t* item_seq, const float* order_w,
+                               const float* order_b, const float* dist_w, const float* dist_b, const float* scalar, int B, int L,
+                               int H, int dh, int two_level, int combine_option, float comb_scalar, int rich_mode,
+                               const float* rich_ratio, float p_attn, const float* D1, const float* D2, const float* D3,
+                               const float* noise, const void* rng, uint32_t rng_stream, float* d_mq, float* d_mk, float* d_mv,
+                               float* d_aq, float* d_ak, float* d_gate_logit, float* d_order_w, float* d_order_b,
+                               float* d_dist_w, float* d_dist_b, float* d_scalar, float* d_rich_ratio, const float* state,
+                               const int32_t* order, const int64_t* ctx_rows, void* stream) {
   AttnParams p = {};
   attn_fill_common(p, mq, mk, mv, aq, ak, gate_logit, item_seq, order_w, order_b, dist_w, dist_b, scalar, B, L, H, dh, two_level,
                    combine_option, comb_scalar, rich_mode, rich_ratio, p_attn, D1, D2, D3, noise, rng, rng_stream, order, ctx_rows);
@@ -329,8 +330,29 @@
   if (rc) return rc;
   ACSR_REQUIRE(d_mq && d_mk && d_mv && d_aq && d_ak, "attn_calib_bwd2: NULL output");
   ACSR_REQUIRE(combine_option != ACSR_ATTN_COMBINE_GATE || d_gate_logit != nullptr, "attn_calib_bwd2: d_gate_logit is NULL");
+  ACSR_REQUIRE(state == nullptr || L <= 64, "attn_calib_bwd2: the saved state is implemented for L <= 64 (L=%d)", L);
   if (L > 64) return attn_long_bwd(p, 2, (cudaStream_t)stream);
+  if (state != nullptr) {
+    p.state = const_cast<float*>(state);
+    return dispatch_bwd<2, true>(p, (cudaStream_t)stream);
+  }
   return dispatch_bwd<2>(p, (cudaStream_t)stream);
 }
 
-}
+int acsr_attn_calib_bwd2(const float* d_ctx_cal0, const float* d_pen_sq0, const float* d_ctx_att1, const float* d_ctx_cal1,
+                         const float* d_pen_sq1, const float* mq, const float* mk, const float* mv, const float* aq,
+                         const float* ak, const float* gate_logit, const int64_t* item_seq, const float* order_w,
+                         const float* order_b, const float* dist_w, const float* dist_b, const float* scalar, int B, int L, int H,
+                         int dh, int two_level, int combine_option, float comb_scalar, int rich_mode, const float* rich_ratio,
+                         float p_attn, const float* D1, const float* D2, const float* D3, const float* noise, const void* rng,
+                         uint32_t rng_stream, float* d_mq, float* d_mk, float* d_mv, float* d_aq, float* d_ak,
+                         float* d_gate_logit, float* d_order_w, float* d_order_b, float* d_dist_w, float* d_dist_b,
+                         float* d_scalar, float* d_rich_ratio, const int32_t* order, const int64_t* ctx_rows, void* stream) {
+  return acsr_attn_calib_bwd2_saved(d_ctx_cal0, d_pen_sq0, d_ctx_att1, d_ctx_cal1, d_pen_sq1, mq, mk, mv, aq, ak, gate_logit,
+                                    item_seq, order_w, order_b, dist_w, dist_b, scalar, B, L, H, dh, two_level, combine_option,
+                                    comb_scalar, rich_mode, rich_ratio, p_attn, D1, D2, D3, noise, rng, rng_stream, d_mq, d_mk,
+                                    d_mv, d_aq, d_ak, d_gate_logit, d_order_w, d_order_b, d_dist_w, d_dist_b, d_scalar,
+                                    d_rich_ratio, nullptr, order, ctx_rows, stream);
+}
+
+}
diff --git a/ac-tsr_b200/csrc/attn_bwd_rows.cuh b/ac-tsr_b200/csrc/attn_bwd_rows.cuh
--- a/ac-tsr_b200/csrc/attn_bwd_rows.cuh
+++ b/ac-tsr_b200/csrc/attn_bwd_rows.cuh
@@ -24,7 +24,7 @@
   float sc2;
 };
 
-template <int DH, int G, int NJ, int NS, bool LONG = false>
+template <int DH, int G, int NJ, int NS, bool LONG = false, bool SAVED = false>
 __device__ __forceinline__ void bwd_row_iter(const AttnParams& p, const AttnSmem& sm, const BwdSmem<NS>& bs, const RowConst& kc,
                                              const BwdFlags& f, const float* dpen, int b, int h, int i, bool rowok, int bound,
                                              int grp, int sub, int rstride, float* wbuf, BwdAcc& acc, float* accOq,
@@ -33,7 +33,8 @@
   using CM = CMap<DH, G>;
   const int L = p.L, LP = (L + 3) & ~3;
   RowF<NJ> r;
-  row_forward<DH, G, NJ>(p, sm, kc, b, h, i, bound, sub, f.has_att, r);
+  if (SAVED) row_load<G, NJ>(p, sm, kc, b, h, i, bound, sub, f.has_att, r);
+  else row_forward<DH, G, NJ>(p, sm, kc, b, h, i, bound, sub, f.has_att, r);
   const unsigned act = r.act;
   float d0[NJ], d1[NJ];
 #pragma unroll
diff --git a/ac-tsr_b200/csrc/attn_common.cuh b/ac-tsr_b200/csrc/attn_common.cuh
--- a/ac-tsr_b200/csrc/attn_common.cuh
+++ b/ac-tsr_b200/csrc/attn_common.cuh
@@ -37,7 +37,27 @@
   const float *d_pen0, *d_pen1;
   long long s1_td, s1_ll;
   float *d_mq, *d_mk, *d_mv, *d_aq, *d_ak, *d_gate, *d_ow, *d_ob, *d_dw, *d_db, *d_scalar, *d_ratio;
-};
+  float* state;
+};
+
+struct StatePlanes {
+  int P, M, R, C;
+  int GF;
+  int P0;
+  int A, NZ;
+  int n;
+};
+__host__ __device__ __forceinline__ StatePlanes state_planes(int two_level, int combine, bool att) {
+  StatePlanes s;
+  int k = 0;
+  s.P = k++; s.M = k++; s.R = k++; s.C = k++;
+  s.GF = combine != ACSR_ATTN_COMBINE_ANNEAL ? k++ : -1;
+  s.P0 = two_level ? -1 : k++;
+  s.A = k++; s.NZ = k++;
+  s.n = att ? k : k - 2;
+  return s;
+}
+__device__ __forceinline__ float with_drop_bit(float v, float mask) { return mask == 0.f ? __int_as_float(__float_as_int(v) | 0x80000000) : v; }
 
 template <int G>
 __device__ __forceinline__ float grp_sum(float v) {
@@ -275,9 +295,26 @@
   return k;
 }
 
+__device__ __forceinline__ long long state_plane_floats(const AttnParams& p) { return (long long)p.B * p.H * p.L * ((p.L + 3) & ~3); }
+__device__ __forceinline__ long long state_row(const AttnParams& p, int b, int h, int i) {
+  return (((long long)b * p.H + h) * p.L + i) * ((p.L + 3) & ~3);
+}
+
+__device__ __forceinline__ void calib_terms(const AttnParams& p, const AttnSmem& sm, const RowConst& kc, int i, int j, float rowO,
+                                            float rowD, float& sg, float& dl) {
+  sg = 0.f; dl = 0.f;
+  if (p.ow) sg = fsigmoid(rowO + sm.colO[j] + kc.ob);
+  if (p.dw) {
+    const int dist = i > j ? i - j : j - i;
+    dl = sm.logd[dist] - (rowD + sm.colD[j] + kc.db);
+  }
+}
+
 template <int DH, int G, int NJ>
 __device__ __forceinline__ void row_forward(const AttnParams& p, const AttnSmem& sm, const RowConst& kc, int b, int h, int i,
-                                            int bound, int sub, bool need_att, RowF<NJ>& r) {
+                                            int bound, int sub, bool need_att, RowF<NJ>& r, float* st = nullptr) {
+  const StatePlanes sp = state_planes(p.two_level, p.combine, need_att);
+  const long long ps = st != nullptr ? state_plane_floats(p) : 0;
   constexpr int dhp = DH + 4;
   const int L = p.L;
   int jc[NJ];
@@ -357,19 +394,10 @@
     const bool v = a && (p.bidir || j <= i) && (sm.keyok[j] != 0.f);
     valid |= (v ? 1u : 0u) << jj;
     const float msk = v ? 0.f : kMaskNeg;
-    r.sig[jj] = 0.f; r.delta[jj] = 0.f;
+    calib_terms(p, sm, kc, i, j, rowO, rowD, r.sig[jj], r.delta[jj]);
     float eo = 0.f, ed = 0.f;
-    if (p.ow) {
-      const float sg = fsigmoid(rowO + sm.colO[j] + kc.ob);
-      r.sig[jj] = sg;
-      eo = (j > i) ? flog(sg + kOrderEps) : flog((1.0f - sg) + kOrderEps);
-    }
-    if (p.dw) {
-      const int dist = i > j ? i - j : j - i;
-      const float dl = sm.logd[dist] - (rowD + sm.colD[j] + kc.db);
-      r.delta[jj] = dl;
-      ed = -(dl * dl) * kc.sc2h;
-    }
+    if (p.ow) eo = (j > i) ? flog(r.sig[jj] + kOrderEps) : flog((1.0f - r.sig[jj]) + kOrderEps);
+    if (p.dw) ed = -(r.delta[jj] * r.delta[jj]) * kc.sc2h;
     zP[jj] = (S[jj] + eo + ed) * kc.inv_sq + msk;
     z0[jj] = S[jj] * kc.inv_sq + msk;
     zM[jj] = S2[jj] * kc.inv_sq + msk;
@@ -421,6 +449,17 @@
       if (p.noise) r.nz[jj] = p.noise[e];
     }
   }
+  if (st != nullptr) {
+#pragma unroll
+    for (int jj = 0; jj < NJ; ++jj) {
+      if (!((act >> jj) & 1u)) continue;
+      float* e = st + G * jj;
+      e[sp.P * ps] = with_drop_bit(r.Psoft[jj], r.D1[jj]);
+      e[sp.M * ps] = with_drop_bit(r.Msoft[jj], r.D3[jj]);
+      if (sp.P0 >= 0) e[sp.P0 * ps] = with_drop_bit(r.P0soft[jj], r.D2[jj]);
+      if (need_att) e[sp.NZ * ps] = r.nz[jj];
+    }
+  }
   float O[NJ], M[NJ], expm[NJ], z[NJ];
 #pragma unroll
   for (int jj = 0; jj < NJ; ++jj) {
@@ -475,10 +514,19 @@
     const bool fixed = p.combine == ACSR_ATTN_COMBINE_FIXED;
 #pragma unroll
     for (int jj = 0; jj < NJ; ++jj) r.R[jj] = fixed ? r.F[jj] : (((act >> jj) & 1u) ? z[jj] : 0.f);
-    return;
-  }
-  if (kc.bounded) softmax_row_bounded<G, NJ>(z, act, r.R);
+  } else if (kc.bounded) softmax_row_bounded<G, NJ>(z, act, r.R);
   else softmax_row<G, NJ>(z, act, r.R);
+  if (st != nullptr) {
+#pragma unroll
+    for (int jj = 0; jj < NJ; ++jj) {
+      if (!((act >> jj) & 1u)) continue;
+      float* e = st + G * jj;
+      e[sp.R * ps] = r.R[jj];
+      e[sp.C * ps] = r.C[jj];
+      if (sp.GF >= 0) e[sp.GF * ps] = p.combine == ACSR_ATTN_COMBINE_FIXED ? r.F[jj] : r.g[jj];
+      if (need_att) e[sp.A * ps] = r.A[jj];
+    }
+  }
 }
 
 template <int DH, int G, int NJ>
@@ -523,6 +571,54 @@
 #pragma unroll
     for (int jj = 0; jj < NJ; ++jj) if ((act >> jj) & 1u) D3[jj] = p.D3[ebase + jc[jj]];
   }
+}
+
+
+__device__ __forceinline__ float saved_mask(const RowConst& kc, float v, const float* Dt, long long e) {
+  if (Dt != nullptr) return Dt[e];
+  if (kc.philox_drop) return (__float_as_int(v) < 0) ? 0.f : kc.inv_keep;
+  return 1.0f;
+}
+
+template <int G, int NJ>
+__device__ __forceinline__ void row_load(const AttnParams& p, const AttnSmem& sm, const RowConst& kc, int b, int h, int i,
+                                         int bound, int sub, bool need_att, RowF<NJ>& r) {
+  const StatePlanes sp = state_planes(p.two_level, p.combine, need_att);
+  const long long ps = state_plane_floats(p);
+  const float* e0 = p.state + state_row(p, b, h, i) + sub;
+  const long long ebase = (((long long)b * p.H + h) * p.L + i) * p.L + sub;
+  const float rowO = sm.rowO[i], rowD = sm.rowD[i];
+  unsigned act = 0;
+#pragma unroll
+  for (int jj = 0; jj < NJ; ++jj) {
+    const int j = sub + G * jj;
+    const bool a = j < bound;
+    act |= (a ? 1u : 0u) << jj;
+    r.Psoft[jj] = r.Msoft[jj] = r.P0soft[jj] = 0.f;
+    r.D1[jj] = r.D2[jj] = r.D3[jj] = 1.0f;
+    r.nz[jj] = r.A[jj] = r.C[jj] = r.g[jj] = r.F[jj] = r.R[jj] = 0.f;
+    r.sig[jj] = r.delta[jj] = 0.f;
+    if (!a) continue;
+    const float* e = e0 + G * jj;
+    const float vP = __ldg(e + sp.P * ps), vM = __ldg(e + sp.M * ps);
+    r.Psoft[jj] = fabsf(vP); r.D1[jj] = saved_mask(kc, vP, p.D1, ebase + G * jj);
+    r.Msoft[jj] = fabsf(vM); r.D3[jj] = saved_mask(kc, vM, p.D3, ebase + G * jj);
+    r.R[jj] = __ldg(e + sp.R * ps);
+    r.C[jj] = __ldg(e + sp.C * ps);
+    if (sp.GF >= 0) {
+      const float v = __ldg(e + sp.GF * ps);
+      if (p.combine == ACSR_ATTN_COMBINE_FIXED) r.F[jj] = v;
+      else r.g[jj] = v;
+    } else r.g[jj] = p.comb_scalar;
+    if (sp.P0 >= 0) {
+      const float v = __ldg(e + sp.P0 * ps);
+      r.P0soft[jj] = fabsf(v); r.D2[jj] = saved_mask(kc, v, p.D2, ebase + G * jj);
+    }
+    if (need_att) { r.A[jj] = __ldg(e + sp.A * ps); r.nz[jj] = __ldg(e + sp.NZ * ps); }
+    calib_terms(p, sm, kc, i, j, rowO, rowD, r.sig[jj], r.delta[jj]);
+  }
+  r.act = act;
+  r.valid = 0;
 }
 
 __device__ __forceinline__ AttnSmem carve_common(float*& ptr, int LP, int dh) {
diff --git a/ac-tsr_b200/csrc/attn_fwd.cu b/ac-tsr_b200/csrc/attn_fwd.cu
--- a/ac-tsr_b200/csrc/attn_fwd.cu
+++ b/ac-tsr_b200/csrc/attn_fwd.cu
@@ -2,7 +2,7 @@
 
 namespace acsr {
 
-template <int DH, int G, int MAXNJ>
+template <int DH, int G, int MAXNJ, bool SAVE>
 __device__ __forceinline__ void fwd_rows(const AttnParams& p, const AttnSmem& sm, const RowConst& kc, int b, int h, int nkey,
                                          bool need_att, int rstride, FwdCtx& cx) {
   constexpr int RPW = 32 / G;
@@ -25,14 +25,14 @@
       else fwd_row_iter_m<DH, G, (MAXNJ >= 4 ? 4 : 1)>(p, sm, kc, b, h, i, rowok, bound, sub, cx);
       continue;
     }
-    if (MAXNJ == 1 || nj == 1) fwd_row_iter<DH, G, 1>(p, sm, kc, b, h, i, rowok, bound, grp, sub, need_att, rstride, cx);
-    else if (nj == 2) fwd_row_iter<DH, G, (MAXNJ >= 2 ? 2 : 1)>(p, sm, kc, b, h, i, rowok, bound, grp, sub, need_att, rstride, cx);
-    else if (nj == 3) fwd_row_iter<DH, G, (MAXNJ >= 3 ? 3 : 1)>(p, sm, kc, b, h, i, rowok, bound, grp, sub, need_att, rstride, cx);
-    else fwd_row_iter<DH, G, (MAXNJ >= 4 ? 4 : 1)>(p, sm, kc, b, h, i, rowok, bound, grp, sub, need_att, rstride, cx);
+    if (MAXNJ == 1 || nj == 1) fwd_row_iter<DH, G, 1, SAVE>(p, sm, kc, b, h, i, rowok, bound, grp, sub, need_att, rstride, cx);
+    else if (nj == 2) fwd_row_iter<DH, G, (MAXNJ >= 2 ? 2 : 1), SAVE>(p, sm, kc, b, h, i, rowok, bound, grp, sub, need_att, rstride, cx);
+    else if (nj == 3) fwd_row_iter<DH, G, (MAXNJ >= 3 ? 3 : 1), SAVE>(p, sm, kc, b, h, i, rowok, bound, grp, sub, need_att, rstride, cx);
+    else fwd_row_iter<DH, G, (MAXNJ >= 4 ? 4 : 1), SAVE>(p, sm, kc, b, h, i, rowok, bound, grp, sub, need_att, rstride, cx);
   }
 }
 
-template <int DH>
+template <int DH, bool SAVE>
 __global__ void __launch_bounds__(kAttnThreads, 4) attn_fwd_kernel(const AttnParams p) {
   pdl_launch_dependents();
   pdl_wait();
@@ -60,8 +60,8 @@
       for (int k = 0; k < 6; ++k) base[k * plane + e] = 0.f;
     __syncthreads();
   }
-  if (nkey <= 8) fwd_rows<DH, 8, 1>(p, sm, kc, b, h, nkey, need_att, 8, cx);
-  else fwd_rows<DH, 16, 4>(p, sm, kc, b, h, nkey, need_att, LP, cx);
+  if (nkey <= 8) fwd_rows<DH, 8, 1, SAVE>(p, sm, kc, b, h, nkey, need_att, 8, cx);
+  else fwd_rows<DH, 16, 4, SAVE>(p, sm, kc, b, h, nkey, need_att, LP, cx);
   const double pd = warp_sum_d((double)cx.pen);
   if (lane == 0 && p.pen_sq != nullptr) {
     atomicAdd(pen_red, pd);
@@ -76,13 +76,17 @@
   return f * sizeof(float) + kAttnWarps * sizeof(double);
 }
 
+template <int DH, bool SAVE>
+static int launch_fwd_k(const AttnParams& p, cudaStream_t st) {
+  size_t smem = fwd_smem_bytes(p.L, DH);
+  int rc = prep_kernel(attn_fwd_kernel<DH, SAVE>, smem, "attn_calib_fwd");
+  if (rc) return rc;
+  launch_pdl(attn_fwd_kernel<DH, SAVE>, dim3(p.B * p.H), dim3(kAttnThreads), smem, st, p);
+  return check_launch("attn_calib_fwd");
+}
 template <int DH>
 static int launch_fwd(const AttnParams& p, cudaStream_t st) {
-  size_t smem = fwd_smem_bytes(p.L, DH);
-  int rc = prep_kernel(attn_fwd_kernel<DH>, smem, "attn_calib_fwd");
-  if (rc) return rc;
-  launch_pdl(attn_fwd_kernel<DH>, dim3(p.B * p.H), dim3(kAttnThreads), smem, st, p);
-  return check_launch("attn_calib_fwd");
+  return p.state != nullptr ? launch_fwd_k<DH, true>(p, st) : launch_fwd_k<DH, false>(p, st);
 }
 
 __global__ void __launch_bounds__(256) seq_order_kernel(const int64_t* __restrict__ item_seq, int B, int L, int32_t* __restrict__ order) {
@@ -128,15 +132,16 @@
                                    int two_level, int combine_option, float comb_scalar, int rich_mode, const float* rich_ratio,
                                    float p_attn, const float* D1, const float* D2, const float* D3, const float* noise,
                                    const void* rng, uint32_t rng_stream, float* ctx_att, float* ctx_cal, double* pen_sq,
-                                   float* probs_out, const int32_t* order, const int64_t* ctx_rows, void* stream) {
+                                   float* probs_out, float* state, const int32_t* order, const int64_t* ctx_rows, void* stream) {
   AttnParams p = {};
   attn_fill_common(p, mq, mk, mv, aq, ak, gate_logit, item_seq, order_w, order_b, dist_w, dist_b, scalar, B, L, H, dh, two_level,
                    combine_option, comb_scalar, rich_mode, rich_ratio, p_attn, D1, D2, D3, noise, rng, rng_stream, order, ctx_rows);
-  p.ctx_att = ctx_att; p.ctx_cal = ctx_cal; p.pen_sq = pen_sq; p.probs = probs_out;
+  p.ctx_att = ctx_att; p.ctx_cal = ctx_cal; p.pen_sq = pen_sq; p.probs = probs_out; p.state = state;
   plain_range(p, ctx_att != nullptr || probs_out != nullptr);
   int rc = attn_validate(p, "attn_calib_fwd");
   if (rc) return rc;
   ACSR_REQUIRE(ctx_cal != nullptr, "attn_calib_fwd: ctx_cal is NULL");
+  ACSR_REQUIRE(state == nullptr || L <= 64, "attn_calib_fwd: the saved state is implemented for L <= 64 (L=%d)", L);
   if (L > 64) return attn_long_fwd(p, (cudaStream_t)stream);
   switch (dh) {
     case 8: return launch_fwd<8>(p, (cudaStream_t)stream);
@@ -145,6 +150,12 @@
     case 64: return launch_fwd<64>(p, (cudaStream_t)stream);
   }
   return ACSR_ERR_UNSUPPORTED;
+}
+
+extern "C" int64_t acsr_attn_state_floats(int B, int L, int H, int two_level, int combine_option, int attacked) {
+  if (B <= 0 || H <= 0 || L < 1 || L > 64) return 0;
+  const StatePlanes sp = state_planes(two_level & 1, combine_option, attacked != 0);
+  return (int64_t)sp.n * B * H * L * ((L + 3) & ~3);
 }
 
 extern "C" int acsr_attn_calib_ti_fwd(const float* s_bias, const float* mq, const float* mk, const float* mv, const float* aq,
diff --git a/ac-tsr_b200/csrc/attn_fwd_rows.cuh b/ac-tsr_b200/csrc/attn_fwd_rows.cuh
--- a/ac-tsr_b200/csrc/attn_fwd_rows.cuh
+++ b/ac-tsr_b200/csrc/attn_fwd_rows.cuh
@@ -8,14 +8,15 @@
   float pen;
 };
 
-template <int DH, int G, int NJ>
+template <int DH, int G, int NJ, bool SAVE = false>
 __device__ __forceinline__ void fwd_row_iter(const AttnParams& p, const AttnSmem& sm, const RowConst& kc, int b, int h, int i,
                                              bool rowok, int bound, int grp, int sub, bool need_att, int rstride, FwdCtx& cx) {
   constexpr int dhp = DH + 4;
   using CM = CMap<DH, G>;
   const int L = p.L;
   RowF<NJ> r;
-  row_forward<DH, G, NJ>(p, sm, kc, b, h, i, bound, sub, need_att, r);
+  row_forward<DH, G, NJ>(p, sm, kc, b, h, i, bound, sub, need_att, r,
+                         (SAVE && rowok) ? p.state + state_row(p, b, h, i) + sub : nullptr);
   float* bufR = cx.rowbuf + (grp * 2 + 0) * rstride;
   float* bufA = cx.rowbuf + (grp * 2 + 1) * rstride;
 #pragma unroll
diff --git a/ac-tsr_b200/fused_step.py b/ac-tsr_b200/fused_step.py
--- a/ac-tsr_b200/fused_step.py
+++ b/ac-tsr_b200/fused_step.py
@@ -56,6 +56,11 @@
             qkv, aqk = qkv5[:3], qkv5[3:]
             lb = dict(qkv5=qkv5, qkv=qkv, aqk=aqk, mq=qkv[0], mk=qkv[1], mv=qkv[2], aq=aqk[0], ak=aqk[1], gl=f(T, L),
                       ctx=f(2 * T if last else T, d))
+            if grads:
+                layer = m.trm_encoder.layer[l]
+                n = LIB.query('acsr_attn_state_floats', Bs, L, m.n_heads, int(bool(layer.two_level)),
+                              ops.COMBINE_IDS[layer.combine_option], 1 if last else 0)
+                lb['state'] = f(n) if n > 0 else None
             if not last:
                 lb.update(hz=f(T, d), st_a=f(T, 2), h=f(T, d), z1=f(T, I), a1=f(T, I), z2=f(T, d), st_f=f(T, 2), out=f(T, d))
             if grads:
@@ -332,7 +337,8 @@
             if l == 0:
                 cur.wait_event(order_done)
             LIB.call('acsr_attn_calib_fwd', *lb['attn_args'], _p(ctx_att), _p(ctx_cal),
-                     jb['pen'][l:].data_ptr() if need_att else None, None, _p(b['order'], torch.int32),
+                     jb['pen'][l:].data_ptr() if need_att else None, None, _p(lb.get('state')) if training else None,
+                     _p(b['order'], torch.int32),
                      _p(ln, torch.int64) if l == N - 1 else None, st)
             m_a, m_f = mask2(l, 'D5', 'D4', last), mask2(l, 'D7', 'D6', last)
             if l == N - 1:
@@ -474,10 +480,10 @@
             dc = b['d_ctx']
             d_att1, d_cal1 = (dc[T:], None) if last else (None, dc[T:])
             ops.attn_workspace(Bs, L, m.n_heads, 2, seq.device)
-            LIB.call('acsr_attn_calib_bwd2', _p(dc[:T]), None, _p(d_att1), _p(d_cal1), _p(dpen[l:l + 1]), *lb['attn_args'],
+            LIB.call('acsr_attn_calib_bwd2_saved', _p(dc[:T]), None, _p(d_att1), _p(d_cal1), _p(dpen[l:l + 1]), *lb['attn_args'],
                      _p(lb['d_mq']), _p(lb['d_mk']), _p(lb['d_mv']), _p(lb['d_aq']), _p(lb['d_ak']),
                      _p(lb['d_gl']) if gate else None, _p(g(ow)), _p(g(ob_)), _p(g(dw)), _p(g(db_)), _p(g(sc)), _p(g(rr)),
-                     _p(b['order'], torch.int32), _p(ln, torch.int64) if last else None, st)
+                     _p(lb['state']), _p(b['order'], torch.int32), _p(ln, torch.int64) if last else None, st)
             aqt, akt = aa.attack_query_transform, aa.attack_key_transform
             self._wgrad(lb['d_aq'][T:], lb['mq'], T, aqt.weight.grad, aqt.bias.grad, wg)
             self._wgrad(lb['d_ak'][T:], lb['mk'], T, akt.weight.grad, akt.bias.grad, wg)
diff --git a/ac-tsr_b200/ops.py b/ac-tsr_b200/ops.py
--- a/ac-tsr_b200/ops.py
+++ b/ac-tsr_b200/ops.py
@@ -239,7 +239,7 @@
                  _p(order_w), _p(order_b), _p(dist_w), _p(dist_b), _p(scalar), B, L, H, dh,
                  opts.two_level, opts.combine, float(comb_scalar), opts.rich, _p(rich_ratio),
                  p_attn, _p(D1), _p(D2), _p(D3), _p(noise), rngp, rng_stream,
-                 _p(ctx_att), _p(ctx_cal), pen.data_ptr(), _p(probs), None, None, _stream())
+                 _p(ctx_att), _p(ctx_cal), pen.data_ptr(), _p(probs), None, None, None, _stream())
         ctx.save_for_backward(mq, mk, mv, aq, ak, gate_logit, key_ids, order_w, order_b, dist_w, dist_b, scalar, rich_ratio,
                               D1, D2, D3, noise)
         ctx.meta = (B, L, H, dh, opts, float(comb_scalar), p_attn, rng, rng_stream, need_att)
diff --git a/include/acsr.h b/include/acsr.h
--- a/include/acsr.h
+++ b/include/acsr.h
@@ -53,8 +53,9 @@
                         int two_level, int combine_option, float comb_scalar, int rich_mode, const float* rich_ratio,
                         float p_attn, const float* D1, const float* D2, const float* D3, const float* noise,
                         const void* rng, uint32_t rng_stream,
-                        float* ctx_att, float* ctx_cal, double* pen_sq, float* probs_out,
+                        float* ctx_att, float* ctx_cal, double* pen_sq, float* probs_out, float* state,
                         const int32_t* order, const int64_t* ctx_rows, void* stream);
+int64_t acsr_attn_state_floats(int B, int L, int H, int two_level, int combine_option, int attacked);
 int acsr_attn_calib_bwd(const float* d_ctx_att, const float* d_ctx_cal, const float* d_pen_sq,
                         const float* mq, const float* mk, const float* mv, const float* aq, const float* ak,
                         const float* gate_logit, const int64_t* item_seq,
@@ -82,6 +83,20 @@
                          float* d_gate_logit, float* d_order_w, float* d_order_b,
                          float* d_dist_w, float* d_dist_b, float* d_scalar, float* d_rich_ratio,
                         const int32_t* order, const int64_t* ctx_rows, void* stream);
+int acsr_attn_calib_bwd2_saved(const float* d_ctx_cal0, const float* d_pen_sq0,
+                               const float* d_ctx_att1, const float* d_ctx_cal1, const float* d_pen_sq1,
+                               const float* mq, const float* mk, const float* mv, const float* aq, const float* ak,
+                               const float* gate_logit, const int64_t* item_seq,
+                               const float* order_w, const float* order_b,
+                               const float* dist_w, const float* dist_b, const float* scalar,
+                               int B, int L, int H, int dh,
+                               int two_level, int combine_option, float comb_scalar, int rich_mode, const float* rich_ratio,
+                               float p_attn, const float* D1, const float* D2, const float* D3, const float* noise,
+                               const void* rng, uint32_t rng_stream,
+                               float* d_mq, float* d_mk, float* d_mv, float* d_aq, float* d_ak,
+                               float* d_gate_logit, float* d_order_w, float* d_order_b,
+                               float* d_dist_w, float* d_dist_b, float* d_scalar, float* d_rich_ratio, const float* state,
+                               const int32_t* order, const int64_t* ctx_rows, void* stream);
 
 int acsr_bias_dropout_res_ln_fwd(const float* h, const float* bias, const float* res,
                                  const float* ln_w, const float* ln_b, float eps, int T, int d, int res_rows,
```

New measurement: 413,300 (median of 6 runs). About the same (+0.8%).
